# visinf/veto

Measured on AMD Instinct MI355X. Metric: relation-pairs/sec (PredCls, 36 obj/img), higher is better.
Workload: dtype fp16 + e4m3 correction terms (fp16 MFMA main product, e4m3 K=128 MFMA cross terms, fp32 accumulate); 1 GPU; BASELINE.json configs[1]: synthetic PredCls, 12 img x 36 obj = 15120 pairs/GPU, d=576, 8 heads, 4 layers, 51 predicates; images_per_gpu=12, objects_per_image=36, pairs_per_gpu=15120, layers=4, heads=8, precision=mixed, parallelism=single GPU

## Files before the change

### include/veto_amd.h

```cpp
#ifndef VETO_AMD_H_
#define VETO_AMD_H_

#include <stddef.h>
#include <stdint.h>

#ifdef __cplusplus
extern "C" {
#endif

typedef struct veto_handle_s* veto_handle_t;

enum veto_status {
  VETO_OK = 0,
  VETO_ERR_INVALID = -1,
  VETO_ERR_HIP = -2,
  VETO_ERR_WEIGHTS = -3,
  VETO_ERR_WORKSPACE = -4
};

enum veto_precision {
  VETO_PRECISE = 0,
  VETO_FAST = 1,
  VETO_MIXED = 2
};
// ... 425 lines not shown
  float* norms;
  float* total_norm;
  float* coef;
} veto_optim_args_t;

size_t veto_optim_step_workspace_bytes(const veto_optim_args_t* args);
int veto_optim_step(void* stream, const veto_optim_args_t* args, void* workspace, size_t workspace_bytes);

typedef struct veto_roi_pool_args {
  int32_t struct_size;
  int32_t n_levels;
  int32_t n_img, n_roi;
  int32_t channels;
  int32_t depth_channels;
  int32_t pooled;
  int32_t sampling_ratio;
  const float* level_feat[4];
  int32_t level_h[4];
  int32_t level_w[4];
  float level_scale[4];
  const float* depth_feat;
  int32_t depth_h, depth_w;
  const float* rois;
  float* out_rgb;
  float* out_depth;
  int32_t* out_levels;
} veto_roi_pool_args_t;

int veto_roi_pool(void* stream, const veto_roi_pool_args_t* args);

int veto_roi_pool_backward(void* stream, const veto_roi_pool_args_t* args, const float* grad_rgb, const float* grad_depth,
                           float* const* level_grad, float* depth_grad);

typedef struct veto_sgg_eval_args {
  int32_t struct_size;
  int32_t n_img;
  int32_t n_rel_cls;
  int32_t n_zeroshot;
  float iou_thres;
  int32_t reserved0;
  const int32_t* gt_offset;
  const int32_t* obj_offset;
  const int32_t* pair_offset;
  const int64_t* gt_rels;
  const int64_t* gt_classes;
  const float* gt_boxes;
  const int64_t* pred_pairs;
  const float* rel_scores;
  const int64_t* pred_classes;
  const float* pred_boxes;
  const float* obj_scores;
  const int64_t* zeroshot;
  int32_t* gc_rank;
  int32_t* ng_rank;
  int32_t* acc_rank;
  int32_t* zeroshot_flag;
  int32_t* ng_rows;
  int32_t* ng_cols;
  int32_t* ng_count;
  double* metrics;
  const int32_t* pred_obj_offset;
} veto_sgg_eval_args_t;

size_t veto_sgg_eval_workspace_bytes(int32_t n_img, int32_t n_pair_total, int32_t n_gt_total, int32_t n_rel_cls);
int veto_sgg_eval(void* stream, const veto_sgg_eval_args_t* args, int32_t n_pair_total, int32_t n_gt_total,
                  void* workspace, size_t workspace_bytes);

typedef struct veto_sgg_eval_fold_args {
  int32_t struct_size;
  int32_t n_img;
  int32_t n_rel_cls;
  int32_t mode;
  int32_t n_gt_total;
  int32_t reserved0;
  const int32_t* img_gt_offset;
  const int32_t* img_pair_count;
  const int32_t* gt_predicate;
  const int32_t* gc_rank;
  const int32_t* ng_rank;
  const int32_t* acc_rank;
  const int32_t* zeroshot_flag;
  double* metrics;
  double* per_image;
} veto_sgg_eval_fold_args_t;

size_t veto_sgg_eval_fold_workspace_bytes(int32_t n_img, int32_t n_rel_cls);
int veto_sgg_eval_fold(void* stream, const veto_sgg_eval_fold_args_t* args, void* workspace, size_t workspace_bytes);

int veto_sgg_eval_fold_limits(int32_t* images_per_chunk, int32_t* max_rel_cls);

typedef struct veto_det_eval_match_args {
  int32_t struct_size;
  int32_t n_img;
  int32_t n_cls;
  int32_t n_gt;
  int32_t n_det;
  int32_t reserved0;
  int64_t first_gt_id;
  int64_t row_offset;
  double iou_thrs[10];
  double area_rngs[8];
  const int32_t* gt_offset;
  const int32_t* det_offset;
  const int32_t* gt_offset_host;
  const int32_t* det_offset_host;
  const float* gt_boxes;
  const int64_t* gt_labels;
  const float* det_boxes;
  const float* det_scores;
  const int64_t* det_labels;
  uint64_t* rec_key;
  uint64_t* rec_match;
  uint64_t* rec_ignore;
  int64_t* gt_counts;
  int32_t* label_errors;
} veto_det_eval_match_args_t;

size_t veto_det_eval_match_workspace_bytes(int32_t n_img, int32_t n_gt, int32_t n_det);
int veto_det_eval_match(void* stream, const veto_det_eval_match_args_t* args, void* workspace, size_t workspace_bytes);

typedef struct veto_det_eval_accumulate_args {
  int32_t struct_size;
  int32_t n_cls;
  int64_t n_rec;
  double iou_thrs[10];
  double rec_thrs[101];
  const uint64_t* rec_key;
  const uint64_t* rec_match;
  const uint64_t* rec_ignore;
  const int64_t* gt_counts;
  double* precision;
  double* recall;
  double* stats;
  double* recall50_100;
} veto_det_eval_accumulate_args_t;

size_t veto_det_eval_accumulate_workspace_bytes(int64_t n_rec, int32_t n_cls);
int veto_det_eval_accumulate(void* stream, const veto_det_eval_accumulate_args_t* args, void* workspace, size_t workspace_bytes);

int veto_det_eval_limits(int32_t* max_gt_per_image, int32_t* max_det_per_image, int32_t* scan_chunk, int32_t* sort_tile);

int veto_profile_enable(veto_handle_t h, int32_t on);
int veto_profile_collect(veto_handle_t h);
int veto_profile_entry(veto_handle_t h, int index, const char** name, double* total_ms, int64_t* launches,
                       double* flops_per_launch, double* bytes_per_launch);
int veto_profile_reset(veto_handle_t h);

int veto_debug_gemm(void* stream, const float* a, const float* w, const float* bias, float* c, int32_t m,
                    int32_t n, int32_t k, int32_t precision, void* workspace, size_t workspace_bytes);
size_t veto_debug_gemm_workspace_bytes(int32_t m, int32_t n, int32_t k);
int veto_debug_gemm_forms(void* stream, const float* a, const float* w, void* c, int32_t m, int32_t n, int32_t k,
                          int32_t kb_tiles, int32_t kb_steps, int32_t out_form, void* workspace, size_t workspace_bytes);

int veto_debug_ffn(void* stream, const float* a, const float* w1, const float* b1, const float* w2, const float* b2,
                   float* x, int32_t m, int32_t mode, int32_t flags, int32_t reps, float* ms_per_rep, void* workspace,
                   size_t workspace_bytes, const float* ln_w, const float* ln_b, void* ln_rows);
size_t veto_debug_ffn_workspace_bytes(int32_t m);

int veto_debug_outproj(void* stream, const float* a, const float* w, const float* b, float* x, int32_t m, int32_t mode,
                       int32_t flags, int32_t reps, float* ms_per_rep, void* workspace, size_t workspace_bytes,
                       const float* ln_w, const float* ln_b, void* ln_rows);
size_t veto_debug_outproj_workspace_bytes(int32_t m);

int veto_debug_layer_tail(void* stream, const float* a, const float* wo, const float* bo, const float* ln2_w, const float* ln2_b,
                          const float* w1, const float* b1, const float* w2, const float* b2, float* x, int32_t m, int32_t mode,
                          int32_t reps, float* ms_per_rep, void* workspace, size_t workspace_bytes, const float* ln_w,
                          const float* ln_b, void* ln_rows);
size_t veto_debug_layer_tail_workspace_bytes(int32_t m);

int veto_debug_qkv_attn(void* stream, const float* a, const float* wqkv, int32_t n_pair, int32_t heads, int32_t mode, int32_t reps,
                        float* ms_per_rep, void* workspace, size_t workspace_bytes, void* out_rows);
size_t veto_debug_qkv_attn_workspace_bytes(int32_t n_pair);

size_t veto_ce_loss_workspace_bytes(int32_t n);
int veto_ce_loss(void* stream, const float* logits, int64_t ld, const int64_t* labels, const float* weight,
                 const int64_t* rows, int32_t n, int32_t n_cls, float* loss, float* grad, void* workspace,
                 size_t workspace_bytes);

int veto_meet_sample(void* stream, const int64_t* labels, int32_t n, const uint32_t* words, int32_t n_words,
                     const int32_t* incre_idx_list, const int32_t* pos_in_group, const int32_t* group_size,
                     const double* sample_rates, int32_t n_groups, int32_t n_cls, int64_t* chosen,
                     int64_t* group_labels, int32_t* counts, int32_t* words_used);

typedef struct veto_train_opts {
  int32_t struct_size;
  float p_pos, p_emb, p_attn;
  uint64_t seed;
  float* d_roi_rgb;
  float* d_roi_depth;
} veto_train_opts_t;

size_t veto_train_workspace_bytes(veto_handle_t h, int32_t n_obj, int32_t n_pair);
size_t veto_grad_floats(veto_handle_t h);
int veto_weight_offset(veto_handle_t h, int index, size_t* offset_floats);
int veto_forward_train(veto_handle_t h, void* stream, const veto_inputs_t* in, const veto_train_opts_t* opts, void* workspace,
                       size_t workspace_bytes, float* out_logits);
int veto_backward(veto_handle_t h, void* stream, const veto_inputs_t* in, const veto_train_opts_t* opts, void* workspace,
                  size_t workspace_bytes, const float* dlogits, float* grads);

int veto_debug_wgrad(void* stream, const float* dy, const float* x, float* dw, int32_t m, int32_t n, int32_t k,
                     int32_t k_splits, void* workspace, size_t workspace_bytes);
size_t veto_debug_wgrad_workspace_bytes(int32_t m, int32_t n, int32_t k, int32_t k_splits);

int veto_debug_attention_backward(void* stream, const float* qkv, const float* dout, float* dqkv, int32_t n_pair, int32_t heads);
size_t veto_debug_layernorm_backward_workspace_bytes(int32_t rows);
int veto_debug_layernorm_backward(void* stream, const float* x, const float* dy, const float* gamma, const float* dres,
                                  float* dx, float* dgamma_dbeta, int32_t rows, void* workspace, size_t workspace_bytes);
int veto_debug_gelu_backward(void* stream, const float* pre, const float* dh, float* dpre, size_t n);
int veto_debug_column_sums(void* stream, const float* dy, int64_t ld, int32_t rows, int32_t n_cols, float* out,
                           void* workspace, size_t workspace_bytes);

#define VETO_ATTN_BWD_CLS_ONLY 1u
#define VETO_ATTN_BWD_QKV_F24 2u
#define VETO_ATTN_BWD_SPLIT_OUT 4u
int veto_debug_attention_backward_forms(void* stream, const void* qkv, const float* dout, void* dqkv, float* qkv_unpacked,
                                        int32_t n_pair, int32_t heads, uint32_t flags);
int32_t veto_debug_layernorm_backward_col_partial_rows(int32_t rows);
int veto_debug_layernorm_backward_split(void* stream, const float* x, const float* dy, const float* gamma, const float* dres,
                                        float* dx, float* dgamma_dbeta, void* split_rows, float* col_partials, int32_t rows,
                                        uint64_t drop_seed, uint32_t drop_thresh, float drop_scale, void* workspace,
                                        size_t workspace_bytes);

#ifdef __cplusplus
}
#endif
#endif
```

### veto_amd/csrc/abi_core.hip

```cpp
#include <atomic>
#include <cstdlib>
#include <cstring>

#include "abi_internal.h"

thread_local std::string g_abi_err;

namespace veto {
bool env_knob_is(const char* name, const char* value) {
  const char* v = getenv(name);
  return v && !strcmp(v, value);
}
int device_cu_count() {
  static std::atomic<int> cache[64];
  int dev = 0, cus = 0;
  if (hipGetDevice(&dev) != hipSuccess || dev < 0) return -1;
  if (dev < 64 && (cus = cache[dev].load(std::memory_order_relaxed)) > 0) return cus;
  if (hipDeviceGetAttribute(&cus, hipDeviceAttributeMultiprocessorCount, dev) != hipSuccess || cus <= 0) return -1;
  if (dev < 64) cache[dev].store(cus, std::memory_order_relaxed);
  return cus;
}
int env_knob_int(const char* name, int dflt) {
  const char* v = getenv(name);
  return v ? atoi(v) : dflt;
}
}

static int fold_block_width(int heads) {
  static const bool off = env_knob_is("VETO_FOLD_BLOCKS", "0");
  if (off || heads <= 0 || kDim % heads != 0) return 0;
  const int dhp = (kDim / heads + 31) / 32 * 32;
  return 192 % dhp == 0 && (heads * dhp) % 192 == 0 ? dhp : 0;
}

int finalize_weights(veto_handle_t h, hipStream_t s, bool train_only) {
  for (const Param& q : h->params)
    if (!q.loaded) return fail(VETO_ERR_WEIGHTS, "weight '%s' was never loaded", q.name.c_str());
  const int L = h->cfg.layers;
  const bool base = h->dirty;
  for (int l = 0; l < L; ++l) {
    LayerW& w = h->layers[l];
    if (base)
      for (int i = 0; i < 4; ++i) {
        const LayerLinear& q = kLayerLinears[i];
        HIP_TRY(launch_split_rows(h->p(lname(l, q.weight)), w.split(i), q.N, q.K, s));
      }
    if (h->cfg.precision != VETO_PRECISE && !train_only)
      for (int i = 0; i < 4; ++i) {
        const LayerLinear& q = kLayerLinears[i];
        HIP_TRY(launch_mixed_weight_rows(h->p(lname(l, q.weight)), w.mixed_rows(i), q.N, q.K, w.exp_m + i, s));
      }
  }
  if (base) {
  const std::string pe = std::string(kT) + "patch_embed.";
  HIP_TRY(launch_build_patch_weight(h->p(pe + "proj_d.weight"), h->p(pe + "proj_d.bias"), h->p(pe + "proj_v.weight"),
                                    h->p(pe + "proj_v.bias"), h->patch_w, h->patch_bias, s));
  HIP_TRY(launch_transpose_pair_proj(h->p("location_projection.0.weight"), h->loc_wt, kPosDim, s));
  HIP_TRY(launch_transpose_pair_proj(h->p("class_projection.0.weight"), h->cls_wt, h->cfg.embed_dim, s));
  HIP_TRY(launch_transpose_head(h->p("rel_out.weight"), h->head_wt, h->cfg.num_out, s));
  }
  if (train_only) {
    h->dirty = false;
    h->infer_dirty = true;
    ++h->weight_gen;
    return VETO_OK;
  }
  {
    const std::string T0 = kT;
    HIP_TRY(launch_qkv0_consts(h->p(lname(0, "0.fn.to_qkv.weight")), h->layers[0].ln1_w, h->layers[0].ln1_b, h->p(T0 + "pos_embedding"),
                               h->p(T0 + "cls_token"), h->fold_tmp, h->q0_vec, s));
    HIP_TRY(launch_split_rows(h->fold_tmp, h->q0_w, 3 * kDim, kDim, s));
  }
  if (h->cfg.heads <= cls_fold_max_heads()) {
    const int H = h->cfg.heads, dh = kDim / H;
    const float* qkv = h->p(lname(L - 1, "0.fn.to_qkv.weight"));
    const float* wo = h->p(lname(L - 1, "0.fn.to_out.0.weight"));
    if (h->fold_dhp > 0) {
      const int np = H * h->fold_dhp;
      HIP_TRY(launch_fold_blocks(qkv, wo, h->fold_tmp, 0, H, h->fold_dhp, s));
      HIP_TRY(launch_split_rows(h->fold_tmp, h->fold_q, (size_t)np, kDim, s));
      HIP_TRY(launch_fold_blocks(qkv, wo, h->fold_tmp, 1, H, h->fold_dhp, s));
      HIP_TRY(launch_split_rows(h->fold_tmp, h->fold_k, (size_t)H * kDim, np, s));
      HIP_TRY(launch_fold_blocks(qkv, wo, h->fold_tmp, 2, H, h->fold_dhp, s));
      HIP_TRY(launch_split_rows(h->fold_tmp, h->fold_v, (size_t)np, H * kDim, s));
      HIP_TRY(launch_fold_blocks(qkv, wo, h->fold_tmp, 3, H, h->fold_dhp, s));
      HIP_TRY(launch_split_rows(h->fold_tmp, h->fold_o, (size_t)kDim, np, s));
    } else {
    for (int hd = 0; hd < H; ++hd)
      HIP_TRY(launch_sgemm_tn(qkv + ((size_t)kDim + hd * dh) * kDim, kDim, qkv + (size_t)hd * dh * kDim, kDim,
                              h->fold_tmp + (size_t)hd * kDim * kDim, kDim, dh, kDim, kDim, s));
    HIP_TRY(launch_split_rows(h->fold_tmp, h->fold_m, (size_t)H * kDim, kDim, s));
    for (int hd = 0; hd < H; ++hd)
      HIP_TRY(launch_sgemm_nn(wo + hd * dh, kDim, qkv + ((size_t)2 * kDim + hd * dh) * kDim, kDim, h->fold_tmp + (size_t)hd * kDim,
                              (long)H * kDim, kDim, kDim, dh, s));
    HIP_TRY(launch_split_rows(h->fold_tmp, h->fold_n, (size_t)kDim, H * kDim, s));
    }
  }
  if (base) ++h->weight_gen;
  h->dirty = false;
  h->infer_dirty = false;
  return VETO_OK;
}

int run_gemm(veto_handle_t h, hipStream_t s, const char* name, const __bf16* a, SplitW w, const float* bias,
             const float* resid, long ldr, float* c, __bf16* c_split, long ldc, int M, int N, int K, int epi,
             long lda, int w_row0, DropSite drop, const int* w_exp, int kb_tiles, int kb_steps) {
  GemmArgs g{};
  g.kb_tiles = kb_tiles; g.kb_steps = kb_steps;
  if (w_exp) { g.fmt = FMT_MIXED; g.w_exp = w_exp; }
  if (drop.thresh) {
    if (epi != EPI_RESID) return fail(VETO_ERR_INVALID, "dropout is fused into the residual epilogue only");
    epi = EPI_RESID_DROP;
    g.drop_seed = drop.seed; g.drop_thresh = drop.thresh; g.drop_scale = drop.scale; g.drop_row_step = drop.row_step;
  }
  g.a = a; g.lda = lda;
  g.w = w + (size_t)w_row0 * 2 * K;
  g.bias = bias; g.resid = resid; g.c = c; g.c_split = c_split;
  g.M = M; g.N = N; g.K = K; g.ldr = ldr; g.ldc = ldc;
  if (epi == EPI_PRE_GELU) g.ldc_f32 = N;
  const double kk = kb_tiles > 0 ? 32.0 * kb_steps : (double)K;
  const double flops = 2.0 * M * (double)N * kk;
  const double bytes = 4.0 * ((double)M * K + (double)N * kk) + (double)M * N * (epi == EPI_RESID ? 8.0 : epi == EPI_F24 ? 3.0 : 4.0);
  ProfScope ps(h, s, name, flops, bytes);
  HIP_TRY(launch_gemm_split(g, epi, 0, s));
  return VETO_OK;
}

static size_t carve_derived(veto_handle_t h, char* base) {
  Carver c{base};
  const veto_config_t& cfg = h->cfg;
  const int L = cfg.layers, E = cfg.embed_dim;
  const bool mixed = cfg.precision != VETO_PRECISE;
  for (LayerW& w : h->layers) {
    w.qkv = c.take<__bf16>((size_t)3 * kDim * kDim * 4);
    w.out = c.take<__bf16>((size_t)kDim * kDim * 4);
    w.fc1 = c.take<__bf16>((size_t)2 * kDim * kDim * 4);
    w.fc2 = c.take<__bf16>((size_t)2 * kDim * kDim * 4);
    if (!mixed) continue;
    w.qkv_m = c.take<__bf16>((size_t)3 * kDim * kDim * 4);
    w.out_m = c.take<__bf16>((size_t)kDim * kDim * 4);
    w.fc1_m = c.take<__bf16>((size_t)2 * kDim * kDim * 4);
    w.fc2_m = c.take<__bf16>((size_t)2 * kDim * kDim * 4);
  }
  int* exps = c.take<int>((size_t)L * 4 * sizeof(int));
  for (int l = 0; l < L && mixed && exps; ++l) h->layers[l].exp_m = exps + 4 * l;
  h->patch_w = c.take<__bf16>((size_t)2 * kDim * 2048 * 4);
  h->patch_bias = c.take<float>((size_t)2 * kDim * 4);
  h->loc_wt = c.take<float>((size_t)kPosDim * 2 * kDim * 4);
  h->cls_wt = c.take<float>((size_t)E * 2 * kDim * 4);
  h->head_wt = c.take<float>((size_t)kDim * cfg.num_out * 4);
  const int fold_dhp = h->fold_dhp = fold_block_width(cfg.heads);
  const size_t fold_np = (size_t)cfg.heads * (fold_dhp > 0 ? fold_dhp : 0);
  const size_t fold_el = fold_dhp > 0 ? (size_t)cfg.heads * kDim * fold_np : (size_t)cfg.heads * kDim * kDim;
  h->fold_m = c.take<__bf16>(fold_dhp > 0 ? 256 : fold_el * 4);
  h->fold_n = c.take<__bf16>(fold_dhp > 0 ? 256 : fold_el * 4);
  h->fold_tmp = c.take<float>(fold_el * 4);
  h->fold_q = c.take<__bf16>(fold_np * kDim * 4 + 256);
  h->fold_k = c.take<__bf16>((size_t)cfg.heads * kDim * fold_np * 4 + 256);
  h->fold_v = c.take<__bf16>((size_t)cfg.heads * kDim * fold_np * 4 + 256);
  h->fold_o = c.take<__bf16>(fold_np * kDim * 4 + 256);
  h->q0_w = c.take<__bf16>((size_t)3 * kDim * kDim * 4);
  h->q0_vec = c.take<float>((size_t)3 * 3 * kDim * 4);
  return c.off;
}

extern "C" {

const char* veto_last_error(void) { return g_abi_err.c_str(); }
const char* veto_version(void) { return "veto_amd 0.1 (gfx950)"; }

int veto_create(const veto_config_t* cfg, veto_handle_t* out) {
  CHECK_STRUCT_AND(veto_config_t, cfg, out != nullptr);
  if (cfg->dim != kDim) return fail(VETO_ERR_INVALID, "T_INPUT_DIM must be 576 (proj_d 512 + proj_v 64), got %d", cfg->dim);
  if (cfg->patch != 2 || cfg->channels != 256 || cfg->resolution != 8)
    return fail(VETO_ERR_INVALID, "only PATCH_SIZE 2, 256 channels, POOLER_RESOLUTION 8 are supported");
  if (cfg->layers < 1 || cfg->layers > 64) return fail(VETO_ERR_INVALID, "bad ENC_LAYERS %d", cfg->layers);
  if (cfg->heads < 1 || kDim % cfg->heads != 0 || (kDim / cfg->heads) % 4 != 0)
    return fail(VETO_ERR_INVALID, "NHEADS %d must divide 576 with head dim %% 4 == 0", cfg->heads);
  if (cfg->num_obj_cls < 2 || cfg->num_obj_cls > 256 || cfg->embed_dim < 1 || cfg->embed_dim > 256)
    return fail(VETO_ERR_INVALID, "num_obj_cls/embed_dim out of range");
  if (cfg->num_out < 1 || cfg->num_out > 4096) return fail(VETO_ERR_INVALID, "bad num_out %d", cfg->num_out);
  if (cfg->precision != VETO_PRECISE && cfg->precision != VETO_FAST && cfg->precision != VETO_MIXED) return fail(VETO_ERR_INVALID, "bad precision");
  HIP_TRY(hipSetDevice(cfg->device));

  veto_handle_t h = new veto_handle_s();
  h->cfg = *cfg;
  h->dh = kDim / cfg->heads;
  h->chunk = cfg->max_chunk_pairs > 0 ? cfg->max_chunk_pairs : 32768;
  const int E = cfg->embed_dim, L = cfg->layers;
  h->add("obj_embed.weight", (size_t)cfg->num_obj_cls * E);
  h->add("class_projection.0.weight", (size_t)kDim * 2 * E);
  h->add("class_projection.0.bias", kDim);
  h->add("pos_embed.0.weight", 4);
  h->add("pos_embed.0.bias", 4);
  h->add("pos_embed.0.running_mean", 4);
  h->add("pos_embed.0.running_var", 4);
  h->add("pos_embed.1.weight", (size_t)kPosDim * 4);
  h->add("pos_embed.1.bias", kPosDim);
  h->add("location_projection.0.weight", (size_t)kDim * 2 * kPosDim);
  h->add("location_projection.0.bias", kDim);
  h->add(std::string(kT) + "cls_token", kDim);
  h->add(std::string(kT) + "pos_embedding", kDim);
  h->add(std::string(kT) + "patch_embed.proj_d.weight", (size_t)512 * 2048);
  h->add(std::string(kT) + "patch_embed.proj_d.bias", 512);
  h->add(std::string(kT) + "patch_embed.proj_v.weight", (size_t)64 * 2048);
  h->add(std::string(kT) + "patch_embed.proj_v.bias", 64);
  for (int l = 0; l < L; ++l) {
    h->add(lname(l, "0.norm.weight"), kDim);
    h->add(lname(l, "0.norm.bias"), kDim);
    h->add(lname(l, "0.fn.to_qkv.weight"), (size_t)3 * kDim * kDim);
    h->add(lname(l, "0.fn.to_out.0.weight"), (size_t)kDim * kDim);
    h->add(lname(l, "0.fn.to_out.0.bias"), kDim);
    h->add(lname(l, "1.norm.weight"), kDim);
    h->add(lname(l, "1.norm.bias"), kDim);
    h->add(lname(l, "1.fn.net.0.weight"), (size_t)2 * kDim * kDim);
    h->add(lname(l, "1.fn.net.0.bias"), 2 * kDim);
    h->add(lname(l, "1.fn.net.3.weight"), (size_t)2 * kDim * kDim);
    h->add(lname(l, "1.fn.net.3.bias"), kDim);
  }
  h->add("rel_out.weight", (size_t)cfg->num_out * kDim);
  h->add("rel_out.bias", cfg->num_out);
  for (Param& q : h->params) {
    q.offset = h->raw_floats;
    h->raw_floats += align_up(q.numel, 64);
  }
  hipError_t e = hipMalloc((void**)&h->raw, h->raw_floats * sizeof(float));
  if (e != hipSuccess) { delete h; return fail(VETO_ERR_HIP, "hipMalloc(raw weights): %s", hipGetErrorString(e)); }

  h->layers.resize(L);
  e = hipMalloc((void**)&h->derived, carve_derived(h, nullptr));
  if (e != hipSuccess) { (void)hipFree(h->raw); delete h; return fail(VETO_ERR_HIP, "hipMalloc(derived weights): %s", hipGetErrorString(e)); }
  carve_derived(h, h->derived);
  for (int l = 0; l < L; ++l) {
    LayerW& w = h->layers[l];
    w.ln1_w = h->p(lname(l, "0.norm.weight")); w.ln1_b = h->p(lname(l, "0.norm.bias"));
    w.ln2_w = h->p(lname(l, "1.norm.weight")); w.ln2_b = h->p(lname(l, "1.norm.bias"));
    w.out_b = h->p(lname(l, "0.fn.to_out.0.bias"));
    w.fc1_b = h->p(lname(l, "1.fn.net.0.bias"));
    w.fc2_b = h->p(lname(l, "1.fn.net.3.bias"));
  }
  if (cfg->precision == VETO_MIXED) {
    e = hipMalloc((void**)&h->sat_buf, (size_t)L * VETO_SAT_SITES * 4 * sizeof(unsigned long long));
    if (e != hipSuccess) { (void)hipFree(h->raw); (void)hipFree(h->derived); delete h; return fail(VETO_ERR_HIP, "hipMalloc(saturation counters): %s", hipGetErrorString(e)); }
  }
  *out = h;
  return VETO_OK;
}

int veto_destroy(veto_handle_t h) {
  if (!h) return VETO_OK;
  for (ProfRec& r : h->prof_recs) { (void)hipEventDestroy(r.start); (void)hipEventDestroy(r.stop); }
  for (hipEvent_t e : h->event_pool) (void)hipEventDestroy(e);
  (void)hipFree(h->raw);
  (void)hipFree(h->derived);
  if (h->sat_buf) (void)hipFree(h->sat_buf);
  delete h;
  return VETO_OK;
}

int veto_num_weights(veto_handle_t h) { return h ? (int)h->params.size() : fail(VETO_ERR_INVALID, "null handle"); }

int veto_weight_info(veto_handle_t h, int index, const char** name, size_t* numel) {
  if (!h || index < 0 || index >= (int)h->params.size()) return fail(VETO_ERR_INVALID, "bad weight index");
  if (name) *name = h->params[index].name.c_str();
  if (numel) *numel = h->params[index].numel;
  return VETO_OK;
}

int veto_load_weights(veto_handle_t h, const char* name, const float* src, size_t numel, void* stream) {
  if (!h || !name || !src) return fail(VETO_ERR_INVALID, "null argument");
  auto it = h->index.find(name);
  if (it == h->index.end()) return fail(VETO_ERR_INVALID, "unknown weight '%s'", name);
  Param& q = h->params[it->second];
  if (q.numel != numel) return fail(VETO_ERR_INVALID, "weight '%s': expected %zu elements, got %zu", name, q.numel, numel);
  HIP_TRY(hipMemcpyAsync(h->raw + q.offset, src, numel * sizeof(float), hipMemcpyDefault, (hipStream_t)stream));
  q.loaded = true;
  h->dirty = true;
// ... 57 lines not shown
```

### veto_amd/csrc/abi_debug.hip

```cpp
#include "abi_internal.h"

namespace {

struct EventTimer {
  hipEvent_t e0 = nullptr, e1 = nullptr;
  hipStream_t s = nullptr;
  float total_ms = 0.f;
  hipError_t init(hipStream_t stream) {
    s = stream;
    hipError_t e = hipEventCreate(&e0);
    return e != hipSuccess ? e : hipEventCreate(&e1);
  }
  hipError_t start() { return e1 ? hipEventRecord(e0, s) : hipSuccess; }
  hipError_t stop() {
    if (!e1) return hipSuccess;
    float ms = 0.f;
    hipError_t e = hipEventRecord(e1, s);
    if (e == hipSuccess) e = hipEventSynchronize(e1);
    if (e == hipSuccess) e = hipEventElapsedTime(&ms, e0, e1);
    total_ms += ms;
    return e;
  }
  ~EventTimer() {
    if (e0) (void)hipEventDestroy(e0);
    if (e1) (void)hipEventDestroy(e1);
  }
};

const size_t kW = (size_t)kDim * kDim * 4;
size_t act_bytes(size_t rows, size_t k) { return (size_t)gemm_rows_padded((int)rows) * k * 4; }

struct GemmWs { __bf16 *a, *w; int* w_exp; size_t total; };
GemmWs carve_gemm(Carver c, int m, int n, int k) {
  return GemmWs{c.take<__bf16>(act_bytes(m, k)), c.take<__bf16>((size_t)n * k * 4), c.take<int>(256), c.off};
}

struct FfnWs { __bf16 *a, *hid, *w1, *w2; int* exps; size_t total; };
FfnWs carve_ffn(Carver c, int m) {
  return FfnWs{c.take<__bf16>(act_bytes(m, kDim)), c.take<__bf16>(act_bytes(m, 2 * kDim)), c.take<__bf16>(2 * kW), c.take<__bf16>(2 * kW),
               c.take<int>(256), c.off};
}

struct OutprojWs { __bf16 *a, *w; int* exps; size_t total; };
OutprojWs carve_outproj(Carver c, int m) {
  return OutprojWs{c.take<__bf16>(act_bytes(m, kDim)), c.take<__bf16>(kW), c.take<int>(256), c.off};
}

struct LayerTailWs { __bf16 *a, *wo, *w1, *w2; int* exps; size_t total; };
LayerTailWs carve_layer_tail(Carver c, int m) {
  return LayerTailWs{c.take<__bf16>(act_bytes(m, kDim)), c.take<__bf16>(kW), c.take<__bf16>(2 * kW), c.take<__bf16>(2 * kW), c.take<int>(256),
                     c.off};
}

struct QkvAttnWs { __bf16* a; char *o, *qkv; __bf16* w; int* exps; size_t total; };
QkvAttnWs carve_qkv_attn(Carver c, int n_pair) {
  const size_t tile_rows = qkv_attn_rows_padded(n_pair), m = (size_t)n_pair * kTokens, rows = tile_rows > m ? tile_rows : m;
  return QkvAttnWs{c.take<__bf16>(act_bytes(rows, kDim)), c.take(act_bytes(rows, kDim)), c.take((size_t)gemm_rows_padded((int)rows) * 3 * kDim * 3),
                   c.take<__bf16>(3 * kW), c.take<int>(256), c.off};
}

}

extern "C" {

size_t veto_debug_gemm_workspace_bytes(int32_t m, int32_t n, int32_t k) {
  if (m <= 0 || n <= 0 || k <= 0) return 0;
  return carve_gemm(Carver{nullptr}, m, n, k).total;
}

int veto_debug_gemm(void* stream, const float* a, const float* w, const float* bias, float* c, int32_t m, int32_t n,
                    int32_t k, int32_t precision, void* workspace, size_t workspace_bytes) {
  if (!a || !w || !c || !workspace) return fail(VETO_ERR_INVALID, "null argument");
  ABI_TRY(check_workspace(workspace, workspace_bytes, veto_debug_gemm_workspace_bytes(m, n, k), false));
  hipStream_t s = (hipStream_t)stream;
  const auto [a_s, w_s, w_exp, ws_bytes] = carve_gemm(Carver{(char*)workspace}, m, n, k);
  HIP_TRY(hipMemsetAsync(a_s, 0, (char*)w_s - (char*)a_s, s));
  GemmArgs g{};
  if (precision == VETO_MIXED) {
    if (k % 64 != 0) return fail(VETO_ERR_INVALID, "mixed rows need K %% 64 == 0");
    HIP_TRY(launch_mixed_act_rows(a, a_s, (size_t)m, k, s));
    HIP_TRY(launch_mixed_weight_rows(w, w_s, (size_t)n, k, w_exp, s));
    g.fmt = FMT_MIXED; g.w_exp = w_exp;
  } else {
    HIP_TRY(launch_split_rows(a, a_s, (size_t)m, k, s));
    HIP_TRY(launch_split_rows(w, w_s, (size_t)n, k, s));
  }
  g.a = a_s; g.w = w_s; g.bias = bias; g.c = c;
  g.M = m; g.N = n; g.K = k; g.ldc = n;
  hipError_t e = launch_gemm_split(g, EPI_F32, precision == VETO_FAST ? 1 : 0, s);
  if (e != hipSuccess) return fail(e == hipErrorInvalidValue ? VETO_ERR_INVALID : VETO_ERR_HIP,
                                   "gemm launch failed (N must be a multiple of 192, K of 32): %s", hipGetErrorString(e));
  return VETO_OK;
}

int veto_debug_gemm_forms(void* stream, const float* a, const float* w, void* c, int32_t m, int32_t n, int32_t k, int32_t kb_tiles,
                          int32_t kb_steps, int32_t out_form, void* workspace, size_t workspace_bytes) {
  if (!a || !w || !c || !workspace) return fail(VETO_ERR_INVALID, "null argument");
  if (out_form < 0 || out_form > 2) return fail(VETO_ERR_INVALID, "out_form must be 0, 1 or 2");
  ABI_TRY(check_workspace(workspace, workspace_bytes, veto_debug_gemm_workspace_bytes(m, n, k), false));
  hipStream_t s = (hipStream_t)stream;
  const auto [a_s, w_s, w_exp, ws_bytes] = carve_gemm(Carver{(char*)workspace}, m, n, k);
  HIP_TRY(hipMemsetAsync(a_s, 0, (char*)w_s - (char*)a_s, s));
  HIP_TRY(launch_split_rows(a, a_s, (size_t)m, k, s));
  HIP_TRY(launch_split_rows(w, w_s, (size_t)n, k, s));
  GemmArgs g{};
  g.a = a_s; g.w = w_s; g.M = m; g.N = n; g.K = k;
  g.kb_tiles = kb_tiles; g.kb_steps = kb_steps;
  if (out_form == 1) { g.c_split = (__bf16*)c; g.ldc = 2L * n; }
  else { g.c = (float*)c; g.ldc = n; }
  hipError_t e = launch_gemm_split(g, out_form == 1 ? EPI_SPLIT : out_form == 2 ? EPI_F24 : EPI_F32, 0, s);
  if (e != hipSuccess) return fail(e == hipErrorInvalidValue ? VETO_ERR_INVALID : VETO_ERR_HIP,
                                   "gemm launch failed (N a multiple of 192, K of 32, the blocks must tile K): %s", hipGetErrorString(e));
  return VETO_OK;
}

size_t veto_debug_ffn_workspace_bytes(int32_t m) {
  return m > 0 ? carve_ffn(Carver{nullptr}, m).total : 0;
}

int veto_debug_ffn(void* stream, const float* a, const float* w1, const float* b1, const float* w2, const float* b2, float* x,
                   int32_t m, int32_t mode, int32_t flags, int32_t reps, float* ms_per_rep, void* workspace, size_t workspace_bytes,
                   const float* ln_w, const float* ln_b, void* ln_rows) {
  if (!a || !w1 || !b1 || !w2 || !b2 || !x || !workspace) return fail(VETO_ERR_INVALID, "null argument");
  if (m <= 0 || reps <= 0 || (mode != 0 && mode != 1)) return fail(VETO_ERR_INVALID, "bad m / reps / mode");
  if (ln_rows && (!ln_w || !ln_b)) return fail(VETO_ERR_INVALID, "ln_rows needs ln_w and ln_b");
  ABI_TRY(check_workspace(workspace, workspace_bytes, veto_debug_ffn_workspace_bytes(m), false));
  hipStream_t s = (hipStream_t)stream;
  const auto [a_m, hid, w1_m, w2_m, exps, ws_bytes] = carve_ffn(Carver{(char*)workspace}, m);
  if (flags & 1) {
    HIP_TRY(hipMemsetAsync(a_m, 0, (char*)hid - (char*)a_m, s));
    HIP_TRY(launch_mixed_act_rows(a, a_m, (size_t)m, kDim, s));
    HIP_TRY(launch_mixed_weight_rows(w1, w1_m, (size_t)2 * kDim, kDim, exps + 0, s));
    HIP_TRY(launch_mixed_weight_rows(w2, w2_m, (size_t)kDim, 2 * kDim, exps + 1, s));
  }
  EventTimer timer;
  if (ms_per_rep) HIP_TRY(timer.init(s));
  HIP_TRY(timer.start());
  for (int r = 0; r < reps; ++r) {
    if (mode == 1) {
      HIP_TRY(launch_ffn_fused(ffn_panel_args(a_m, MixedLinear{w1_m, b1, exps + 0}, MixedLinear{w2_m, b2, exps + 1}, x, m,
                                              ln_rows ? RowNorm{ln_w, ln_b, ln_rows} : RowNorm()), s));
    } else {
      GemmArgs g1{};
      g1.fmt = FMT_MIXED; g1.w_exp = exps + 0; g1.a = a_m; g1.w = w1_m; g1.bias = b1; g1.c_split = hid;
      g1.M = m; g1.N = 2 * kDim; g1.K = kDim; g1.ldc = 4 * kDim;
      HIP_TRY(launch_gemm_split(g1, EPI_GELU_SPLIT, 0, s));
      GemmArgs g2{};
      g2.fmt = FMT_MIXED; g2.w_exp = exps + 1; g2.a = hid; g2.w = w2_m; g2.bias = b2; g2.resid = x; g2.c = x;
      g2.M = m; g2.N = kDim; g2.K = 2 * kDim; g2.ldr = kDim; g2.ldc = kDim;
      HIP_TRY(launch_gemm_split(g2, EPI_RESID, 0, s));
      if (ln_rows) HIP_TRY(launch_layernorm(x, kDim, ln_w, ln_b, (__bf16*)ln_rows, m, s, FMT_MIXED));
    }
  }
  HIP_TRY(timer.stop());
  if (ms_per_rep) *ms_per_rep = timer.total_ms / reps;
  return VETO_OK;
}

size_t veto_debug_outproj_workspace_bytes(int32_t m) {
  return m > 0 ? carve_outproj(Carver{nullptr}, m).total : 0;
}

int veto_debug_outproj(void* stream, const float* a, const float* w, const float* b, float* x, int32_t m, int32_t mode, int32_t flags,
                       int32_t reps, float* ms_per_rep, void* workspace, size_t workspace_bytes, const float* ln_w, const float* ln_b,
                       void* ln_rows) {
  if (!a || !w || !b || !x || !workspace) return fail(VETO_ERR_INVALID, "null argument");
  if (m <= 0 || reps <= 0 || (mode != 0 && mode != 1)) return fail(VETO_ERR_INVALID, "bad m / reps / mode");
  if (ln_rows && (!ln_w || !ln_b)) return fail(VETO_ERR_INVALID, "ln_rows needs ln_w and ln_b");
  ABI_TRY(check_workspace(workspace, workspace_bytes, veto_debug_outproj_workspace_bytes(m), false));
  hipStream_t s = (hipStream_t)stream;
  const auto [a_m, w_m, exps, ws_bytes] = carve_outproj(Carver{(char*)workspace}, m);
  if (flags & 1) HIP_TRY(launch_mixed_weight_rows(w, w_m, (size_t)kDim, kDim, exps, s));
  EventTimer timer;
  if (ms_per_rep) HIP_TRY(timer.init(s));
  for (int r = 0; r < reps; ++r) {
    HIP_TRY(hipMemsetAsync(a_m, 0, (char*)w_m - (char*)a_m, s));
    HIP_TRY(launch_mixed_act_rows(a, a_m, (size_t)m, kDim, s));
    HIP_TRY(timer.start());
    if (mode == 1) {
      HIP_TRY(launch_out_fused(out_panel_args(a_m, MixedLinear{w_m, b, exps}, x, m, ln_rows ? RowNorm{ln_w, ln_b, ln_rows} : RowNorm()), s));
    } else {
      GemmArgs g{};
      g.fmt = FMT_MIXED; g.w_exp = exps; g.a = a_m; g.w = w_m; g.bias = b; g.resid = x; g.c = x;
      g.M = m; g.N = kDim; g.K = kDim; g.ldr = kDim; g.ldc = kDim;
      HIP_TRY(launch_gemm_split(g, EPI_RESID, 0, s));
      if (ln_rows) HIP_TRY(launch_layernorm(x, kDim, ln_w, ln_b, (__bf16*)ln_rows, m, s, FMT_MIXED));
    }
    HIP_TRY(timer.stop());
  }
  if (ms_per_rep) *ms_per_rep = timer.total_ms / reps;
  return VETO_OK;
}

size_t veto_debug_layer_tail_workspace_bytes(int32_t m) {
  return m > 0 ? carve_layer_tail(Carver{nullptr}, m).total : 0;
}

int veto_debug_layer_tail(void* stream, const float* a, const float* wo, const float* bo, const float* ln2_w, const float* ln2_b,
                          const float* w1, const float* b1, const float* w2, const float* b2, float* x, int32_t m, int32_t mode,
                          int32_t reps, float* ms_per_rep, void* workspace, size_t workspace_bytes, const float* ln_w, const float* ln_b,
                          void* ln_rows) {
  if (!a || !wo || !bo || !ln2_w || !ln2_b || !w1 || !b1 || !w2 || !b2 || !x || !workspace) return fail(VETO_ERR_INVALID, "null argument");
  if (m <= 0 || reps <= 0 || (mode != 0 && mode != 1)) return fail(VETO_ERR_INVALID, "bad m / reps / mode");
  if (ln_rows && (!ln_w || !ln_b)) return fail(VETO_ERR_INVALID, "ln_rows needs ln_w and ln_b");
  ABI_TRY(check_workspace(workspace, workspace_bytes, veto_debug_layer_tail_workspace_bytes(m), false));
  hipStream_t s = (hipStream_t)stream;
  const auto [a_m, wo_m, w1_m, w2_m, exps, ws_bytes] = carve_layer_tail(Carver{(char*)workspace}, m);
  HIP_TRY(launch_mixed_weight_rows(wo, wo_m, (size_t)kDim, kDim, exps + 0, s));
  HIP_TRY(launch_mixed_weight_rows(w1, w1_m, (size_t)2 * kDim, kDim, exps + 1, s));
  HIP_TRY(launch_mixed_weight_rows(w2, w2_m, (size_t)kDim, 2 * kDim, exps + 2, s));
  EventTimer timer;
  if (ms_per_rep) HIP_TRY(timer.init(s));
  for (int r = 0; r < reps; ++r) {
    HIP_TRY(hipMemsetAsync(a_m, 0, (char*)wo_m - (char*)a_m, s));
    HIP_TRY(launch_mixed_act_rows(a, a_m, (size_t)m, kDim, s));
    HIP_TRY(timer.start());
// ... 55 lines not shown
```

### veto_amd/csrc/abi_forward.hip

```cpp
#include "abi_internal.h"

namespace {

struct Workspace {
  int32_t *subj, *obj;
  float* lc;
  __bf16* pa;
  float* patch_tab;
  float* x;
  __bf16* a;
  char* big;
  float* xc;
  __bf16* ptab_split;
  float *sw, *ow;
  float* stats;
  __bf16 *ac, *hc;
  size_t total;
};

Workspace carve(char* base, int n_obj, int n_pair, int chunk) {
  Workspace w;
  Carver c{base};
  const size_t prow = (size_t)gemm_rows_padded(n_obj * 16);
  const size_t tile_rows = qkv_attn_rows_padded(chunk);
  const size_t mpad = (size_t)gemm_rows_padded((int)(tile_rows > (size_t)chunk * kTokens ? tile_rows : (size_t)chunk * kTokens));
  const size_t cpad = (size_t)gemm_rows_padded(chunk);
  w.subj = c.take<int32_t>((size_t)n_pair * 4);
  w.obj = c.take<int32_t>((size_t)n_pair * 4);
  w.lc = c.take<float>((size_t)n_obj * 2 * 2 * kDim * 4);
  w.pa = c.take<__bf16>(prow * 2 * 2048 * 2);
  w.patch_tab = c.take<float>((size_t)n_obj * 16 * 2 * kDim * 4);
  w.x = c.take<float>(mpad * kDim * 4);
  w.a = c.take<__bf16>(mpad * 2 * kDim * 2);
  {
    const size_t qkv_bytes = mpad * 3 * kDim * 4, fold_bytes = 2 * (align_up(cpad * (size_t)cls_fold_max_heads() * kDim * 4, 256));
    w.big = c.take(qkv_bytes > fold_bytes ? qkv_bytes : fold_bytes);
  }
  w.xc = c.take<float>(cpad * kDim * 4);
  w.ptab_split = c.take<__bf16>(prow * 2 * 2 * kDim * 2);
  w.sw = c.take<float>(prow * 3 * kDim * 4);
  w.ow = c.take<float>(prow * 3 * kDim * 4);
  w.stats = c.take<float>(mpad * 2 * 4);
  w.ac = c.take<__bf16>(cpad * 2 * kDim * 2);
  w.hc = c.take<__bf16>(cpad * 4 * kDim * 2);
  w.total = c.off;
  return w;
}

struct ForwardPlan {
  int L, H, dhp;
  bool qkv0_tables, fold_last, mixed, fast, mixed_out, cls_mixed, tail_fused, panel, qkv_f24, qa_fused, x_f24;
  bool ffn_ln_next(int l) const { return mixed && panel && l + 1 < L - 1; }
};

ForwardPlan make_plan(veto_handle_t h, bool sat) {
  ForwardPlan p;
  const int L = p.L = h->cfg.layers, H = p.H = h->cfg.heads;
  p.dhp = h->fold_dhp;
  static const bool tables_off = env_knob_is("VETO_QKV0_TABLES", "0");
  p.qkv0_tables = L >= 2 && !tables_off;
  static const bool fold_off = env_knob_is("VETO_CLS_FOLD", "0");
  p.fold_last = !fold_off && H <= cls_fold_max_heads();
  p.mixed = h->cfg.precision != VETO_PRECISE;
  p.fast = h->cfg.precision == VETO_FAST;
  p.mixed_out = p.mixed && attention_reads_tables(H);
  p.cls_mixed = p.mixed;
  static const bool tail_off = env_knob_is("VETO_TAIL_FUSED", "0");
  p.tail_fused = !tail_off && !sat;
  p.panel = !sat;
  static const bool qkv_f24_off = env_knob_is("VETO_QKV_F24", "0");
  p.qkv_f24 = !qkv_f24_off && attention_reads_tables(H);
  static const bool qa_off = env_knob_is("VETO_QKV_ATTN_FUSED", "0");
  p.qa_fused = p.mixed && p.mixed_out && p.tail_fused && !qa_off && qkv_attn_fused_supports(H);
  static const bool x_f24_on = env_knob_is("VETO_X_F24", "1");
  p.x_f24 = x_f24_on && !p.fast && p.mixed && p.mixed_out && p.tail_fused && p.fold_last && p.qkv0_tables && p.qa_fused && L >= 3;
  return p;
}

int object_side(veto_handle_t h, hipStream_t s, const Workspace& ws, const ForwardPlan& p, const veto_inputs_t* in,
                const veto_debug_outputs_t* dbg) {
  const int n_obj = in->n_obj, n_pair = in->n_pair;
  {
    ProfScope ps(h, s, "pair_indices", 0, (double)n_pair * 24);
    HIP_TRY(launch_pair_indices(in->rel_pairs, in->img_obj_offset, in->img_pair_offset, in->n_img, n_pair, ws.subj,
                                ws.obj, dbg ? dbg->subj_inds : nullptr, dbg ? dbg->obj_inds : nullptr, s));
  }
  {
    if (in->bn_batch_stats) HIP_TRY(launch_bn_batch_stats(in->boxes, in->box_mode, n_obj, in->bn_batch_stats, s));
    const ObjPrepArgs a = obj_prep_args(h, in, ws.lc);
    ProfScope ps(h, s, "obj_prep", 2.0 * n_obj * 2 * kDim * (kPosDim + h->cfg.embed_dim), (double)n_obj * 2 * 2 * kDim * 4);
    HIP_TRY(launch_obj_prep(a, s));
  }
  {
    ProfScope ps(h, s, "patchify", 0, (double)n_obj * 2 * 256 * 64 * (4 + 4));
    HIP_TRY(launch_patchify(in->roi_depth, in->roi_rgb, ws.pa, n_obj, s));
  }
  int rc = run_gemm(h, s, "gemm_patch", ws.pa, h->patch_w, h->patch_bias, nullptr, 0, ws.patch_tab, nullptr, 2 * kDim,
                    n_obj * 16, 2 * kDim, 2048, EPI_F32);
  if (rc || !p.qkv0_tables) return rc;
  const int R = n_obj * 16;
  HIP_TRY(launch_centre_split(ws.patch_tab, ws.ptab_split, R, s));
  ABI_TRY(run_gemm(h, s, "gemm_qkv0_tab", ws.ptab_split, h->q0_w, h->q0_vec + 3 * kDim, nullptr, 0, ws.sw, nullptr, 3 * kDim, R, 3 * kDim, kDim,
                   EPI_F32, (long)2 * 2 * kDim, 0));
  return run_gemm(h, s, "gemm_qkv0_tab", ws.ptab_split + 2 * kDim, h->q0_w, nullptr, nullptr, 0, ws.ow, nullptr, 3 * kDim, R, 3 * kDim, kDim,
                  EPI_F32, (long)2 * 2 * kDim, 0);
}

struct Chunk {
  veto_handle_t h;
  hipStream_t s;
  const Workspace& ws;
  const ForwardPlan& p;
  int c0, np, M;
  unsigned long long* sat;
  const float* xlast;
  float* qkv() const { return (float*)ws.big; }
  __bf16* hid() const { return (__bf16*)ws.big; }
  hipError_t count_sat(int layer, int site, const void* rows, long stride_bytes, int n_rows, int K) const {
    if (!sat) return hipSuccess;
    return launch_count_saturation(rows, stride_bytes, n_rows, K, sat + ((size_t)layer * VETO_SAT_SITES + site) * 4, s);
  }

  int assemble_tokens(float* dbg_tokens) {
    {
      AssembleArgs a = assemble_args(h, ws.patch_tab, ws.lc, ws.subj + c0, ws.obj + c0, ws.x, ws.a, np);
      a.stats = p.qkv0_tables ? ws.stats : nullptr;
      a.x_f24 = p.x_f24 ? 1 : 0;
      a.a_fmt = p.mixed && p.qkv0_tables ? FMT_MIXED : FMT_SPLIT;
      ProfScope ps(h, s, "assemble_tokens", 0, (double)M * kDim * (p.x_f24 ? 3 : 4) + (p.qkv0_tables ? (double)M * 8 + 2.0 * np * kDim * 4 : (double)M * kDim * 4));
      HIP_TRY(launch_assemble(a, s));
    }
    if (dbg_tokens) {
      float* dst = dbg_tokens + (size_t)c0 * kTokens * kDim;
      if (p.x_f24) HIP_TRY(launch_unpack_f24(ws.x, dst, (size_t)M * kDim, s));
      else HIP_TRY(hipMemcpyAsync(dst, ws.x, (size_t)M * kDim * 4, hipMemcpyDeviceToDevice, s));
    }
    return VETO_OK;
  }

  int qkv0_from_tables() {
    const LayerW& w = h->layers[0];
    const bool mixed = p.mixed;
    if (!attention_reads_tables(p.H)) {
      ProfScope ps(h, s, "qkv0_combine", 0, (double)np * 17 * 3 * kDim * 4 * 3);
      HIP_TRY(launch_qkv0_combine(ws.sw, ws.ow, ws.stats, h->q0_vec, ws.subj + c0, ws.obj + c0, qkv(), np, s));
    }
    for (int t = kTokens - 2; t < kTokens; ++t) {
      if (mixed) HIP_TRY(count_sat(0, VETO_SAT_QKV_IN, ws.a + (size_t)t * 2 * kDim, (long)kTokens * kDim * 4, np, kDim));
      ABI_TRY(run_gemm(h, s, "gemm_qkv0_lc", ws.a + (size_t)t * 2 * kDim, mixed ? w.qkv_m : w.qkv, nullptr, nullptr, 0,
                       qkv() + (size_t)t * 3 * kDim, nullptr, (long)kTokens * 3 * kDim, np, 3 * kDim, kDim, EPI_F32, (long)kTokens * 2 * kDim, 0,
                       DropSite(), mixed ? w.exp_m + LIN_QKV : nullptr));
    }
    return VETO_OK;
  }

  int attention(int l, bool qkv_f24) {
    const bool last = l == p.L - 1;
    AttnArgs a{};
    a.qkv = qkv(); a.n_pair = np; a.heads = p.H; a.cls_only = last ? 1 : 0;
    a.qkv_f24 = qkv_f24 ? 1 : 0;
    a.o = last ? ws.ac : ws.a;
    a.o_fmt = (!last && p.mixed_out) ? FMT_MIXED : FMT_SPLIT;
    if (l == 0 && p.qkv0_tables && attention_reads_tables(p.H)) {
      a.sw = ws.sw; a.ow = ws.ow; a.stats = ws.stats; a.vec = h->q0_vec; a.subj = ws.subj + c0; a.obj = ws.obj + c0;
    }
    const double nq = last ? 1 : kTokens;
    ProfScope ps(h, s, last ? "attention_cls" : "attention", 4.0 * np * nq * kTokens * kDim,
                 (double)M * 3 * kDim * (qkv_f24 ? 3 : 4) + (double)np * nq * kDim * 4);
    HIP_TRY(launch_attention(a, s));
    if (a.o_fmt == FMT_MIXED) HIP_TRY(count_sat(l, VETO_SAT_ATTN_OUT, ws.a, (long)kDim * 4, M, kDim));
    return VETO_OK;
  }

  int qkv_attention(int l, bool* attn_in_big) {
    const LayerW& w = h->layers[l];
    if (p.qa_fused && l > 0) {
      QkvAttnArgs q{};
      q.a = (const char*)ws.a; q.w = (const char*)w.qkv_m; q.w_exp = w.exp_m + LIN_QKV; q.o = ws.big; q.n_pair = np; q.heads = p.H; q.fast = p.fast ? 1 : 0;
      ProfScope ps(h, s, "qkv_attn_fused", 2.0 * M * 3.0 * kDim * kDim + 4.0 * np * kTokens * kTokens * kDim,
                   (double)M * kDim * 8 + 3.0 * kDim * kDim * 4);
      HIP_TRY(launch_qkv_attn_fused(q, s));
      *attn_in_big = true;
      return VETO_OK;
    }
    const bool mq = p.mixed && l > 0;
    const bool qkv_f24 = mq && p.qkv_f24;
    if (mq) HIP_TRY(count_sat(l, VETO_SAT_QKV_IN, ws.a, (long)kDim * 4, M, kDim));
    int rc = run_gemm(h, s, "gemm_qkv", ws.a, mq ? w.qkv_m : w.qkv, nullptr, nullptr, 0, qkv(), nullptr, 3 * kDim, M, 3 * kDim, kDim,
                      qkv_f24 ? EPI_F24 : EPI_F32, 0, 0, DropSite(), mq ? w.exp_m + LIN_QKV : nullptr);
    return rc ? rc : attention(l, qkv_f24);
  }

  int layer_tail_one_launch(int l, bool attn_in_big) {
    const LayerW& w = h->layers[l];
    const LayerW& nx = h->layers[l + 1];
    const bool ln_next = p.ffn_ln_next(l);
    char* rows = attn_in_big ? ws.big : (char*)ws.a;
    const RowNorm next{ln_next ? nx.ln1_w : nullptr, ln_next ? nx.ln1_b : nullptr, attn_in_big ? ws.a : nullptr};
    FfnArgs f = layer_tail_args(rows, w.mixed(LIN_OUT), RowNorm{w.ln2_w, w.ln2_b, rows}, w.mixed(LIN_FC1), w.mixed(LIN_FC2), ws.x, M, next);
    f.fast = p.fast ? 1 : 0;
    if (p.x_f24) {
      f.resid_f24 = 1;
      if (l + 1 < p.L - 1) f.out_f24 = 1;
      else {
        if (!attn_in_big) return fail(VETO_ERR_INVALID, "internal: 3-byte residual rows without a free buffer for the last tail's fp32 rows");
        f.out = (float*)ws.a;
        xlast = (const float*)ws.a;
      }
    }
    ProfScope ps(h, s, "layer_tail_fused", 2.0 * M * (double)kDim * kDim + 2.0 * 2.0 * M * (double)kDim * 2 * kDim,
                 (double)M * kDim * (p.x_f24 ? (f.out_f24 ? 14 : 15) : 16) + 5.0 * kDim * kDim * 4);
    HIP_TRY(launch_layer_tail(f, s));
    return VETO_OK;
  }

  int out_projection(int l) {
    const LayerW& w = h->layers[l];
    if (p.mixed_out && p.panel) {
      const FfnArgs f = out_panel_args(ws.a, w.mixed(LIN_OUT), ws.x, M, RowNorm{w.ln2_w, w.ln2_b, ws.a});
      ProfScope ps(h, s, "out_ln_fused", 2.0 * M * (double)kDim * kDim, (double)M * kDim * 16 + (double)kDim * kDim * 4);
      HIP_TRY(launch_out_fused(f, s));
      return VETO_OK;
    }
    ABI_TRY(run_gemm(h, s, "gemm_out", ws.a, p.mixed_out ? w.out_m : w.out, w.out_b, ws.x, kDim, ws.x, nullptr, kDim, M, kDim, kDim, EPI_RESID,
                     0, 0, DropSite(), p.mixed_out ? w.exp_m + LIN_OUT : nullptr));
    {
      ProfScope ps(h, s, "layernorm", 0, (double)M * kDim * 8);
      HIP_TRY(launch_layernorm(ws.x, kDim, w.ln2_w, w.ln2_b, ws.a, M, s, p.mixed ? FMT_MIXED : FMT_SPLIT));
    }
    if (p.mixed) HIP_TRY(count_sat(l, VETO_SAT_FFN_IN, ws.a, (long)kDim * 4, M, kDim));
    return VETO_OK;
  }

  int feed_forward(int l) {
    const LayerW& w = h->layers[l];
    const bool mixed = p.mixed;
    if (mixed && p.panel) {
      const LayerW& nx = h->layers[l + 1];
      const FfnArgs f = ffn_panel_args(ws.a, w.mixed(LIN_FC1), w.mixed(LIN_FC2), ws.x, M,
                                       p.ffn_ln_next(l) ? RowNorm{nx.ln1_w, nx.ln1_b, ws.a} : RowNorm());
      ProfScope ps(h, s, "ffn_fused", 2.0 * 2.0 * M * (double)kDim * 2 * kDim, (double)M * kDim * 12 + 2.0 * 2 * kDim * kDim * 4);
      HIP_TRY(launch_ffn_fused(f, s));
      return VETO_OK;
    }
    ABI_TRY(run_gemm(h, s, "gemm_fc1", ws.a, mixed ? w.fc1_m : w.fc1, w.fc1_b, nullptr, 0, nullptr, hid(), 4 * kDim, M, 2 * kDim, kDim,
                     EPI_GELU_SPLIT, 0, 0, DropSite(), mixed ? w.exp_m + LIN_FC1 : nullptr));
    if (mixed) HIP_TRY(count_sat(l, VETO_SAT_HIDDEN, hid(), (long)2 * kDim * 4, M, 2 * kDim));
    return run_gemm(h, s, "gemm_fc2", hid(), mixed ? w.fc2_m : w.fc2, w.fc2_b, ws.x, kDim, ws.x, nullptr, kDim, M, kDim, 2 * kDim, EPI_RESID,
                    0, 0, DropSite(), mixed ? w.exp_m + LIN_FC2 : nullptr);
  }

  int layer_tail(int l, bool attn_in_big) {
    if (p.mixed_out && p.tail_fused) return layer_tail_one_launch(l, attn_in_big);
    const int rc = out_projection(l);
    return rc ? rc : feed_forward(l);
  }

  int layernorm_next(int l) {
    const LayerW& nx = h->layers[l + 1];
    if (l + 1 == p.L - 1 && p.fold_last) return VETO_OK;
    if (p.ffn_ln_next(l)) return VETO_OK;
    ProfScope ps(h, s, "layernorm", 0, (double)M * kDim * 8);
    HIP_TRY(launch_layernorm(ws.x, kDim, nx.ln1_w, nx.ln1_b, ws.a, M, s, (p.mixed && l + 1 < p.L - 1) ? FMT_MIXED : FMT_SPLIT));
    return VETO_OK;
  }

  int last_layer_folded() {
    const LayerW& w = h->layers[p.L - 1];
    const int H = p.H;
    int rc;
    Carver fold{ws.big};
    float* u = fold.take<float>((size_t)gemm_rows_padded(np) * H * kDim * 4);
    __bf16* abar = fold.take<__bf16>((size_t)gemm_rows_padded(np) * 2 * H * kDim * 2);
    {
      ProfScope ps(h, s, "layernorm_cls", 0, (double)np * kDim * 8);
      HIP_TRY(launch_layernorm(xlast, (long)kTokens * kDim, w.ln1_w, w.ln1_b, ws.ac, np, s));
    }
    const int dhp = p.dhp, npad = H * dhp;
    bool u24 = false;
    if (dhp > 0) {
      ABI_TRY(run_gemm(h, s, "gemm_q_cls", ws.ac, h->fold_q, nullptr, nullptr, 0, nullptr, ws.hc, 2L * npad, np, npad, kDim, EPI_SPLIT));
      u24 = cls_fold_reads_f24();
      rc = run_gemm(h, s, "gemm_u_cls", ws.hc, h->fold_k, nullptr, nullptr, 0, u, nullptr, (long)H * kDim, np, H * kDim, npad,
                    u24 ? EPI_F24 : EPI_F32, 0, 0, DropSite(), nullptr, 3, dhp / 32);
    } else {
      rc = run_gemm(h, s, "gemm_u_cls", ws.ac, h->fold_m, nullptr, nullptr, 0, u, nullptr, (long)H * kDim, np, H * kDim, kDim, EPI_F32);
    }
    if (rc) return rc;
    {
      ProfScope ps(h, s, "attention_cls", 4.0 * np * H * kTokens * kDim, (double)M * kDim * 4 + (double)np * H * kDim * 8);
      HIP_TRY(launch_cls_fold_attention(xlast, w.ln1_w, w.ln1_b, u, abar, np, H, s, u24));
    }
    if (dhp > 0) {
      const int hpt = 192 / dhp;
      ABI_TRY(run_gemm(h, s, "gemm_v_cls", abar, h->fold_v, nullptr, nullptr, 0, nullptr, ws.hc, 2L * npad, np, npad, H * kDim, EPI_SPLIT,
                       0, 0, DropSite(), nullptr, 1, hpt * kDim / 32));
      return run_gemm(h, s, "gemm_out_cls", ws.hc, h->fold_o, w.out_b, xlast, (long)kTokens * kDim, ws.xc, nullptr, kDim, np, kDim, npad,
                      EPI_RESID);
// ... 125 lines not shown
```

### veto_amd/csrc/abi_internal.h

```cpp
#pragma once
#include <hip/hip_runtime.h>

#include <cmath>
#include <cstdarg>
#include <cstddef>
#include <cstdint>
#include <cstdio>
#include <map>
#include <string>
#include <vector>

#include "../../include/veto_amd.h"
#include "kernels.h"

using namespace veto;

#pragma GCC visibility push(hidden)

extern thread_local std::string g_abi_err;

inline int fail(int code, const char* fmt, ...) {
  char buf[512];
  va_list ap;
  va_start(ap, fmt);
// ... 96 lines not shown
  p.obj_logits = a->obj_logits; p.rel_pairs = a->rel_pairs;
  p.n_obj = a->n_obj; p.n_pair = a->n_pair; p.n_rel_cls = a->n_rel_cls; p.n_obj_cls = a->n_obj_cls;
  p.obj_scores = a->obj_scores; p.obj_pred = a->obj_pred; p.out_prob = a->rel_prob_sorted;
  p.out_pairs = a->rel_pairs_sorted; p.out_labels = a->rel_labels_sorted; p.out_triple = a->triple_sorted;
  return p;
}

struct Param {
  std::string name;
  size_t numel = 0;
  size_t offset = 0;
  bool loaded = false;
};

typedef __bf16* SplitW;

enum { LIN_QKV = 0, LIN_OUT = 1, LIN_FC1 = 2, LIN_FC2 = 3 };
struct LayerLinear { const char* weight; const char* bias; int N, K; };
const LayerLinear kLayerLinears[4] = {{"0.fn.to_qkv.weight", nullptr, 3 * kDim, kDim},
                                      {"0.fn.to_out.0.weight", "0.fn.to_out.0.bias", kDim, kDim},
                                      {"1.fn.net.0.weight", "1.fn.net.0.bias", 2 * kDim, kDim},
                                      {"1.fn.net.3.weight", "1.fn.net.3.bias", kDim, 2 * kDim}};

struct MixedLinear {
  const void* w;
  const float* b;
  const int* exp;
};

struct LayerW {
  const float *ln1_w, *ln1_b, *ln2_w, *ln2_b, *out_b, *fc1_b, *fc2_b;
  SplitW qkv = nullptr, out = nullptr, fc1 = nullptr, fc2 = nullptr;
  SplitW qkv_m = nullptr, out_m = nullptr, fc1_m = nullptr, fc2_m = nullptr;
  int* exp_m = nullptr;
  SplitW split(int lin) const { return lin == LIN_QKV ? qkv : lin == LIN_OUT ? out : lin == LIN_FC1 ? fc1 : fc2; }
  SplitW mixed_rows(int lin) const { return lin == LIN_QKV ? qkv_m : lin == LIN_OUT ? out_m : lin == LIN_FC1 ? fc1_m : fc2_m; }
  MixedLinear mixed(int lin) const {
    const float* const bias[4] = {nullptr, out_b, fc1_b, fc2_b};
    return MixedLinear{mixed_rows(lin), bias[lin], exp_m + lin};
  }
};

struct ProfRec {
  int name_id;
  hipEvent_t start, stop;
  double flops, bytes;
};

struct veto_handle_s {
  veto_config_t cfg;
  int dh = 0;
  int chunk = 0;
  std::vector<Param> params;
  std::map<std::string, int> index;
  float* raw = nullptr;
  size_t raw_floats = 0;
  char* derived = nullptr;
  bool dirty = true;
  bool infer_dirty = false;
  uint64_t weight_gen = 0;
  static constexpr size_t kMaxTrainWorkspaces = 8;
  std::map<const void*, uint64_t> train_gen;
  void stamp_train_workspace(const void* ws) {
    if (train_gen.size() >= kMaxTrainWorkspaces && !train_gen.count(ws)) {
      auto old = train_gen.begin();
      for (auto it = train_gen.begin(); it != train_gen.end(); ++it)
        if (it->second < old->second) old = it;
      train_gen.erase(old);
    }
    train_gen[ws] = weight_gen;
  }
  std::vector<LayerW> layers;
  SplitW patch_w = nullptr;
  SplitW fold_m = nullptr, fold_n = nullptr;
  float* fold_tmp = nullptr;
  SplitW fold_q = nullptr, fold_k = nullptr, fold_v = nullptr, fold_o = nullptr;
  int fold_dhp = 0;
  SplitW q0_w = nullptr;
  float* q0_vec = nullptr;
  float* patch_bias = nullptr;
  float* loc_wt = nullptr;
  float* cls_wt = nullptr;
  float* head_wt = nullptr;
  unsigned long long* sat_buf = nullptr;
  bool prof_on = false;
  std::vector<std::string> prof_names;
  std::vector<ProfRec> prof_recs;
  std::vector<hipEvent_t> event_pool;
  struct Agg { double ms = 0; int64_t n = 0; double flops = 0, bytes = 0; };
  std::vector<Agg> prof_agg;

  const float* p(const std::string& name) const { return raw + params[index.at(name)].offset; }
  void add(const std::string& name, size_t numel) {
    Param q;
    q.name = name;
    q.numel = numel;
    index[name] = (int)params.size();
    params.push_back(q);
  }
};

constexpr const char* kT = "fusion_transformer.transformer.";

inline std::string lname(int l, const char* rest) {
  char buf[160];
  snprintf(buf, sizeof(buf), "%slayers.%d.%s", kT, l, rest);
  return buf;
}

inline int prof_id(veto_handle_t h, const char* name) {
  for (size_t i = 0; i < h->prof_names.size(); ++i)
    if (h->prof_names[i] == name) return (int)i;
  h->prof_names.push_back(name);
  h->prof_agg.emplace_back();
  return (int)h->prof_names.size() - 1;
}

struct ProfScope {
  veto_handle_t h;
  hipStream_t s;
  int rec = -1;
  ProfScope(veto_handle_t h_, hipStream_t s_, const char* name, double flops, double bytes) : h(h_), s(s_) {
    if (!h || !h->prof_on) return;
    ProfRec r;
    r.name_id = prof_id(h, name);
    r.flops = flops;
    r.bytes = bytes;
    for (hipEvent_t* e : {&r.start, &r.stop}) {
      if (!h->event_pool.empty()) { *e = h->event_pool.back(); h->event_pool.pop_back(); }
      else if (hipEventCreate(e) != hipSuccess) return;
    }
    (void)hipEventRecord(r.start, s);
    h->prof_recs.push_back(r);
    rec = (int)h->prof_recs.size() - 1;
  }
  ~ProfScope() {
    if (rec >= 0) (void)hipEventRecord(h->prof_recs[rec].stop, s);
  }
};

int finalize_weights(veto_handle_t h, hipStream_t s, bool train_only = false);

struct DropSite {
  unsigned long long seed = 0;
  unsigned thresh = 0;
  float scale = 1.f;
  int row_step = 1;
};

int run_gemm(veto_handle_t h, hipStream_t s, const char* name, const __bf16* a, SplitW w, const float* bias, const float* resid, long ldr,
             float* c, __bf16* c_split, long ldc, int M, int N, int K, int epi, long lda = 0, int w_row0 = 0, DropSite drop = DropSite(),
             const int* w_exp = nullptr, int kb_tiles = 0, int kb_steps = 0);

inline ObjPrepArgs obj_prep_args(veto_handle_t h, const veto_inputs_t* in, float* lc) {
  ObjPrepArgs a{};
  a.boxes = in->boxes; a.box_mode = in->box_mode; a.labels = in->obj_labels; a.obj_logits = in->obj_logits;
  a.embed = h->p("obj_embed.weight"); a.num_obj_cls = h->cfg.num_obj_cls; a.embed_dim = h->cfg.embed_dim;
  a.bn_w = h->p("pos_embed.0.weight"); a.bn_b = h->p("pos_embed.0.bias");
  a.bn_mean = in->bn_batch_stats ? in->bn_batch_stats : h->p("pos_embed.0.running_mean");
  a.bn_var = in->bn_batch_stats ? in->bn_batch_stats + 4 : h->p("pos_embed.0.running_var");
  a.pos_w = h->p("pos_embed.1.weight"); a.pos_b = h->p("pos_embed.1.bias");
  a.loc_wt = h->loc_wt; a.loc_b = h->p("location_projection.0.bias");
  a.cls_wt = h->cls_wt; a.cls_b = h->p("class_projection.0.bias");
  a.lc = lc; a.pos_out = nullptr; a.n_obj = in->n_obj;
  return a;
}

inline AssembleArgs assemble_args(veto_handle_t h, const float* patch_tab, const float* lc, const int32_t* subj, const int32_t* obj, float* x,
                                  __bf16* a_rows, int n_pair) {
  AssembleArgs a{};
  a.patch_tab = patch_tab; a.lc = lc; a.cls_token = h->p(std::string(kT) + "cls_token");
  a.pos_embedding = h->p(std::string(kT) + "pos_embedding");
  a.ln_w = h->layers[0].ln1_w; a.ln_b = h->layers[0].ln1_b;
  a.subj = subj; a.obj = obj; a.x = x; a.a = a_rows; a.n_pair = n_pair;
  return a;
}

struct RowNorm {
  const float* w = nullptr;
  const float* b = nullptr;
  void* rows = nullptr;
};

inline FfnArgs ffn_panel_args(const void* a, MixedLinear fc1, MixedLinear fc2, float* x, int M, RowNorm next = RowNorm()) {
  FfnArgs f{};
  f.a = (const char*)a; f.w1 = (const char*)fc1.w; f.w2 = (const char*)fc2.w; f.b1 = fc1.b; f.b2 = fc2.b;
  f.resid = x; f.out = x; f.ldr = kDim; f.ldo = kDim; f.M = M; f.exp1 = fc1.exp; f.exp2 = fc2.exp;
  f.ln_w = next.w; f.ln_b = next.b; f.ln_out = (char*)next.rows;
  return f;
}

inline FfnArgs out_panel_args(const void* a, MixedLinear out, float* x, int M, RowNorm ln2 = RowNorm()) {
  FfnArgs f{};
  f.a = (const char*)a; f.w2 = (const char*)out.w; f.b2 = out.b; f.resid = x; f.out = x; f.ldr = kDim; f.ldo = kDim;
  f.M = M; f.exp2 = out.exp; f.ln_w = ln2.w; f.ln_b = ln2.b; f.ln_out = (char*)ln2.rows;
  return f;
}

inline FfnArgs layer_tail_args(const void* a, MixedLinear out, RowNorm ln2, MixedLinear fc1, MixedLinear fc2, float* x, int M,
                               RowNorm next = RowNorm()) {
  FfnArgs f = ffn_panel_args(a, fc1, fc2, x, M);
  f.wo = (const char*)out.w; f.bo = out.b; f.expo = out.exp; f.lnm_w = ln2.w; f.lnm_b = ln2.b; f.ln_out = (char*)ln2.rows;
  f.ln_w = next.w; f.ln_b = next.b; f.ln1_out = (char*)next.rows;
  return f;
}

#pragma GCC visibility pop
```

### veto_amd/csrc/gemm_split_ps.hip

```cpp
#include "common.h"
#include "kernels.h"

#include <cstdio>
#include <cstdlib>

namespace veto {

namespace {

constexpr int BM = 256, BN = 192, BK = 32;
constexpr int NCONS = 8, NLOAD = 4;
constexpr int kABytes = BM * 128;
constexpr int kWBytes = BN * 128;
constexpr int kDumpOff = 3 * kABytes + 2 * kWBytes;
constexpr int kBiasOff = kDumpOff + 1024;
constexpr int kBiasSlices = 3;
constexpr int kLdsBytes = kBiasOff + kBiasSlices * BN * 4;
constexpr int kPrefSteps = BN * 4 / 128;
constexpr int CPA = BM / 8 / NLOAD;
constexpr int CPWL = BN / 8 / NLOAD;
#ifndef VETO_GEMM_EPI_T
#define VETO_GEMM_EPI_T 1
#endif
constexpr bool kEpiT = VETO_GEMM_EPI_T;

__device__ __forceinline__ void glds16(const char* src, char* lds_dst) {
  __builtin_amdgcn_global_load_lds((const __attribute__((address_space(1))) void*)src,
                                   (__attribute__((address_space(3))) void*)lds_dst, 16, 0, 0);
}

#ifdef VETO_GEMM_STAMPS
__device__ unsigned long long g_stamps[256 * 8];
__device__ __forceinline__ unsigned long long stamp() {
  __builtin_amdgcn_sched_barrier(0);
  unsigned long long t;
  asm volatile("s_memtime %0\n\ts_waitcnt lgkmcnt(0)" : "=s"(t)::"memory");
  __builtin_amdgcn_sched_barrier(0);
  return t;
}
#define STAMP(x) x = stamp()
#define ACC(a, t1, t0) a += (t1) - (t0)
#else
#define STAMP(x)
#define ACC(a, t1, t0)
#endif

__device__ __forceinline__ void wg_barrier() {
  asm volatile("" ::: "memory");
  __builtin_amdgcn_s_barrier();
  asm volatile("" ::: "memory");
}

typedef int i32x4 __attribute__((ext_vector_type(4)));
typedef int i32x8 __attribute__((ext_vector_type(8)));
typedef _Float16 f16x8 __attribute__((ext_vector_type(8)));
template <int V> struct IntTag { static constexpr int value = V; };

typedef short s16x4 __attribute__((ext_vector_type(4)));
typedef short s16x8 __attribute__((ext_vector_type(8)));
__device__ __forceinline__ s16x4 lds_tr16(const char* p) {
  return __builtin_amdgcn_ds_read_tr16_b64_v4i16((__attribute__((address_space(3))) s16x4*)p);
}
__device__ __forceinline__ bf16x8 lds_tr_frag(const char* p, int pitch4) {
  const s16x4 a = lds_tr16(p), b = lds_tr16(p + pitch4);
  const s16x8 v = __builtin_shufflevector(a, b, 0, 1, 2, 3, 4, 5, 6, 7);
  return __builtin_bit_cast(bf16x8, v);
}

template <int NTERMS, int EPI_T, bool TN = false>
__global__ __launch_bounds__(64 * (NCONS + NLOAD), 3) void gemm_split_ps_kernel(GemmArgs g) {
  constexpr bool kDrop = EPI_T == EPI_RESID_DROP;
  constexpr bool kMixed = NTERMS == 2;
  if constexpr (kMixed) saturating_conversions_on();
  static_assert(!(kMixed && TN), "the mixed-row format has no transposed (weight-gradient) form");
  constexpr bool kGeluBwd = EPI_T == EPI_GELU_BWD;
  constexpr int EPI = kDrop || kGeluBwd ? (int)EPI_RESID : EPI_T;
  __shared__ __attribute__((aligned(16))) char smem[kLdsBytes];

  const int tid = threadIdx.x;
  const int lane = tid & 63;
  const int w = __builtin_amdgcn_readfirstlane(tid >> 6);
  const int b = blockIdx.x;
  const int ksp = EPI == EPI_ATOMIC && g.k_splits > 1 ? g.k_splits : 1;
  const int out_tiles = g.tiles_m * g.tiles_n;
  const int ntiles = out_tiles * ksp;
  const int K = g.K;
  const int nk = g.kb_tiles > 0 ? g.kb_steps : K / BK / ksp;
  const int per_xcd = gridDim.x >> 3;
  auto tile_of = [&](int it) { return (it * 8 + (b & 7)) * per_xcd + (b >> 3); };
  int my_tiles = 0;
  while (tile_of(my_tiles) < ntiles) ++my_tiles;
  if (my_tiles == 0) return;
  const int nstages = my_tiles * nk;

  if (w >= NCONS) {
    const int lw = (w - NCONS) & (NLOAD - 1);
    const int rr = lane >> 3;
    const char* srcA[CPA];
    const char* srcW[CPWL];
    auto src_of = [&](const __bf16* base, long ld, int row, int c) {
      const int r16 = ((c & 1) << 3) + rr;
      const int slot = (lane & 7) ^ ((r16 >> 1) & 7);
      return (const char*)(base + (size_t)row * ld) + slot * 16;
    };
    auto tn_swz = [](int r) { return 2 * ((r & 3) | (((r >> 3) & 1) << 2)); };
    const char* tnA = nullptr;
    const char* tnW = nullptr;
    int tn_rowA = 0, tn_rowW = 0;
    int tn_xa[2] = {0, 0}, tn_wr[CPWL], tn_wx[CPWL];
    if constexpr (TN) {
      tn_xa[0] = (lane ^ tn_swz(lw)) << 4;
      tn_xa[1] = (lane ^ tn_swz(lw + 8)) << 4;
#pragma unroll
      for (int i = 0; i < CPWL; ++i) {
        const int slot = (lw + NLOAD * i) * 64 + lane, r = slot / 48, cc = slot % 48;
        tn_wr[i] = r;
        tn_wx[i] = (cc ^ tn_swz(r)) << 4;
      }
    }
    auto setupA = [&](int tile) {
      int k0 = (tile / out_tiles) * nk;
      tile %= out_tiles;
      const int tile_m = tile / g.tiles_n;
      if (g.kb_tiles > 0) k0 = ((tile % g.tiles_n) / g.kb_tiles) * nk;
      if constexpr (TN) {
        tnA = (const char*)g.a + (size_t)tile_m * (BM * 4);
        tn_rowA = k0 * BK;
        return;
      }
#pragma unroll
      for (int i = 0; i < CPA; ++i) {
        const int c = lw + NLOAD * i;
        int row = tile_m * BM + c * 8 + rr;
        if (g.lda != 2 * K && row >= g.M) row = g.M - 1;
        srcA[i] = src_of(g.a, g.lda, row, c) + (size_t)k0 * 128;
      }
    };
    auto setupW = [&](int tile) {
      int k0 = (tile / out_tiles) * nk;
      tile %= out_tiles;
      const int tile_n = tile % g.tiles_n;
      if (g.kb_tiles > 0) k0 = (tile_n / g.kb_tiles) * nk;
      if constexpr (TN) {
        tnW = (const char*)g.w + (size_t)tile_n * (BN * 4);
        tn_rowW = k0 * BK;
        return;
      }
#pragma unroll
      for (int i = 0; i < CPWL; ++i) {
        const int c = lw + NLOAD * i;
        srcW[i] = src_of(g.w, 2 * K, tile_n * BN + c * 8 + rr, c) + (size_t)k0 * 128;
      }
    };
    int itA = 0, ktA = 0, bufA = 0, itW = 0, ktW = 0, bufW = 0;
    auto issueA = [&]() {
      if (ktA == 0 && lw == 0 && g.bias && lane < BN / 4) {
        const int tn = (tile_of(itA) % out_tiles) % g.tiles_n;
        glds16((const char*)(g.bias + tn * BN) + lane * 16, smem + kBiasOff + (itA % kBiasSlices) * (BN * 4));
      }
      char* dst = smem + bufA * kABytes + lw * 1024;
      if constexpr (TN) {
#pragma unroll
        for (int i = 0; i < CPA; ++i) {
          const int row = tn_rowA + ktA * BK + lw + NLOAD * i;
          const char* p = row < g.k_valid ? tnA + (size_t)row * (size_t)(g.lda * 2) : (const char*)g.zero;
          glds16(p + tn_xa[(i >> 1) & 1], dst + NLOAD * i * 1024);
        }
      } else {
#pragma unroll
      for (int i = 0; i < CPA; ++i) glds16(srcA[i] + (size_t)ktA * 128, dst + NLOAD * i * 1024);
      }
      bufA = bufA == 2 ? 0 : bufA + 1;
      if (++ktA == nk) {
        ktA = 0;
        if (++itA < my_tiles) setupA(tile_of(itA));
      }
    };
    auto issueW = [&]() {
      char* dst = smem + 3 * kABytes + bufW * kWBytes + lw * 1024;
      if constexpr (TN) {
#pragma unroll
        for (int i = 0; i < CPWL; ++i) {
          const int row = tn_rowW + ktW * BK + tn_wr[i];
          const char* p = row < g.k_valid ? tnW + (size_t)row * (size_t)(g.ldw * 2) : (const char*)g.zero;
          glds16(p + tn_wx[i], dst + NLOAD * i * 1024);
        }
      } else {
#pragma unroll
      for (int i = 0; i < CPWL; ++i) glds16(srcW[i] + (size_t)ktW * 128, dst + NLOAD * i * 1024);
      }
      bufW ^= 1;
      if (++ktW == nk) {
        ktW = 0;
        if (++itW < my_tiles) setupW(tile_of(itW));
      }
    };
    auto prefetch_resid = [&](int tile, int j) {
      const int tile_n = tile % g.tiles_n, tile_m = tile / g.tiles_n;
      int row = tile_m * BM + lw * 64 + lane;
      if (row >= g.M) row = g.M - 1;
      const float* p = g.resid + (size_t)row * g.ldr + tile_n * BN + j * 32;
      __builtin_amdgcn_global_load_lds((const __attribute__((address_space(1))) void*)p,
                                       (__attribute__((address_space(3))) void*)(smem + kDumpOff + lw * 256), 4, 0, 0);
    };
    unsigned long long tA = 0, tB = 0, tC = 0, tD = 0, t_begin = 0, a_vm = 0, a_bar = 0, a_iss = 0;
    (void)tA; (void)tB; (void)tC; (void)tD; (void)t_begin; (void)a_vm; (void)a_bar; (void)a_iss;
    STAMP(t_begin);
    setupA(tile_of(0));
    setupW(tile_of(0));
    issueA();
    issueW();
    if (nstages > 1) issueA();
    bool pref_in_flight = false;
    int itC = 0, ktC = 0;
    for (int s = 0; s < nstages; ++s) {
      STAMP(tA);
      if (s + 1 >= nstages) asm volatile("s_waitcnt vmcnt(0)" ::: "memory");
      else if (pref_in_flight) asm volatile("s_waitcnt vmcnt(%0)" ::"n"(CPA + 1) : "memory");
      else asm volatile("s_waitcnt vmcnt(%0)" ::"n"(CPA) : "memory");
      STAMP(tB);
      wg_barrier();
      STAMP(tC);
      if (s + 1 < nstages) issueW();
      if (s + 2 < nstages) issueA();
      pref_in_flight = false;
      if (EPI == EPI_RESID && s + 2 < nstages && ktC >= nk - kPrefSteps) {
        prefetch_resid(tile_of(itC), ktC - (nk - kPrefSteps));
        pref_in_flight = true;
      }
      if (++ktC == nk) { ktC = 0; ++itC; }
      STAMP(tD);
      ACC(a_vm, tB, tA); ACC(a_bar, tC, tB); ACC(a_iss, tD, tC);
    }
#ifdef VETO_GEMM_STAMPS
    if (lw == 0 && lane == 0) {
      g_stamps[b * 8 + 4] = a_vm; g_stamps[b * 8 + 5] = a_bar; g_stamps[b * 8 + 6] = a_iss; g_stamps[b * 8 + 7] = tD - t_begin;
    }
#endif
    return;
  }

  const int wm = w >> 1, wn = w & 1;
  const int fr = lane & 15, fq = lane >> 4;
  const int frag_off = fr * 128 + ((fq ^ ((fr >> 1) & 7)) << 4);
  const int a_off = (wm * 64) * 128 + frag_off;
  const int w_off = 3 * kABytes + (wn * 96) * 128 + frag_off;
  const int tn_g = lane >> 4, tn_q = (lane >> 2) & 3, tn_p = lane & 3;
  const int tn_y = ((2 * (tn_q | ((tn_g & 1) << 2))) ^ (tn_p >> 1)) << 4;
  const int tn_a = (8 * tn_g + tn_q) * (BM * 4) + tn_y + (tn_p & 1) * 8 + wm * 256;
  const int tn_w = 3 * kABytes + (8 * tn_g + tn_q) * (BN * 4) + (tn_p & 1) * 8;

  const int mix_scale = kMixed ? (127 - kMixActExp - __builtin_amdgcn_readfirstlane(*g.w_exp)) * 0x01010101 : 0;
  (void)mix_scale;
  unsigned long long t0 = 0, t1 = 0, t2 = 0, t3 = 0, t_begin = 0, a_bar = 0, a_cmp = 0, a_epi = 0;
  (void)t0; (void)t1; (void)t2; (void)t3; (void)t_begin; (void)a_bar; (void)a_cmp; (void)a_epi;
  STAMP(t_begin);
  int s = 0, s3 = 0;
  for (int it = 0; it < my_tiles; ++it) {
    const int tile = tile_of(it) % out_tiles;
    const int tile_n = tile % g.tiles_n, tile_m = tile / g.tiles_n;
    f32x4 acc[6][4];
#pragma unroll
    for (int n = 0; n < 6; ++n)
#pragma unroll
      for (int m = 0; m < 4; ++m) acc[n][m] = f32x4{0.f, 0.f, 0.f, 0.f};

    bf16x8 ah[4], al[4], wh[6], wl[6];
    i32x4 fa0[4], fa1[4], fw0[6], fw1[6];
    auto stage = [&](auto kind_tag) {
      constexpr int KIND = decltype(kind_tag)::value;
      STAMP(t0);
      wg_barrier();
      STAMP(t1);
      const char* sa = smem + s3 * kABytes;
      const char* sw = smem + (s & 1) * kWBytes;
      auto rdA = [&](int m) {
        if constexpr (kMixed) {
          fa0[m] = *(const i32x4*)(sa + a_off + m * 2048);
          fa1[m] = *(const i32x4*)(sa + ((a_off + m * 2048) ^ 64));
        } else if constexpr (TN) {
          const int o = tn_a ^ (((m >> 1) * 8 + (m & 1) * 2) << 4);
          ah[m] = lds_tr_frag(sa + o, 4 * BM * 4);
          if (NTERMS == 3) al[m] = lds_tr_frag(sa + (o ^ 64), 4 * BM * 4);
        } else {
          ah[m] = *(const bf16x8*)(sa + a_off + m * 2048);
          if (NTERMS == 3) al[m] = *(const bf16x8*)(sa + ((a_off + m * 2048) ^ 64));
        }
      };
      auto rdW = [&](int n) {
        if constexpr (kMixed) {
          fw0[n] = *(const i32x4*)(sw + w_off + n * 2048);
          fw1[n] = *(const i32x4*)(sw + ((w_off + n * 2048) ^ 64));
        } else if constexpr (TN) {
          const int o = tn_w + ((((wn * 3 + (n >> 1)) * 8 + (n & 1) * 2) << 4) ^ tn_y);
          wh[n] = lds_tr_frag(sw + o, 4 * BN * 4);
          if (NTERMS == 3) wl[n] = lds_tr_frag(sw + (o ^ 64), 4 * BN * 4);
        } else {
          wh[n] = *(const bf16x8*)(sw + w_off + n * 2048);
          if (NTERMS == 3) wl[n] = *(const bf16x8*)(sw + ((w_off + n * 2048) ^ 64));
        }
      };
      auto mma = [&](int n, int m) {
        if constexpr (kMixed) {
          if constexpr (KIND == 0) {
            acc[n][m] = __builtin_amdgcn_mfma_f32_16x16x32_f16(__builtin_bit_cast(f16x8, fw0[n]), __builtin_bit_cast(f16x8, fa0[m]), acc[n][m], 0, 0, 0);
            acc[n][m] = __builtin_amdgcn_mfma_f32_16x16x32_f16(__builtin_bit_cast(f16x8, fw1[n]), __builtin_bit_cast(f16x8, fa1[m]), acc[n][m], 0, 0, 0);
          } else {
            const i32x8 w8 = __builtin_shufflevector(fw0[n], fw1[n], 0, 1, 2, 3, 4, 5, 6, 7), a8 = __builtin_shufflevector(fa0[m], fa1[m], 0, 1, 2, 3, 4, 5, 6, 7);
            acc[n][m] = __builtin_amdgcn_mfma_scale_f32_16x16x128_f8f6f4(w8, a8, acc[n][m], 0, 0, 0, mix_scale, 0, 0x7f7f7f7f);
          }
        } else {
          if (NTERMS == 3) {
            acc[n][m] = __builtin_amdgcn_mfma_f32_16x16x32_bf16(wl[n], ah[m], acc[n][m], 0, 0, 0);
            acc[n][m] = __builtin_amdgcn_mfma_f32_16x16x32_bf16(wh[n], al[m], acc[n][m], 0, 0, 0);
          }
          acc[n][m] = __builtin_amdgcn_mfma_f32_16x16x32_bf16(wh[n], ah[m], acc[n][m], 0, 0, 0);
        }
      };
      rdW(0);
      rdA(0);
#pragma unroll
      for (int m = 0; m < 4; ++m) {
        if (m < 3) rdA(m + 1); else rdW(1);
        mma(0, m);
      }
#pragma unroll
      for (int n = 1; n < 6; ++n) {
        if (n < 5) rdW(n + 1);
#pragma unroll
        for (int m = 0; m < 4; ++m) mma(n, m);
      }
      if (NTERMS >= 2) {
        constexpr int R = TN ? 2 : 1;
        constexpr int MPB = kMixed ? (KIND == 0 ? 2 : 1) : 3;
        __builtin_amdgcn_sched_group_barrier(0x100, 4 * R, 0);
#pragma unroll
        for (int m = 0; m < 4; ++m) {
          __builtin_amdgcn_sched_group_barrier(0x100, 2 * R, 0);
          __builtin_amdgcn_sched_group_barrier(0x8, MPB, 0);
        }
#pragma unroll
        for (int n = 1; n < 6; ++n) {
          if (n < 5) __builtin_amdgcn_sched_group_barrier(0x100, 2 * R, 0);
          __builtin_amdgcn_sched_group_barrier(0x8, 4 * MPB, 0);
        }
      }
      STAMP(t2);
      ACC(a_bar, t1, t0); ACC(a_cmp, t2, t1);
      ++s;
      s3 = s3 == 2 ? 0 : s3 + 1;
    };
    if constexpr (kMixed) {
      for (int kt = 0; kt < nk; kt += 2) {
        stage(IntTag<0>());
        stage(IntTag<1>());
      }
    } else {
      for (int kt = 0; kt < nk; ++kt) stage(IntTag<0>());
    }

    int lane_e = lane;
    asm volatile("" : "+v"(lane_e));
    const int er = kEpiT ? lane_e >> 2 : lane_e & 15;
    const int eq = kEpiT ? lane_e & 3 : lane_e >> 4;
    const int perm_addr = ((eq << 4) + er) << 2;
    const int row0 = tile_m * BM + wm * 64 + er;
    const int col0 = tile_n * BN + wn * 96 + eq * 4;
    const char* bias_lds = smem + kBiasOff + (it % kBiasSlices) * (BN * 4) + (wn * 96 + eq * 4) * 4;
    f32x4 res[2][3];
    auto load_res = [&](int u, f32x4 (&r)[3]) {
      int row = row0 + (u >> 1) * 16;
      if (row >= g.M) row = g.M - 1;
#pragma unroll
      for (int j = 0; j < 3; ++j) r[j] = *(const f32x4*)(g.resid + (size_t)row * g.ldr + col0 + ((u & 1) * 3 + j) * 16);
    };
    if (EPI == EPI_RESID) load_res(0, res[0]);
#pragma unroll
    for (int u = 0; u < 8; ++u) {
      const int m = u >> 1, h = u & 1;
      if (EPI == EPI_RESID && u < 7) load_res(u + 1, res[(u + 1) & 1]);
      const int row = row0 + m * 16;
#pragma unroll
      for (int j = 0; j < 3; ++j) {
        const int n = h * 3 + j;
        f32x4 t = acc[n][m];
        if (kEpiT) {
#pragma unroll
          for (int e = 0; e < 4; ++e)
            t[e] = __int_as_float(__builtin_amdgcn_ds_bpermute(perm_addr, __float_as_int(acc[n][m][e])));
        }
        if (kGeluBwd) {
          f32x4 v;
#pragma unroll
          for (int e = 0; e < 4; ++e) v[e] = row < g.M ? t[e] * gelu_erf_grad(res[u & 1][j][e]) : 0.f;
          acc[n][m] = v;
        } else if (EPI == EPI_RESID && !kDrop) {
          f32x4 v = t + res[u & 1][j];
          if (g.bias) v += *(const f32x4*)(bias_lds + n * 64);
          acc[n][m] = v;
        } else if (row < g.M) {
          const int col = col0 + n * 16;
          f32x4 v = t;
          if (g.bias) v += *(const f32x4*)(bias_lds + n * 64);
          if (kDrop) {
#pragma unroll
            for (int e = 0; e < 4; ++e)
              v[e] = dropout_keep(g.drop_seed, (unsigned long long)row * g.drop_row_step * g.N + col + e, g.drop_thresh) ? v[e] * g.drop_scale : 0.f;
          }
          if (EPI == EPI_RESID) v += res[u & 1][j];
          if (EPI == EPI_GELU_SPLIT || EPI == EPI_SPLIT) {
            if (EPI == EPI_GELU_SPLIT) {
#pragma unroll
              for (int e = 0; e < 4; ++e) v[e] = gelu_sigmoid(v[e]);
            }
            store_act4<kMixed ? FMT_MIXED : FMT_SPLIT>(g.c_split + (size_t)row * g.ldc, col, v);
          } else if (EPI == EPI_PRE_GELU) {
            *(f32x4*)(g.c + (size_t)row * g.ldc_f32 + col) = v;
#pragma unroll
            for (int e = 0; e < 4; ++e) v[e] = gelu_erf(v[e]);
            store_act4<FMT_SPLIT>(g.c_split + (size_t)row * g.ldc, col, v);
          } else if (EPI == EPI_ATOMIC) {
            float* dstc = g.c + (size_t)row * g.ldc + col;
#pragma unroll
            for (int e = 0; e < 4; ++e) unsafeAtomicAdd(dstc + e, v[e]);
          } else if (EPI == EPI_RESID) {
            acc[n][m] = v;
          } else if (EPI == EPI_F24) {
            *(u32x3*)((char*)g.c + ((size_t)row * g.ldc + col) * 3) = pack_f24x4(v);
          } else {
            *(f32x4*)(g.c + (size_t)row * g.ldc + col) = v;
          }
        }
      }
    }
    if (kGeluBwd) {
      float* cp = g.col_partial + (size_t)(tile_m * 4 + wm) * g.N + col0;
#pragma unroll
      for (int n = 0; n < 6; ++n) {
        f32x4 sum = (acc[n][0] + acc[n][1]) + (acc[n][2] + acc[n][3]);
#pragma unroll
        for (int e = 0; e < 4; ++e) {
          float x = sum[e];
          if (kEpiT) { x += __shfl_xor(x, 4, 64); x += __shfl_xor(x, 8, 64); x += __shfl_xor(x, 16, 64); x += __shfl_xor(x, 32, 64); }
          else { x += __shfl_xor(x, 1, 64); x += __shfl_xor(x, 2, 64); x += __shfl_xor(x, 4, 64); x += __shfl_xor(x, 8, 64); }
          sum[e] = x;
        }
        if (er == 0) *(f32x4*)(cp + n * 16) = sum;
      }
#pragma unroll
      for (int u = 0; u < 8; ++u) {
        const int m = u >> 1, h = u & 1;
        const int row = row0 + m * 16;
        if (row < g.M) {
#pragma unroll
          for (int j = 0; j < 3; ++j) {
            const int n = h * 3 + j;
            store_act4<FMT_SPLIT>(g.c_split + (size_t)row * g.ldc, col0 + n * 16, acc[n][m]);
          }
        }
      }
    } else if (EPI == EPI_RESID) {
#pragma unroll
      for (int u = 0; u < 8; ++u) {
        const int m = u >> 1, h = u & 1;
        const int row = row0 + m * 16;
        if (row < g.M) {
#pragma unroll
          for (int j = 0; j < 3; ++j) {
            const int n = h * 3 + j;
            *(f32x4*)(g.c + (size_t)row * g.ldc + col0 + n * 16) = acc[n][m];
          }
        }
      }
    }
    STAMP(t3);
    ACC(a_epi, t3, t2);
  }
#ifdef VETO_GEMM_STAMPS
  if (w == 0 && lane == 0) {
    g_stamps[b * 8 + 0] = a_bar; g_stamps[b * 8 + 1] = a_cmp; g_stamps[b * 8 + 2] = a_epi; g_stamps[b * 8 + 3] = t3 - t_begin;
  }
#endif
}

template <int NTERMS>
hipError_t launch_ps_terms(GemmArgs g, int epi, int nblocks, hipStream_t s) {
  dim3 grid(nblocks), block(64 * (NCONS + NLOAD));
  if constexpr (NTERMS == 2) {
    switch (epi) {
      case EPI_F32: VETO_LAUNCH((gemm_split_ps_kernel<2, EPI_F32>), grid, block, 0, s, g); break;
      case EPI_F24: VETO_LAUNCH((gemm_split_ps_kernel<2, EPI_F24>), grid, block, 0, s, g); break;
      case EPI_RESID: VETO_LAUNCH((gemm_split_ps_kernel<2, EPI_RESID>), grid, block, 0, s, g); break;
      case EPI_GELU_SPLIT: VETO_LAUNCH((gemm_split_ps_kernel<2, EPI_GELU_SPLIT>), grid, block, 0, s, g); break;
      default: return hipErrorInvalidValue;
    }
    return hipGetLastError();
  } else
  switch (epi) {
    case EPI_F32: VETO_LAUNCH((gemm_split_ps_kernel<NTERMS, EPI_F32>), grid, block, 0, s, g); break;
    case EPI_F24: VETO_LAUNCH((gemm_split_ps_kernel<NTERMS, EPI_F24>), grid, block, 0, s, g); break;
    case EPI_RESID: VETO_LAUNCH((gemm_split_ps_kernel<NTERMS, EPI_RESID>), grid, block, 0, s, g); break;
    case EPI_GELU_SPLIT: VETO_LAUNCH((gemm_split_ps_kernel<NTERMS, EPI_GELU_SPLIT>), grid, block, 0, s, g); break;
    case EPI_SPLIT: VETO_LAUNCH((gemm_split_ps_kernel<NTERMS, EPI_SPLIT>), grid, block, 0, s, g); break;
    case EPI_PRE_GELU:
      if constexpr (NTERMS == 3) { VETO_LAUNCH((gemm_split_ps_kernel<NTERMS, EPI_PRE_GELU>), grid, block, 0, s, g); break; }
      else return hipErrorInvalidValue;
    case EPI_GELU_BWD:
      if constexpr (NTERMS == 3) {
        if (!g.resid || !g.c_split || !g.col_partial || g.bias) return hipErrorInvalidValue;
        VETO_LAUNCH((gemm_split_ps_kernel<NTERMS, EPI_GELU_BWD>), grid, block, 0, s, g);
        break;
      } else return hipErrorInvalidValue;
    case EPI_ATOMIC:
      if (g.tn) VETO_LAUNCH((gemm_split_ps_kernel<NTERMS, EPI_ATOMIC, true>), grid, block, 0, s, g);
      else VETO_LAUNCH((gemm_split_ps_kernel<NTERMS, EPI_ATOMIC>), grid, block, 0, s, g);
      break;
    case EPI_RESID_DROP: VETO_LAUNCH((gemm_split_ps_kernel<NTERMS, EPI_RESID_DROP>), grid, block, 0, s, g); break;
    default: return hipErrorInvalidValue;
  }
  return hipGetLastError();
}

}

int gemm_rows_padded(int m) { return (m + BM - 1) / BM * BM; }

hipError_t launch_gemm_split(GemmArgs g, int epi, int precision, hipStream_t s) {
  if (g.N % BN != 0 || g.K % BK != 0 || g.M <= 0) return hipErrorInvalidValue;
  if (g.lda == 0) g.lda = 2 * (long)g.K;
  g.tiles_m = (g.M + BM - 1) / BM;
  g.tiles_n = g.N / BN;
  return launch_gemm_split_ps(g, epi, precision, s);
}

hipError_t launch_gemm_split_ps(GemmArgs g, int epi, int precision, hipStream_t s) {
  int num_cu = device_cu_count();
  if (num_cu < 1) return hipErrorInvalidDevice;
  num_cu = num_cu / 8 * 8;
  if (num_cu < 8) num_cu = 8;
  const int ksp = epi == EPI_ATOMIC && g.k_splits > 1 ? g.k_splits : 1;
  if ((g.K / BK) % ksp != 0) return hipErrorInvalidValue;
  if (g.kb_tiles > 0 && (ksp != 1 || g.tn || g.fmt == FMT_MIXED || g.kb_steps <= 0 || g.tiles_n % g.kb_tiles != 0 ||
                         (g.tiles_n / g.kb_tiles) * g.kb_steps != g.K / BK))
    return hipErrorInvalidValue;
  if (g.tn && (epi != EPI_ATOMIC || !g.zero || g.lda <= 0 || g.ldw <= 0 || g.k_valid <= 0 || g.k_valid > g.K)) return hipErrorInvalidValue;
  const int ntiles = g.tiles_m * g.tiles_n * ksp;
  int nblocks = num_cu;
  if (ntiles < nblocks) nblocks = (ntiles + 7) / 8 * 8;
  if (g.fmt == FMT_MIXED && (g.tn || !g.w_exp || (g.K / BK) % 2 != 0 || ksp != 1)) return hipErrorInvalidValue;
  hipError_t rc = g.fmt == FMT_MIXED ? launch_ps_terms<2>(g, epi, nblocks, s)
                  : precision == 0 ? launch_ps_terms<3>(g, epi, nblocks, s) : launch_ps_terms<1>(g, epi, nblocks, s);
#ifdef VETO_GEMM_STAMPS
  {
    static unsigned long long host[256 * 8];
    hipDeviceSynchronize();
    hipMemcpyFromSymbol(host, HIP_SYMBOL(g_stamps), sizeof(host));
    double sum[8] = {0};
    for (int bb = 0; bb < nblocks && bb < 256; ++bb)
      for (int k = 0; k < 8; ++k) sum[k] += (double)host[bb * 8 + k];
    fprintf(stderr, "[stamps M%d N%d K%d epi%d] consumer: barrier %.0f compute %.0f epilogue %.0f total %.0f | loader: vmwait %.0f "
            "barrier %.0f issue %.0f total %.0f (mean cycles per workgroup; %d tiles x %d k-steps each)\n", g.M, g.N, g.K, epi,
            sum[0] / nblocks, sum[1] / nblocks, sum[2] / nblocks, sum[3] / nblocks, sum[4] / nblocks, sum[5] / nblocks,
            sum[6] / nblocks, sum[7] / nblocks, (ntiles + nblocks - 1) / nblocks, g.K / BK);
  }
#endif
  return rc;
}

}
```

### veto_amd/csrc/kernels.h

```cpp
#pragma once
#include "common.h"

namespace veto {

enum Epi { EPI_F32 = 0, EPI_RESID = 1, EPI_GELU_SPLIT = 2, EPI_ATOMIC = 3, EPI_RESID_DROP = 4, EPI_F24 = 5, EPI_SPLIT = 6, EPI_PRE_GELU = 7, EPI_GELU_BWD = 8 };

struct GemmArgs {
  const __bf16* a;
  const __bf16* w;
  const float* bias;
  const float* resid;
  float* c;
  __bf16* c_split;
  int M, N, K;
  long lda;
  long ldr;
  long ldc;
  long ldc_f32;
  float* col_partial;
  int k_splits;
  unsigned long long drop_seed;
  unsigned drop_thresh;
  float drop_scale;
  int drop_row_step;
  int tiles_m, tiles_n;
  int fmt;
  int kb_tiles, kb_steps;
  const int* w_exp;
  int tn;
  long ldw;
  int k_valid;
  const __bf16* zero;
};

bool env_knob_is(const char* name, const char* value);
int env_knob_int(const char* name, int dflt);
int gemm_rows_padded(int m);
int device_cu_count();
hipError_t launch_gemm_split(GemmArgs g, int epi, int precision, hipStream_t s);
hipError_t launch_gemm_split_ps(GemmArgs g, int epi, int precision, hipStream_t s);

struct FfnArgs {
  const char* a;
  const char* w1;
  const char* w2;
  const float* b1;
  const float* b2;
  const float* resid;
  float* out;
  long ldr, ldo;
  int M;
  const int* exp1;
  const int* exp2;
  const float* ln_w;
  const float* ln_b;
  char* ln_out;
  char* ln1_out;
  const char* wo;
  const float* bo;
  const int* expo;
  const float* lnm_w;
  const float* lnm_b;
  int resid_f24, out_f24;
  int fast;
  int n_panels;
  int late;
};
int ffn_panel_rows();
hipError_t launch_ffn_fused(FfnArgs g, hipStream_t s);
hipError_t launch_out_fused(FfnArgs g, hipStream_t s);
hipError_t launch_layer_tail(FfnArgs g, hipStream_t s);

hipError_t launch_split_rows(const float* src, __bf16* dst, size_t rows, int K, hipStream_t s);
hipError_t launch_fold_blocks(const float* qkv, const float* wo, float* out, int which, int heads, int dhp, hipStream_t s);
hipError_t launch_mixed_act_rows(const float* src, __bf16* dst, size_t rows, int K, hipStream_t s);
hipError_t launch_mixed_weight_rows(const float* src, __bf16* dst, size_t rows, int K, int* exp_out, hipStream_t s);
hipError_t launch_transpose_split(const float* src, long ld, int M, int N, __bf16* dst, int Mp, hipStream_t s);
hipError_t launch_build_patch_weight(const float* wd, const float* bd, const float* wv, const float* bv,
                                     __bf16* dst, float* bias_cat, hipStream_t s);
hipError_t launch_transpose_pair_proj(const float* src, float* dst, int kin, hipStream_t s);
hipError_t launch_transpose_head(const float* src, float* dst, int n_out, hipStream_t s);

struct ObjPrepArgs {
  const float* boxes;
  int box_mode;
  const int64_t* labels;
  const float* obj_logits;
  const float* embed;
  int num_obj_cls, embed_dim;
  const float* bn_w; const float* bn_b; const float* bn_mean; const float* bn_var;
  const float* pos_w; const float* pos_b;
  const float* loc_wt; const float* loc_b;
  const float* cls_wt; const float* cls_b;
  float* lc;
  float* pos_out;
  int n_obj;
  unsigned long long drop_seed;
  unsigned drop_thresh;
  float drop_scale;
};
hipError_t launch_obj_prep(const ObjPrepArgs& a, hipStream_t s);
hipError_t launch_bn_batch_stats(const float* boxes, int box_mode, int n_obj, float* out, hipStream_t s);
hipError_t launch_patchify(const float* depth, const float* rgb, __bf16* dst, int n_obj, hipStream_t s);

hipError_t launch_pair_indices(const int64_t* rel_pairs, const int32_t* img_obj_off,
                               const int32_t* img_pair_off, int n_img, int n_pair, int32_t* subj,
                               int32_t* obj, int64_t* subj64, int64_t* obj64, hipStream_t s);
hipError_t launch_enumerate_pairs(int n, int64_t* out, hipStream_t s);

struct AssembleArgs {
  const float* patch_tab;
  const float* lc;
  const float* cls_token;
  const float* pos_embedding;
  const float* ln_w; const float* ln_b;
  const int32_t* subj; const int32_t* obj;
  float* x;
  __bf16* a;
  float* stats;
  int a_fmt;
  int x_f24;
  int n_pair;
  unsigned long long drop_seed;
  unsigned drop_thresh;
  float drop_scale;
};
hipError_t launch_assemble(const AssembleArgs& a, hipStream_t s);
hipError_t launch_centre_split(const float* patch_tab, __bf16* dst, int rows, hipStream_t s);
hipError_t launch_qkv0_combine(const float* sw, const float* ow, const float* stats, const float* vec, const int32_t* subj,
                               const int32_t* obj, float* qkv, int n_pair, hipStream_t s);
hipError_t launch_qkv0_consts(const float* wq, const float* gamma, const float* beta, const float* pos, const float* cls, float* wp,
                              float* vec, hipStream_t s);
hipError_t launch_dropout_apply(const float* x, float* y, size_t rows, int n_cols, unsigned long long seed, unsigned thresh,
                                float scale, hipStream_t s);

hipError_t launch_count_saturation(const void* base, long stride_bytes, int rows, int K, unsigned long long* counters, hipStream_t s);
hipError_t launch_layernorm(const float* x, long ldx, const float* w, const float* b, __bf16* dst, int rows,
                            hipStream_t s, int fmt = FMT_SPLIT, long ldd = 0, bool x_f24 = false);
hipError_t launch_unpack_f24(const void* src, float* dst, size_t n, hipStream_t s);

struct AttnArgs {
  const float* qkv;
  __bf16* o;
  int n_pair, heads, cls_only;
  int qkv_f24 = 0;
  int o_fmt = FMT_SPLIT;
  const float* sw = nullptr;
  const float* ow = nullptr;
  const float* stats = nullptr;
  const float* vec = nullptr;
  const int32_t* subj = nullptr;
  const int32_t* obj = nullptr;
};
hipError_t launch_attention(const AttnArgs& a, hipStream_t s);
bool attention_reads_tables(int heads);

struct QkvAttnArgs {
  const char* a;
  const char* w;
  const int* w_exp;
  char* o;
  int n_pair, heads;
  int fast;
};
bool qkv_attn_fused_supports(int heads);
size_t qkv_attn_rows_padded(int n_pair);
hipError_t launch_qkv_attn_fused(const QkvAttnArgs& g, hipStream_t s);
int cls_fold_max_heads();
hipError_t launch_cls_fold_attention(const float* x, const float* ln_w, const float* ln_b, const float* u, __bf16* abar, int n_pair, int heads,
                                     hipStream_t s, bool u_f24 = false);
bool cls_fold_reads_f24();

hipError_t launch_head(const float* cls, const float* wt, const float* bias, float* out, int n_pair,
                       int n_out, hipStream_t s, long ld = kDim);

struct PostArgs {
  const float* rel_logits;
  const float* obj_logits;
  const int64_t* rel_pairs;
  const int32_t* img_obj_off;
  const int32_t* img_pair_off;
  int n_img, n_obj, n_pair, n_rel_cls, n_obj_cls;
  float* obj_scores;
  int64_t* obj_pred;
  float* out_prob;
  int64_t* out_pairs;
  int64_t* out_labels;
  float* out_triple;
  float* prob_tmp;
  float* triple;
  int32_t* label_tmp;
  int32_t* perm;
  int single_cnt;
  int pair_mod;
  int32_t* kept_count;
};
struct MeetGroup {
  const float* logits;
  int width;
  int row0;
  int cols[104];
};
hipError_t launch_postprocess_meet(PostArgs a, const MeetGroup* groups, int n_groups, hipStream_t s);
struct VoteGroup {
  const float* logits[3];
  int width;
  int row0;
  int cols[104];
};
hipError_t launch_postprocess_vote(PostArgs a, const VoteGroup* groups, int n_groups, int voting, hipStream_t s);
int postprocess_max_pairs_per_image();
hipError_t launch_postprocess(const PostArgs& a, hipStream_t s);

struct ObjDecodeArgs {
  const float* logits;
  const int64_t* labels;
  const float* boxes_per_cls;
  const int32_t* img_off;
  int n_img, n_cls;
  int mode;
  float thr;
  float* prob_ws;
  int64_t* obj_pred;
  float* obj_scores;
  float* out_boxes;
};
int obj_decode_max_objects();
hipError_t launch_obj_decode(const ObjDecodeArgs& a, hipStream_t s);
struct PairArgs {
  const float* boxes;
  const float* scores;
  const int32_t* img_off;
  const int32_t* out_off;
  int n_img, max_pairs, require_overlap;
  int64_t* pairs;
  int32_t* counts;
};
int prepare_pairs_max_pairs();
hipError_t launch_prepare_pairs(const PairArgs& a, hipStream_t s);

struct NmsArgs {
  const float* boxes;
  const float* scores;
  const int32_t* seg_off;
  int n_seg, max_keep;
  float thr;
  int64_t* keep;
  int32_t* counts;
};
int nms_max_segment();
hipError_t launch_nms(const NmsArgs& a, int max_seg, hipStream_t s);
struct BoxPostArgs {
  const float* logits;
  const float* regression;
  const float* proposals;
  const float* image_sizes;
  const int32_t* img_off;
  const int32_t* out_off;
  int n_img, n_box, n_cls, reg_cols, cls_agnostic, topn, filter_dup, det_per_img;
  float score_thresh, nms_thresh, wx, wy, ww, wh, xform_clip;
  float* prob;
// ... 406 lines not shown
```

### veto_amd/csrc/rowops.hip

```cpp
#include "common.h"
#include "kernels.h"

namespace veto {

namespace {

__global__ void split_rows_kernel(const float* __restrict__ src, __bf16* __restrict__ dst, size_t n, int K) {
  size_t i = (size_t)blockIdx.x * blockDim.x + threadIdx.x;
  const size_t stride = (size_t)gridDim.x * blockDim.x;
  for (; i < n; i += stride) {
    const size_t row = i / K;
    const int k = (int)(i % K);
    __bf16 h, l;
    split_bf16(src[i], h, l);
    __bf16* d = dst + row * (2 * (size_t)K) + split_index(k);
    d[0] = h;
    d[32] = l;
  }
}

__global__ void mixed_act_rows_kernel(const float* __restrict__ src, __bf16* __restrict__ dst, size_t n, int K) {
  saturating_conversions_on();
  for (size_t i = ((size_t)blockIdx.x * blockDim.x + threadIdx.x) * 4; i < n; i += (size_t)gridDim.x * blockDim.x * 4) {
    const size_t row = i / K;
// ... 4 lines not shown
__global__ void absmax_bits_kernel(const float* __restrict__ src, size_t n, unsigned* __restrict__ out) {
  unsigned m = 0;
  for (size_t i = (size_t)blockIdx.x * blockDim.x + threadIdx.x; i < n; i += (size_t)gridDim.x * blockDim.x) {
    const unsigned b = __float_as_uint(src[i]) & 0x7fffffffu;
    m = b > m ? b : m;
  }
#pragma unroll
  for (int o = 32; o > 0; o >>= 1) { const unsigned t = __shfl_xor(m, o, 64); m = t > m ? t : m; }
  if ((threadIdx.x & 63) == 0) atomicMax(out, m);
}
__device__ __forceinline__ int weight_exp_of(unsigned maxbits) {
  const float mx = __uint_as_float(maxbits);
  int e = 24;
  while (e > 0 && !(ldexpf(mx, e) <= 448.f)) --e;
  return e;
}
__global__ void mixed_weight_rows_kernel(const float* __restrict__ src, __bf16* __restrict__ dst, size_t n, int K,
                                         const int* __restrict__ maxbits) {
  saturating_conversions_on();
  const int e = weight_exp_of((unsigned)*maxbits);
  const float sx = ldexpf(1.f, e), sy = ldexpf(1.f, e + kMixWLoShift);
  for (size_t i = ((size_t)blockIdx.x * blockDim.x + threadIdx.x) * 4; i < n; i += (size_t)gridDim.x * blockDim.x * 4) {
    const size_t row = i / K;
    const int k = (int)(i % K);
    const f32x4 w = *(const f32x4*)(src + i);
    char* base = (char*)dst + row * (4 * (size_t)K);
    f16x4 h;
    float x[4], y[4];
#pragma unroll
    for (int j = 0; j < 4; ++j) {
      h[j] = (_Float16)w[j];
      x[j] = (float)h[j] * sx;
      y[j] = (w[j] - (float)h[j]) * sy;
    }
    *(f16x4*)(base + mixed_h_offset(k)) = h;
    *(u32x2*)(base + mixed_x_offset(k)) = u32x2{pack_e4m3x4(x[0], x[1], x[2], x[3]), pack_e4m3x4(y[0], y[1], y[2], y[3])};
  }
}
__global__ void finish_weight_exp_kernel(int* e) { *e = weight_exp_of((unsigned)*e); }

__global__ __launch_bounds__(256) void transpose_split_kernel(const float* __restrict__ src, long ld, int M, int N,
                                                              __bf16* __restrict__ dst, int Mp) {
  __shared__ float t[32][65];
  const int m0 = blockIdx.x * 32, n0 = blockIdx.y * 64, tid = threadIdx.x;
  const int tx = tid & 63, ty = tid >> 6;
#pragma unroll
  for (int i = 0; i < 8; ++i) {
    const int m = m0 + ty * 8 + i, n = n0 + tx;
    t[ty * 8 + i][tx] = (m < M && n < N) ? src[(size_t)m * ld + n] : 0.f;
  }
  __syncthreads();
#pragma unroll
  for (int r = 0; r < 2; ++r) {
    const int id = tid + 256 * r, nl = id >> 3, piece = id & 7;
    if (n0 + nl >= N) continue;
    bf16x8 out;
#pragma unroll
    for (int e = 0; e < 8; ++e) {
      __bf16 h, l;
      split_bf16(t[8 * (piece & 3) + e][nl], h, l);
      out[e] = piece < 4 ? h : l;
    }
    __bf16* d = dst + (size_t)(n0 + nl) * (2 * (size_t)Mp) + (size_t)(m0 >> 5) * 64 + (piece < 4 ? 8 * piece : 32 + 8 * (piece - 4));
    *(bf16x8*)d = out;
  }
}

__global__ void build_patch_weight_kernel(const float* __restrict__ wd, const float* __restrict__ bd,
                                          const float* __restrict__ wv, const float* __restrict__ bv,
                                          __bf16* __restrict__ dst, float* __restrict__ bias_cat) {
  const int j = blockIdx.x;
  const int half = j / kDim, jj = j % kDim;
  for (int kk = threadIdx.x; kk < 2048; kk += blockDim.x) {
    const int mod = kk >> 10, f = kk & 1023, pp = f >> 8, c = f & 255;
    float v = 0.f;
    if (jj < 512 && mod == 0) v = wd[(size_t)jj * 2048 + pp * 512 + half * 256 + c];
    if (jj >= 512 && mod == 1) v = wv[(size_t)(jj - 512) * 2048 + pp * 512 + half * 256 + c];
    __bf16 h, l;
    split_bf16(v, h, l);
    __bf16* d = dst + (size_t)j * 4096 + split_index(kk);
    d[0] = h;
    d[32] = l;
  }
  if (threadIdx.x == 0) bias_cat[j] = half == 0 ? (jj < 512 ? bd[jj] : bv[jj - 512]) : 0.f;
}

__global__ void build_patch_weight_t_kernel(const float* __restrict__ wd, const float* __restrict__ wv, __bf16* __restrict__ dst) {
  const int kk = blockIdx.x;
  const int mod = kk >> 10, f = kk & 1023, pp = f >> 8, c = f & 255;
  for (int j = threadIdx.x; j < 2 * kDim; j += blockDim.x) {
    const int half = j / kDim, jj = j % kDim;
    float v = 0.f;
    if (kk < 2048) {
      if (jj < 512 && mod == 0) v = wd[(size_t)jj * 2048 + pp * 512 + half * 256 + c];
      if (jj >= 512 && mod == 1) v = wv[(size_t)(jj - 512) * 2048 + pp * 512 + half * 256 + c];
    }
    __bf16 h, l;
    split_bf16(v, h, l);
    __bf16* d = dst + (size_t)kk * (2 * 2 * kDim) + split_index(j);
    d[0] = h;
    d[32] = l;
  }
}

__global__ void transpose_pair_proj_kernel(const float* __restrict__ src, float* __restrict__ dst,
                                           int kin) {
  const int k = blockIdx.x;
  for (int jj = threadIdx.x; jj < 2 * kDim; jj += blockDim.x) {
    const int half = jj / kDim, j = jj % kDim;
    dst[(size_t)k * (2 * kDim) + jj] = src[(size_t)j * (2 * kin) + half * kin + k];
  }
}

__global__ void transpose_head_kernel(const float* __restrict__ src, float* __restrict__ dst, int n_out) {
  const int k = blockIdx.x;
  for (int c = threadIdx.x; c < n_out; c += blockDim.x) dst[(size_t)k * n_out + c] = src[(size_t)c * kDim + k];
}

__global__ __launch_bounds__(256) void bn_batch_stats_kernel(const float* __restrict__ boxes, int box_mode, int n_obj,
                                                             float* __restrict__ out) {
  __shared__ double s_acc[256][4];
  __shared__ double s_mean[4];
  const int tid = threadIdx.x;
  auto feat = [&](int n, double (&v)[4]) {
    const float* b = boxes + (size_t)n * 4;
    float w, h;
    if (box_mode == 0) { w = b[2] - b[0] + 1.f; h = b[3] - b[1] + 1.f; } else { w = b[2]; h = b[3]; }
    v[0] = b[0] + 0.5f * w; v[1] = b[1] + 0.5f * h; v[2] = w; v[3] = h;
  };
  for (int pass = 0; pass < 2; ++pass) {
    double acc[4] = {0, 0, 0, 0};
    for (int n = tid; n < n_obj; n += 256) {
      double v[4];
      feat(n, v);
      for (int k = 0; k < 4; ++k) { const double d = pass == 0 ? v[k] : v[k] - s_mean[k]; acc[k] += pass == 0 ? d : d * d; }
    }
    for (int k = 0; k < 4; ++k) s_acc[tid][k] = acc[k];
    __syncthreads();
    if (tid < 4) {
      double t = 0;
      for (int i = 0; i < 256; ++i) t += s_acc[i][tid];
      if (pass == 0) {
        s_mean[tid] = t / n_obj;
        out[tid] = (float)s_mean[tid];
      } else {
        out[4 + tid] = (float)(t / n_obj);
        out[8 + tid] = (float)(n_obj > 1 ? t / (n_obj - 1) : t);
      }
    }
    __syncthreads();
  }
}

__global__ __launch_bounds__(256) void obj_prep_kernel(ObjPrepArgs a) {
  __shared__ float s_box[4];
  __shared__ float s_pos[kPosDim];
  __shared__ float s_emb[256];
  __shared__ float s_prob[256];
  __shared__ float s_red[2];
  const int n = blockIdx.x, tid = threadIdx.x;

  if (tid < 4) {
    const float* b = a.boxes + (size_t)n * 4;
    float w, h;
    if (a.box_mode == 0) { w = b[2] - b[0] + 1.f; h = b[3] - b[1] + 1.f; }
    else { w = b[2]; h = b[3]; }
    float v = tid == 0 ? b[0] + 0.5f * w : tid == 1 ? b[1] + 0.5f * h : tid == 2 ? w : h;
    s_box[tid] = (v - a.bn_mean[tid]) / sqrtf(a.bn_var[tid] + 1e-5f) * a.bn_w[tid] + a.bn_b[tid];
  }
  if (a.obj_logits) {
    for (int c = tid; c < a.num_obj_cls; c += 256) s_prob[c] = a.obj_logits[(size_t)n * a.num_obj_cls + c];
  }
  __syncthreads();
  if (tid < kPosDim) {
    float acc = a.pos_b[tid];
#pragma unroll
    for (int k = 0; k < 4; ++k) acc += a.pos_w[tid * 4 + k] * s_box[k];
    s_pos[tid] = fmaxf(acc, 0.f);
    if (a.drop_thresh)
      s_pos[tid] = dropout_keep(a.drop_seed, (unsigned long long)n * kPosDim + tid, a.drop_thresh) ? s_pos[tid] * a.drop_scale : 0.f;
    if (a.pos_out && blockIdx.y == 0) a.pos_out[(size_t)n * kPosDim + tid] = s_pos[tid];
  }
  if (a.obj_logits) {
    if (tid == 0) {
      float mx = -INFINITY;
      for (int c = 0; c < a.num_obj_cls; ++c) mx = fmaxf(mx, s_prob[c]);
      float sum = 0.f;
      for (int c = 0; c < a.num_obj_cls; ++c) sum += expf(s_prob[c] - mx);
      s_red[0] = mx;
      s_red[1] = sum;
    }
    __syncthreads();
    const float mx = s_red[0], inv = 1.f / s_red[1];
    __syncthreads();
    for (int c = tid; c < a.num_obj_cls; c += 256) s_prob[c] = expf(s_prob[c] - mx) * inv;
    __syncthreads();
    for (int e = tid; e < a.embed_dim; e += 256) {
      float acc = 0.f;
      for (int c = 0; c < a.num_obj_cls; ++c) acc += s_prob[c] * a.embed[(size_t)c * a.embed_dim + e];
      s_emb[e] = acc;
    }
  } else {
    const int64_t lab = a.labels[n];
    for (int e = tid; e < a.embed_dim; e += 256) s_emb[e] = a.embed[(size_t)lab * a.embed_dim + e];
  }
  __syncthreads();
  float* out = a.lc + (size_t)n * 2 * (2 * kDim);
  const int jj = blockIdx.y * 256 + tid;
  if (jj < 2 * kDim) {
    float acc = jj < kDim ? a.loc_b[jj] : 0.f;
#pragma unroll 16
    for (int k = 0; k < kPosDim; ++k) acc += a.loc_wt[(size_t)k * (2 * kDim) + jj] * s_pos[k];
    out[jj] = acc;
    float acc2 = jj < kDim ? a.cls_b[jj] : 0.f;
#pragma unroll 8
    for (int k = 0; k < a.embed_dim; ++k) acc2 += a.cls_wt[(size_t)k * (2 * kDim) + jj] * s_emb[k];
    out[2 * kDim + jj] = acc2;
  }
}

__global__ __launch_bounds__(256) void patchify_kernel(const float* __restrict__ depth,
                                                       const float* __restrict__ rgb,
                                                       __bf16* __restrict__ dst) {
  const int n = blockIdx.x, mod = blockIdx.y, c = threadIdx.x;
  const float* in = (mod == 0 ? depth : rgb) + ((size_t)n * 256 + c) * 64;
  float v[64];
#pragma unroll
  for (int i = 0; i < 16; ++i) {
    const f32x4 t = *(const f32x4*)(in + 4 * i);
    v[4 * i] = t[0]; v[4 * i + 1] = t[1]; v[4 * i + 2] = t[2]; v[4 * i + 3] = t[3];
  }
#pragma unroll
  for (int y = 0; y < 8; ++y)
#pragma unroll
    for (int x = 0; x < 8; ++x) {
      const int row = n * 16 + (y >> 1) * 4 + (x >> 1);
      const int col = mod * 1024 + ((y & 1) * 2 + (x & 1)) * 256 + c;
      __bf16 h, l;
      split_bf16(v[y * 8 + x], h, l);
      __bf16* d = dst + (size_t)row * 4096 + split_index(col);
      d[0] = h;
      d[32] = l;
    }
}

__global__ __launch_bounds__(256) void unpatchify_kernel(const float* __restrict__ dpa, long ld, float* __restrict__ d_depth,
                                                         float* __restrict__ d_rgb) {
  const int n = blockIdx.x, mod = blockIdx.y, c = threadIdx.x;
  float* out = (mod == 0 ? d_depth : d_rgb);
  if (!out) return;
  out += ((size_t)n * 256 + c) * 64;
#pragma unroll
  for (int y = 0; y < 8; ++y) {
    f32x4 lo, hi;
#pragma unroll
    for (int x = 0; x < 8; ++x) {
      const int row = n * 16 + (y >> 1) * 4 + (x >> 1);
      const int col = mod * 1024 + ((y & 1) * 2 + (x & 1)) * 256 + c;
      const float v = dpa[(size_t)row * ld + col];
      if (x < 4) lo[x] = v; else hi[x - 4] = v;
    }
    *(f32x4*)(out + y * 8) = lo;
    *(f32x4*)(out + y * 8 + 4) = hi;
  }
}

__global__ void pair_indices_kernel(const int64_t* __restrict__ rel_pairs,
                                    const int32_t* __restrict__ img_obj_off,
                                    const int32_t* __restrict__ img_pair_off, int n_img, int n_pair,
                                    int32_t* __restrict__ subj, int32_t* __restrict__ obj,
                                    int64_t* __restrict__ subj64, int64_t* __restrict__ obj64) {
  const int p = blockIdx.x * blockDim.x + threadIdx.x;
  if (p >= n_pair) return;
  int lo = 0, hi = n_img - 1;
  while (lo < hi) {
    const int mid = (lo + hi + 1) >> 1;
    if (img_pair_off[mid] <= p) lo = mid; else hi = mid - 1;
  }
  const int64_t off = img_obj_off[lo];
  const int64_t s = rel_pairs[2 * (size_t)p] + off, o = rel_pairs[2 * (size_t)p + 1] + off;
  subj[p] = (int32_t)s;
  obj[p] = (int32_t)o;
  if (subj64) subj64[p] = s;
  if (obj64) obj64[p] = o;
}

__global__ void enumerate_pairs_kernel(int n, int64_t* __restrict__ out) {
  const long total = n > 1 ? (long)n * (n - 1) : 1;
  const long p = (long)blockIdx.x * blockDim.x + threadIdx.x;
  if (p >= total) return;
  if (n <= 1) { out[0] = 0; out[1] = 0; return; }
  const long i = p / (n - 1), r = p % (n - 1);
  out[2 * p] = i;
  out[2 * p + 1] = r + (r >= i ? 1 : 0);
}

struct RowQ { f32x4 v[9]; };

__device__ __forceinline__ float group16_sum(float v) {
#pragma unroll
  for (int o = 8; o > 0; o >>= 1) v += __shfl_xor(v, o, 64);
  return v;
}

__device__ __forceinline__ void rowq_stats(const RowQ& r, float& mean, float& rstd) {
  float s = 0.f;
#pragma unroll
  for (int j = 0; j < 9; ++j) s += (r.v[j][0] + r.v[j][1]) + (r.v[j][2] + r.v[j][3]);
  mean = group16_sum(s) * (1.f / kDim);
  float sq = 0.f;
#pragma unroll
  for (int j = 0; j < 9; ++j)
#pragma unroll
    for (int e = 0; e < 4; ++e) { const float d = r.v[j][e] - mean; sq += d * d; }
  rstd = 1.f / sqrtf(group16_sum(sq) * (1.f / kDim) + 1e-5f);
}

template <int FMT = FMT_SPLIT>
__device__ __forceinline__ void rowq_normalized_store(const RowQ& r, int q, float mean, float rstd, const float* __restrict__ w,
                                                      const float* __restrict__ b, __bf16* __restrict__ dst) {
#pragma unroll
  for (int j = 0; j < 9; ++j) {
    const int c = 4 * (q + 16 * j);
    const f32x4 wv = *(const f32x4*)(w + c), bv = *(const f32x4*)(b + c);
    f32x4 y;
#pragma unroll
    for (int e = 0; e < 4; ++e) y[e] = (r.v[j][e] - mean) * rstd * wv[e] + bv[e];
    store_act4<FMT>(dst, c, y);
  }
}

template <int FMT = FMT_SPLIT>
__device__ __forceinline__ void rowq_layernorm_store(const RowQ& r, int q, const float* __restrict__ w,
                                                     const float* __restrict__ b, __bf16* __restrict__ dst) {
  float mean, rstd;
  rowq_stats(r, mean, rstd);
  rowq_normalized_store<FMT>(r, q, mean, rstd, w, b, dst);
}

template <bool STATS_ONLY>
__global__ __launch_bounds__(256) void assemble_kernel(AssembleArgs a) {
  const long per_xcd = gridDim.x >> 3;
  const long row = ((long)(blockIdx.x & 7) * per_xcd + (blockIdx.x >> 3)) * 16 + (threadIdx.x >> 4);
  if (row >= (long)a.n_pair * kTokens) return;
  const int q = threadIdx.x & 15;
  const int p = (int)(row / kTokens), t = (int)(row % kTokens);
  const int s = a.subj[p], o = a.obj[p];
  const float *ps = nullptr, *po = nullptr;
  if (t >= 1 && t <= kPatchTokens) {
    ps = a.patch_tab + ((size_t)s * 16 + (t - 1)) * (2 * kDim);
    po = a.patch_tab + ((size_t)o * 16 + (t - 1)) * (2 * kDim) + kDim;
  } else if (t > kPatchTokens) {
    const int which = t - kPatchTokens - 1;
    ps = a.lc + ((size_t)s * 2 + which) * (2 * kDim);
    po = a.lc + ((size_t)o * 2 + which) * (2 * kDim) + kDim;
  }
  RowQ r;
  float* xr = a.x + (size_t)row * kDim;
  char* xr24 = (char*)a.x + (size_t)row * (kDim * 3);
#pragma unroll
  for (int g3 = 0; g3 < 3; ++g3) {
    f32x4 vs[3], vo[3], vp[3];
#pragma unroll
    for (int jj = 0; jj < 3; ++jj) {
      const int c = 4 * (q + 16 * (g3 * 3 + jj));
      vp[jj] = *(const f32x4*)(a.pos_embedding + c);
      if (t == 0) {
        vs[jj] = *(const f32x4*)(a.cls_token + c);
        vo[jj] = f32x4{0.f, 0.f, 0.f, 0.f};
      } else {
        vs[jj] = *(const f32x4*)(ps + c);
        vo[jj] = *(const f32x4*)(po + c);
      }
    }
#pragma unroll
    for (int jj = 0; jj < 3; ++jj) {
      const int j = g3 * 3 + jj, c = 4 * (q + 16 * j);
      f32x4 v = t == 0 ? vs[jj] : vs[jj] + vo[jj];
      if (t > kPatchTokens) {
#pragma unroll
        for (int e = 0; e < 4; ++e) v[e] = fmaxf(v[e], 0.f);
      }
      v += vp[jj];
      if (a.drop_thresh) {
#pragma unroll
        for (int e = 0; e < 4; ++e)
          v[e] = dropout_keep(a.drop_seed, (unsigned long long)row * kDim + c + e, a.drop_thresh) ? v[e] * a.drop_scale : 0.f;
      }
      r.v[j] = v;
      if (a.x_f24) {
        __builtin_nontemporal_store(pack_f24x4(v), (u32x3*)(xr24 + 3 * c));
        continue;
      }
      __builtin_nontemporal_store(v, (f32x4*)(xr + c));
    }
    asm volatile("" ::: "memory");
  }
  if constexpr (STATS_ONLY) {
    float mean, rstd;
    rowq_stats(r, mean, rstd);
    if (q == 0) *(float2*)(a.stats + (size_t)row * 2) = float2{mean, rstd};
  } else {
    rowq_layernorm_store(r, q, a.ln_w, a.ln_b, a.a + (size_t)row * (2 * kDim));
  }
}

__global__ __launch_bounds__(256) void qkv0_combine_kernel(const float* __restrict__ sw, const float* __restrict__ ow,
                                                           const float* __restrict__ stats, const float* __restrict__ vec,
                                                           const int32_t* __restrict__ subj, const int32_t* __restrict__ obj,
                                                           float* __restrict__ qkv, int n_pair) {
  constexpr int N = 3 * kDim, N4 = N / 4;
  __shared__ __attribute__((aligned(16))) float s_vec[N];
  for (int i = threadIdx.x; i < N4; i += 256) ((f32x4*)s_vec)[i] = ((const f32x4*)vec)[i];
  __syncthreads();
  const f32x4* c2 = (const f32x4*)s_vec;
  const int lane = threadIdx.x & 63;
  const long rows = (long)n_pair * (kPatchTokens + 1), per_xcd = (rows + 7) / 8;
  const long r_begin = (blockIdx.x & 7) * per_xcd, r_end = r_begin + per_xcd < rows ? r_begin + per_xcd : rows;
  const long stride = (long)(gridDim.x >> 3) * 4;
  for (long r = r_begin + (long)(blockIdx.x >> 3) * 4 + (threadIdx.x >> 6); r < r_end; r += stride) {
    const int p = (int)(r / (kPatchTokens + 1)), t = (int)(r % (kPatchTokens + 1));
    f32x4* dst = (f32x4*)(qkv + ((size_t)p * kTokens + t) * N);
    if (t == 0) {
      const f32x4* src = (const f32x4*)(vec + 2 * N);
      for (int i = lane; i < N4; i += 64) dst[i] = src[i];
      continue;
    }
    const float rstd = stats[((size_t)p * kTokens + t) * 2 + 1];
    const f32x4* a = (const f32x4*)(sw + ((size_t)subj[p] * kPatchTokens + t - 1) * N);
    const f32x4* b = (const f32x4*)(ow + ((size_t)obj[p] * kPatchTokens + t - 1) * N);
#pragma unroll
    for (int k = 0; k < (N4 + 63) / 64; ++k) {
      const int i = lane + 64 * k;
      if (i < N4) dst[i] = rstd * (a[i] + b[i]) + c2[i];
    }
  }
}
// ... 64 lines not shown
__global__ __launch_bounds__(256) void layernorm_kernel(const float* __restrict__ x, long ldx,
                                                        const float* __restrict__ w,
                                                        const float* __restrict__ b,
                                                        __bf16* __restrict__ dst, int rows, long ldd) {
  saturating_conversions_on();
  const int row = blockIdx.x * 16 + (threadIdx.x >> 4);
  if (row >= rows) return;
  const int q = threadIdx.x & 15;
  RowQ r;
  if constexpr (XF24) {
    const char* xr = (const char*)x + (size_t)row * ldx * 3;
#pragma unroll
    for (int j = 0; j < 9; ++j) {
      const u32x3 d = *(const u32x3*)(xr + 12 * (q + 16 * j));
      r.v[j] = unpack_f24x4(d[0], d[1], d[2]);
    }
  } else {
    const float* xr = x + (size_t)row * ldx;
#pragma unroll
    for (int j = 0; j < 9; ++j) r.v[j] = *(const f32x4*)(xr + 4 * (q + 16 * j));
  }
  rowq_layernorm_store<FMT>(r, q, w, b, dst + (size_t)row * ldd);
}

__global__ __launch_bounds__(256) void unpack_f24_kernel(const char* __restrict__ src, float* __restrict__ dst, size_t n4) {
  for (size_t i = (size_t)blockIdx.x * 256 + threadIdx.x; i < n4; i += (size_t)gridDim.x * 256) {
    const u32x3 d = *(const u32x3*)(src + i * 12);
    *(f32x4*)(dst + i * 4) = unpack_f24x4(d[0], d[1], d[2]);
  }
}

__global__ __launch_bounds__(256) void dropout_apply_kernel(const float* __restrict__ x, float* __restrict__ y, size_t n,
                                                            unsigned long long seed, unsigned thresh, float scale) {
  size_t i = (size_t)blockIdx.x * 256 + threadIdx.x;
  const size_t stride = (size_t)gridDim.x * 256;
  for (; i < n; i += stride) y[i] = dropout_keep(seed, i, thresh) ? x[i] * scale : 0.f;
}

__global__ __launch_bounds__(128) void head_kernel(const float* __restrict__ cls,
                                                   const float* __restrict__ wt,
                                                   const float* __restrict__ bias, float* __restrict__ out,
                                                   int n_pair, int n_out, long ld) {
  __shared__ float s_cls[4][kDim];
  const int p0 = blockIdx.x * 4;
  for (int i = threadIdx.x; i < 4 * kDim; i += 128) {
    const int pp = i / kDim, k = i % kDim;
    s_cls[pp][k] = p0 + pp < n_pair ? cls[(size_t)(p0 + pp) * ld + k] : 0.f;
  }
  __syncthreads();
  for (int c = threadIdx.x; c < n_out; c += 128) {
    float acc[4] = {0.f, 0.f, 0.f, 0.f};
    for (int k = 0; k < kDim; ++k) {
      const float wv = wt[(size_t)k * n_out + c];
#pragma unroll
      for (int pp = 0; pp < 4; ++pp) acc[pp] += wv * s_cls[pp][k];
    }
    const float bv = bias[c];
#pragma unroll
    for (int pp = 0; pp < 4; ++pp)
      if (p0 + pp < n_pair) out[(size_t)(p0 + pp) * n_out + c] = acc[pp] + bv;
  }
}

}

hipError_t launch_split_rows(const float* src, __bf16* dst, size_t rows, int K, hipStream_t s) {
  if (K % 32 != 0) return hipErrorInvalidValue;
  const size_t n = rows * (size_t)K;
  const int blocks = (int)((n + 255) / 256 < 4096 ? (n + 255) / 256 : 4096);
  VETO_LAUNCH(split_rows_kernel, dim3(blocks), dim3(256), 0, s, src, dst, n, K);
  return hipGetLastError();
}

namespace {
__global__ __launch_bounds__(256) void fold_blocks_kernel(const float* __restrict__ qkv, const float* __restrict__ wo, float* __restrict__ out,
                                                          int which, int H, int dh, int dhp, size_t n) {
  const int np = H * dhp, hk = H * kDim;
  for (size_t e = (size_t)blockIdx.x * 256 + threadIdx.x; e < n; e += (size_t)gridDim.x * 256) {
    float v = 0.f;
    if (which == 0) {
      const int r = (int)(e / kDim), c = (int)(e % kDim), h = r / dhp, d = r % dhp;
      if (d < dh) v = qkv[(size_t)(h * dh + d) * kDim + c];
    } else if (which == 1) {
      const int r = (int)(e / np), k = (int)(e % np), h = r / kDim, c = r % kDim, hk2 = k / dhp, d = k % dhp;
      if (hk2 == h && d < dh) v = qkv[(size_t)(kDim + h * dh + d) * kDim + c];
    } else if (which == 2) {
      const int r = (int)(e / hk), k = (int)(e % hk), h = r / dhp, d = r % dhp, hk2 = k / kDim, c = k % kDim;
      if (hk2 == h && d < dh) v = qkv[(size_t)(2 * kDim + h * dh + d) * kDim + c];
    } else {
      const int r = (int)(e / np), k = (int)(e % np), h = k / dhp, d = k % dhp;
      if (d < dh) v = wo[(size_t)r * kDim + h * dh + d];
    }
    out[e] = v;
  }
}
}

hipError_t launch_fold_blocks(const float* qkv, const float* wo, float* out, int which, int heads, int dhp, hipStream_t s) {
  if (heads <= 0 || kDim % heads != 0 || dhp < kDim / heads || which < 0 || which > 3) return hipErrorInvalidValue;
  const int dh = kDim / heads, np = heads * dhp;
  const size_t n = which == 0 ? (size_t)np * kDim : which == 1 ? (size_t)heads * kDim * np : which == 2 ? (size_t)np * heads * kDim : (size_t)kDim * np;
  const int blocks = (int)((n + 255) / 256 < 4096 ? (n + 255) / 256 : 4096);
  VETO_LAUNCH(fold_blocks_kernel, dim3(blocks), dim3(256), 0, s, qkv, wo, out, which, heads, dh, dhp, n);
  return hipGetLastError();
}

hipError_t launch_build_patch_weight_t(const float* wd, const float* wv, __bf16* dst, hipStream_t s) {
  VETO_LAUNCH(build_patch_weight_t_kernel, dim3(kPatchTRows), dim3(256), 0, s, wd, wv, dst);
  return hipGetLastError();
}

hipError_t launch_unpatchify(const float* dpa, long ld, float* d_depth, float* d_rgb, int n_obj, hipStream_t s) {
  VETO_LAUNCH(unpatchify_kernel, dim3(n_obj, 2), dim3(256), 0, s, dpa, ld, d_depth, d_rgb);
  return hipGetLastError();
}

hipError_t launch_transpose_split(const float* src, long ld, int M, int N, __bf16* dst, int Mp, hipStream_t s) {
  if (Mp % 32 != 0 || Mp < M) return hipErrorInvalidValue;
  VETO_LAUNCH(transpose_split_kernel, dim3(Mp / 32, (N + 63) / 64), dim3(256), 0, s, src, ld, M, N, dst, Mp);
  return hipGetLastError();
}

hipError_t launch_build_patch_weight(const float* wd, const float* bd, const float* wv, const float* bv,
                                     __bf16* dst, float* bias_cat, hipStream_t s) {
  VETO_LAUNCH(build_patch_weight_kernel, dim3(2 * kDim), dim3(256), 0, s, wd, bd, wv, bv, dst, bias_cat);
  return hipGetLastError();
}

hipError_t launch_transpose_pair_proj(const float* src, float* dst, int kin, hipStream_t s) {
  VETO_LAUNCH(transpose_pair_proj_kernel, dim3(kin), dim3(256), 0, s, src, dst, kin);
  return hipGetLastError();
}

hipError_t launch_transpose_head(const float* src, float* dst, int n_out, hipStream_t s) {
  VETO_LAUNCH(transpose_head_kernel, dim3(kDim), dim3(128), 0, s, src, dst, n_out);
  return hipGetLastError();
}

hipError_t launch_dropout_apply(const float* x, float* y, size_t rows, int n_cols, unsigned long long seed, unsigned thresh,
                                float scale, hipStream_t s) {
  const size_t n = rows * (size_t)n_cols;
  const int blocks = (int)((n + 255) / 256 < 16384 ? (n + 255) / 256 : 16384);
  VETO_LAUNCH(dropout_apply_kernel, dim3(blocks), dim3(256), 0, s, x, y, n, seed, thresh, scale);
  return hipGetLastError();
}

hipError_t launch_bn_batch_stats(const float* boxes, int box_mode, int n_obj, float* out, hipStream_t s) {
  VETO_LAUNCH(bn_batch_stats_kernel, dim3(1), dim3(256), 0, s, boxes, box_mode, n_obj, out);
  return hipGetLastError();
}

hipError_t launch_obj_prep(const ObjPrepArgs& a, hipStream_t s) {
  if (a.num_obj_cls > 256 || a.embed_dim > 256) return hipErrorInvalidValue;
  VETO_LAUNCH(obj_prep_kernel, dim3(a.n_obj, (2 * kDim + 255) / 256), dim3(256), 0, s, a);
  return hipGetLastError();
}

hipError_t launch_patchify(const float* depth, const float* rgb, __bf16* dst, int n_obj, hipStream_t s) {
  VETO_LAUNCH(patchify_kernel, dim3(n_obj, 2), dim3(256), 0, s, depth, rgb, dst);
  return hipGetLastError();
}

hipError_t launch_pair_indices(const int64_t* rel_pairs, const int32_t* img_obj_off,
                               const int32_t* img_pair_off, int n_img, int n_pair, int32_t* subj,
                               int32_t* obj, int64_t* subj64, int64_t* obj64, hipStream_t s) {
  VETO_LAUNCH(pair_indices_kernel, dim3((n_pair + 255) / 256), dim3(256), 0, s, rel_pairs,
                     img_obj_off, img_pair_off, n_img, n_pair, subj, obj, subj64, obj64);
  return hipGetLastError();
}

hipError_t launch_enumerate_pairs(int n, int64_t* out, hipStream_t s) {
  const long total = n > 1 ? (long)n * (n - 1) : 1;
  VETO_LAUNCH(enumerate_pairs_kernel, dim3((unsigned)((total + 255) / 256)), dim3(256), 0, s, n, out);
  return hipGetLastError();
}

hipError_t launch_assemble(const AssembleArgs& a, hipStream_t s) {
  const long blocks = ((long)a.n_pair * kTokens + 15) / 16;
  if (a.stats) {
    VETO_LAUNCH(assemble_kernel<true>, dim3((unsigned)((blocks + 7) / 8 * 8)), dim3(256), 0, s, a);
    for (int t = kPatchTokens + 1; t < kTokens; ++t) {
      const float* xt = a.x_f24 ? (const float*)((const char*)a.x + (size_t)t * kDim * 3) : a.x + (size_t)t * kDim;
      hipError_t e = launch_layernorm(xt, (long)kTokens * kDim, a.ln_w, a.ln_b, a.a + (size_t)t * 2 * kDim, a.n_pair, s,
                                      a.a_fmt == FMT_MIXED ? FMT_MIXED : FMT_SPLIT, (long)kTokens * 2 * kDim, a.x_f24 != 0);
      if (e != hipSuccess) return e;
    }
  } else {
    if (a.x_f24) return hipErrorInvalidValue;
    VETO_LAUNCH(assemble_kernel<false>, dim3((unsigned)((blocks + 7) / 8 * 8)), dim3(256), 0, s, a);
  }
  return hipGetLastError();
}

hipError_t launch_unpack_f24(const void* src, float* dst, size_t n, hipStream_t s) {
  if (n % 4 != 0) return hipErrorInvalidValue;
  const size_t n4 = n / 4;
  const int blocks = (int)((n4 + 255) / 256 < 4096 ? (n4 + 255) / 256 : 4096);
  VETO_LAUNCH(unpack_f24_kernel, dim3(blocks), dim3(256), 0, s, (const char*)src, dst, n4);
  return hipGetLastError();
}

hipError_t launch_qkv0_combine(const float* sw, const float* ow, const float* stats, const float* vec, const int32_t* subj,
                               const int32_t* obj, float* qkv, int n_pair, hipStream_t s) {
  const long rows = (long)n_pair * (kPatchTokens + 1);
  const unsigned blocks = (unsigned)(rows / 4 + 8 < 4096 ? (rows / 4 + 8) / 8 * 8 : 4096);
  VETO_LAUNCH(qkv0_combine_kernel, dim3(blocks), dim3(256), 0, s, sw, ow, stats, vec, subj, obj, qkv, n_pair);
  return hipGetLastError();
}

__global__ __launch_bounds__(256) void count_saturation_kernel(const char* base, long stride, int rows, int K, unsigned long long* counters) {
  const int per_row = K / 4;
  const long total = (long)rows * per_row;
  unsigned nf = 0, nv = 0, nr = 0;
  for (long i = (long)blockIdx.x * 256 + threadIdx.x; i < total; i += (long)gridDim.x * 256) {
    const int r = (int)(i / per_row), c = (int)(i % per_row);
    const u32x4 v = *(const u32x4*)(base + (size_t)r * stride + (size_t)c * 16);
    if ((c & 15) < 8) {
#pragma unroll
      for (int e = 0; e < 4; ++e) {
        nf += (v[e] & 0x7fffu) >= 0x7bffu;
        nf += ((v[e] >> 16) & 0x7fffu) >= 0x7bffu;
      }
    } else {
#pragma unroll
      for (int e = 0; e < 4; ++e)
#pragma unroll
        for (int b = 0; b < 4; ++b) {
          const unsigned hit = ((v[e] >> (8 * b)) & 0x7fu) >= 0x7eu;
          if (e & 1) nv += hit; else nr += hit;
        }
    }
  }
  unsigned long long f = nf, vv = nv, rr = nr;
#pragma unroll
  for (int o = 32; o > 0; o >>= 1) {
    f += __shfl_xor(f, o, 64);
    vv += __shfl_xor(vv, o, 64);
    rr += __shfl_xor(rr, o, 64);
  }
  if ((threadIdx.x & 63) == 0) {
    if (f) atomicAdd(counters + 1, f);
    if (vv) atomicAdd(counters + 2, vv);
    if (rr) atomicAdd(counters + 3, rr);
    if (blockIdx.x == 0 && threadIdx.x == 0) atomicAdd(counters, (unsigned long long)rows * K);
  }
}

hipError_t launch_centre_split(const float* patch_tab, __bf16* dst, int rows, hipStream_t s) {
  VETO_LAUNCH(centre_split_kernel, dim3((unsigned)((2L * rows + 15) / 16)), dim3(256), 0, s, patch_tab, dst, rows);
  return hipGetLastError();
}

hipError_t launch_qkv0_consts(const float* wq, const float* gamma, const float* beta, const float* pos, const float* cls, float* wp,
                              float* vec, hipStream_t s) {
  VETO_LAUNCH(qkv0_consts_kernel, dim3(3 * kDim), dim3(64), 0, s, wq, gamma, beta, pos, cls, wp, vec);
  return hipGetLastError();
}

hipError_t launch_layernorm(const float* x, long ldx, const float* w, const float* b, __bf16* dst, int rows,
                            hipStream_t s, int fmt, long ldd, bool x_f24) {
  if (ldd == 0) ldd = 2 * kDim;
  if (x_f24) {
    if (fmt == FMT_MIXED) VETO_LAUNCH((layernorm_kernel<FMT_MIXED, true>), dim3((rows + 15) / 16), dim3(256), 0, s, x, ldx, w, b, dst, rows, ldd);
    else VETO_LAUNCH((layernorm_kernel<FMT_SPLIT, true>), dim3((rows + 15) / 16), dim3(256), 0, s, x, ldx, w, b, dst, rows, ldd);
    return hipGetLastError();
  }
  if (fmt == FMT_MIXED) VETO_LAUNCH(layernorm_kernel<FMT_MIXED>, dim3((rows + 15) / 16), dim3(256), 0, s, x, ldx, w, b, dst, rows, ldd);
  else VETO_LAUNCH(layernorm_kernel<FMT_SPLIT>, dim3((rows + 15) / 16), dim3(256), 0, s, x, ldx, w, b, dst, rows, ldd);
  return hipGetLastError();
}

hipError_t launch_mixed_act_rows(const float* src, __bf16* dst, size_t rows, int K, hipStream_t s) {
  if (K % 64 != 0) return hipErrorInvalidValue;
  const size_t n = rows * (size_t)K;
  const int blocks = (int)((n / 4 + 255) / 256 < 2048 ? (n / 4 + 255) / 256 : 2048);
  VETO_LAUNCH(mixed_act_rows_kernel, dim3(blocks), dim3(256), 0, s, src, dst, n, K);
  return hipGetLastError();
}

hipError_t launch_mixed_weight_rows(const float* src, __bf16* dst, size_t rows, int K, int* exp_out, hipStream_t s) {
  if (K % 64 != 0) return hipErrorInvalidValue;
  const size_t n = rows * (size_t)K;
  const int blocks = (int)((n / 4 + 255) / 256 < 2048 ? (n / 4 + 255) / 256 : 2048);
  hipError_t e = hipMemsetAsync(exp_out, 0, sizeof(int), s);
  if (e != hipSuccess) return e;
  VETO_LAUNCH(absmax_bits_kernel, dim3(blocks), dim3(256), 0, s, src, n, (unsigned*)exp_out);
  VETO_LAUNCH(mixed_weight_rows_kernel, dim3(blocks), dim3(256), 0, s, src, dst, n, K, exp_out);
  VETO_LAUNCH(finish_weight_exp_kernel, dim3(1), dim3(1), 0, s, exp_out);
  return hipGetLastError();
}

hipError_t launch_count_saturation(const void* base, long stride_bytes, int rows, int K, unsigned long long* counters, hipStream_t s) {
  if (rows <= 0 || K % 64 != 0 || !counters) return hipErrorInvalidValue;
  const long pieces = (long)rows * (K / 4);
  const int blocks = (int)((pieces + 255) / 256 < 4096 ? (pieces + 255) / 256 : 4096);
  VETO_LAUNCH(count_saturation_kernel, dim3(blocks), dim3(256), 0, s, (const char*)base, stride_bytes, rows, K, counters);
  return hipGetLastError();
}

hipError_t launch_head(const float* cls, const float* wt, const float* bias, float* out, int n_pair,
                       int n_out, hipStream_t s, long ld) {
  VETO_LAUNCH(head_kernel, dim3((n_pair + 3) / 4), dim3(128), 0, s, cls, wt, bias, out, n_pair, n_out, ld);
  return hipGetLastError();
}

}
```

### veto_amd/native.py

```python
import ctypes
import itertools
import os

import torch
from ctypes import (POINTER, Structure, byref, c_char_p, c_double, c_float, c_int, c_int32, c_int64,
                    c_size_t, c_uint32, c_uint64, c_void_p)

_LIB = None

VETO_PRECISE, VETO_FAST, VETO_MIXED = 0, 1, 2
VETO_ATTN_BWD_CLS_ONLY, VETO_ATTN_BWD_QKV_F24, VETO_ATTN_BWD_SPLIT_OUT = 1, 2, 4


class VetoConfig(Structure):
    _fields_ = [(n, c_int32) for n in (
        "struct_size", "dim", "layers", "heads", "patch", "channels", "resolution", "num_obj_cls",
        "embed_dim", "num_out", "precision", "device", "max_chunk_pairs")]


class VetoInputs(Structure):
    _fields_ = [
        ("struct_size", c_int32), ("n_obj", c_int32), ("n_pair", c_int32), ("n_img", c_int32),
        ("roi_rgb", c_void_p), ("roi_depth", c_void_p), ("boxes", c_void_p),
        ("box_mode", c_int32), ("reserved0", c_int32),
# ... 82 lines not shown
                                       "num_pos_per_img")] + \
               [("seed", ctypes.c_uint64)] + \
               [(n, c_void_p) for n in ("relation", "img_obj_offset", "img_rel_offset", "pairs", "labels", "binary_rel",
                                        "counts")]


class VetoBoxMatchArgs(Structure):
    _fields_ = [(n, c_int32) for n in ("struct_size", "n_img", "n_prp", "n_tgt", "mode")] + \
               [("high_threshold", ctypes.c_float), ("low_threshold", ctypes.c_float), ("reg_weights", ctypes.c_float * 4),
                ("reserved0", c_int32)] + \
               [(n, c_void_p) for n in ("prp_boxes", "tgt_boxes", "tgt_labels", "img_prp_offset", "img_tgt_offset",
                                        "img_prp_offset_host", "img_tgt_offset_host", "matched_idxs", "labels", "matched_rows",
                                        "regression_targets")]


class VetoBoxSubsampleArgs(Structure):
    _fields_ = [(n, c_int32) for n in ("struct_size", "n_img", "n_prp", "batch_size_per_image", "num_pos_per_img", "reserved0")] + \
               [("seed", ctypes.c_uint64)] + \
               [(n, c_void_p) for n in ("labels", "img_prp_offset", "img_prp_offset_host", "sampled_inds", "counts")]


class VetoRpnLossArgs(Structure):
    _fields_ = [(n, c_int32) for n in ("struct_size", "n_img", "n_lvl", "n_tgt", "batch_size_per_image", "num_pos_per_img",
                                       "allow_low_quality_matches", "reserved0")] + \
               [(n, ctypes.c_float) for n in ("high_threshold", "low_threshold", "straddle_thresh", "reserved1")] + \
               [("reg_weights", ctypes.c_float * 4), ("beta", c_double), ("seed", ctypes.c_uint64)] + \
               [(n, c_int32 * RPN_MAX_LEVELS) for n in ("level_a", "level_h", "level_w")] + \
               [(n, c_void_p * RPN_MAX_LEVELS) for n in ("objectness", "box_regression", "anchors", "d_objectness",
                                                         "d_box_regression")] + \
               [(n, c_void_p) for n in ("image_sizes", "tgt_boxes", "img_tgt_offset", "img_tgt_offset_host", "losses", "labels",
                                        "matched_idxs", "regression_targets", "sampled_inds", "counts")]


class VetoBoxLossArgs(Structure):
    _fields_ = [(n, c_int32) for n in ("struct_size", "n_rows", "n_cls", "n_reg_cols", "cls_agnostic", "reserved0")] + \
               [("ld_logits", c_int64), ("ld_reg", c_int64)] + \
               [(n, c_void_p) for n in ("class_logits", "box_regression", "labels", "regression_targets", "losses",
                                        "d_class_logits", "d_box_regression")]


class VetoOptimTensor(Structure):
    _fields_ = [(n, c_void_p) for n in ("param", "grad", "exp_avg", "exp_avg_sq")] + [("numel", c_int64), ("step", c_int64)] + \
               [(n, c_double) for n in ("lr", "weight_decay", "beta1", "beta2", "eps")]


class VetoOptimArgs(Structure):
    _fields_ = [(n, c_int32) for n in ("struct_size", "tensor_size", "n_tensors", "mode")] + [("max_norm", c_double)] + \
               [("tensors", POINTER(VetoOptimTensor))] + [(n, c_void_p) for n in ("norms", "total_norm", "coef")]


VETO_OPTIM_NORMS, VETO_OPTIM_CLIP, VETO_OPTIM_STEP, VETO_OPTIM_CLIP_STEP = 0, 1, 2, 3
VETO_OPTIM_CHUNK = 8192


class VetoPostMeetArgs(Structure):
    _fields_ = [(n, c_int32) for n in ("struct_size", "n_obj", "n_pair", "n_groups", "n_rel_cls", "n_obj_cls")] + \
               [(n, c_void_p) for n in ("group_logits", "group_widths", "incre_idx_list", "obj_logits", "rel_pairs",
                                        "obj_scores", "obj_pred", "rel_prob_sorted", "rel_pairs_sorted",
                                        "rel_labels_sorted", "triple_sorted")]


class VetoPostVoteArgs(Structure):
    _fields_ = [(n, c_int32) for n in ("struct_size", "n_obj", "n_pair", "n_groups", "n_rel_cls", "n_obj_cls",
                                       "voting", "reserved0")] + \
               [(n, c_void_p) for n in ("expert_logits", "group_widths", "incre_idx_list", "obj_logits", "rel_pairs",
                                        "obj_scores", "obj_pred", "rel_prob_sorted", "rel_pairs_sorted",
                                        "rel_labels_sorted", "triple_sorted", "kept_count")]


class VetoRoiPoolArgs(Structure):
    _fields_ = [(n, c_int32) for n in ("struct_size", "n_levels", "n_img", "n_roi", "channels", "depth_channels",
                                       "pooled", "sampling_ratio")] + \
               [("level_feat", c_void_p * 4), ("level_h", c_int32 * 4), ("level_w", c_int32 * 4),
                ("level_scale", ctypes.c_float * 4), ("depth_feat", c_void_p), ("depth_h", c_int32),
                ("depth_w", c_int32), ("rois", c_void_p), ("out_rgb", c_void_p), ("out_depth", c_void_p),
                ("out_levels", c_void_p)]


class VetoSggEvalArgs(Structure):
    _fields_ = [("struct_size", c_int32), ("n_img", c_int32), ("n_rel_cls", c_int32), ("n_zeroshot", c_int32),
                ("iou_thres", ctypes.c_float), ("reserved0", c_int32)] + \
               [(n, c_void_p) for n in ("gt_offset", "obj_offset", "pair_offset", "gt_rels", "gt_classes", "gt_boxes",
                                        "pred_pairs", "rel_scores", "pred_classes", "pred_boxes", "obj_scores", "zeroshot",
                                        "gc_rank", "ng_rank", "acc_rank", "zeroshot_flag", "ng_rows", "ng_cols", "ng_count",
                                        "metrics", "pred_obj_offset")]


class VetoSggEvalFoldArgs(Structure):
    _fields_ = [(n, c_int32) for n in ("struct_size", "n_img", "n_rel_cls", "mode", "n_gt_total", "reserved0")] + \
               [(n, c_void_p) for n in ("img_gt_offset", "img_pair_count", "gt_predicate", "gc_rank", "ng_rank", "acc_rank",
                                        "zeroshot_flag", "metrics", "per_image")]


class VetoDetEvalMatchArgs(Structure):
    _fields_ = [(n, c_int32) for n in ("struct_size", "n_img", "n_cls", "n_gt", "n_det", "reserved0")] + \
               [("first_gt_id", c_int64), ("row_offset", c_int64), ("iou_thrs", c_double * 10), ("area_rngs", c_double * 8)] + \
               [(n, c_void_p) for n in ("gt_offset", "det_offset", "gt_offset_host", "det_offset_host", "gt_boxes", "gt_labels",
                                        "det_boxes", "det_scores", "det_labels", "rec_key", "rec_match", "rec_ignore",
                                        "gt_counts", "label_errors")]


class VetoDetEvalAccumulateArgs(Structure):
    _fields_ = [("struct_size", c_int32), ("n_cls", c_int32), ("n_rec", c_int64), ("iou_thrs", c_double * 10),
                ("rec_thrs", c_double * 101)] + \
               [(n, c_void_p) for n in ("rec_key", "rec_match", "rec_ignore", "gt_counts", "precision", "recall", "stats",
                                        "recall50_100")]


class VetoTrainOpts(Structure):
    _fields_ = [("struct_size", c_int32), ("p_pos", ctypes.c_float), ("p_emb", ctypes.c_float), ("p_attn", ctypes.c_float),
                ("seed", ctypes.c_uint64), ("d_roi_rgb", c_void_p), ("d_roi_depth", c_void_p)]


STRUCTS = {
    "veto_config_t": VetoConfig, "veto_inputs_t": VetoInputs, "veto_debug_outputs_t": VetoDebugOutputs,
    "veto_saturation_t": VetoSaturation, "veto_post_args_t": VetoPostArgs, "veto_post_meet_args_t": VetoPostMeetArgs,
    "veto_post_vote_args_t": VetoPostVoteArgs, "veto_obj_decode_args_t": VetoObjDecodeArgs, "veto_pair_args_t": VetoPairArgs,
    "veto_nms_args_t": VetoNmsArgs, "veto_box_post_args_t": VetoBoxPostArgs, "veto_rpn_args_t": VetoRpnArgs,
    "veto_detect_relsample_args_t": VetoDetectRelsampleArgs, "veto_gtbox_relsample_args_t": VetoGtboxRelsampleArgs,
    "veto_box_match_args_t": VetoBoxMatchArgs, "veto_box_subsample_args_t": VetoBoxSubsampleArgs,
    "veto_rpn_loss_args_t": VetoRpnLossArgs, "veto_box_loss_args_t": VetoBoxLossArgs,
    "veto_optim_tensor_t": VetoOptimTensor, "veto_optim_args_t": VetoOptimArgs,
    "veto_roi_pool_args_t": VetoRoiPoolArgs, "veto_sgg_eval_args_t": VetoSggEvalArgs, "veto_train_opts_t": VetoTrainOpts,
    "veto_det_eval_match_args_t": VetoDetEvalMatchArgs, "veto_det_eval_accumulate_args_t": VetoDetEvalAccumulateArgs,
    "veto_sgg_eval_fold_args_t": VetoSggEvalFoldArgs,
}

_P, _I, _Z = c_void_p, c_int32, c_size_t


def _sig(*argtypes, ret=c_int):
    return ret, list(argtypes)


SIGNATURES = {
    "veto_last_error": _sig(ret=c_char_p),
    "veto_version": _sig(ret=c_char_p),
    "veto_create": _sig(POINTER(VetoConfig), POINTER(_P)),
    "veto_destroy": _sig(_P),
    "veto_num_weights": _sig(_P),
    "veto_weight_info": _sig(_P, _I, POINTER(c_char_p), POINTER(_Z)),
    "veto_load_weights": _sig(_P, c_char_p, _P, _Z, _P),
    "veto_workspace_bytes": _sig(_P, _I, _I, ret=_Z),
    "veto_forward": _sig(_P, _P, POINTER(VetoInputs), _P, _Z, _P, POINTER(VetoDebugOutputs)),
    "veto_forward_saturation": _sig(_P, _P, POINTER(VetoInputs), _P, _Z, _P, POINTER(VetoSaturation), _I),
    "veto_enumerate_pairs": _sig(_P, _I, _P),
    "veto_profile_enable": _sig(_P, _I),
    "veto_profile_collect": _sig(_P),
    "veto_profile_entry": _sig(_P, _I, POINTER(c_char_p), POINTER(c_double), POINTER(c_int64), POINTER(c_double), POINTER(c_double)),
    "veto_profile_reset": _sig(_P),
    "veto_debug_gemm": _sig(_P, _P, _P, _P, _P, _I, _I, _I, _I, _P, _Z),
    "veto_debug_gemm_workspace_bytes": _sig(_I, _I, _I, ret=_Z),
    "veto_debug_gemm_forms": _sig(_P, _P, _P, _P, _I, _I, _I, _I, _I, _I, _P, _Z),
    "veto_debug_ffn": _sig(_P, _P, _P, _P, _P, _P, _P, _I, _I, _I, _I, POINTER(c_float), _P, _Z, _P, _P, _P),
    "veto_debug_ffn_workspace_bytes": _sig(_I, ret=_Z),
    "veto_debug_outproj": _sig(_P, _P, _P, _P, _P, _I, _I, _I, _I, POINTER(c_float), _P, _Z, _P, _P, _P),
    "veto_debug_outproj_workspace_bytes": _sig(_I, ret=_Z),
    "veto_debug_layer_tail": _sig(_P, _P, _P, _P, _P, _P, _P, _P, _P, _P, _P, _I, _I, _I, POINTER(c_float), _P, _Z, _P, _P, _P),
    "veto_debug_layer_tail_workspace_bytes": _sig(_I, ret=_Z),
    "veto_debug_qkv_attn": _sig(_P, _P, _P, _I, _I, _I, _I, POINTER(c_float), _P, _Z, _P),
    "veto_debug_qkv_attn_workspace_bytes": _sig(_I, ret=_Z),
    "veto_postprocess": _sig(_P, POINTER(VetoPostArgs), _P, _Z),
    "veto_postprocess_workspace_bytes": _sig(_I, _I, ret=_Z),
    "veto_postprocess_meet": _sig(_P, POINTER(VetoPostMeetArgs), _P, _Z),
    "veto_postprocess_vote": _sig(_P, POINTER(VetoPostVoteArgs), _P, _Z),
    "veto_obj_decode": _sig(_P, POINTER(VetoObjDecodeArgs), _P, _Z),
    "veto_obj_decode_workspace_bytes": _sig(_I, _I, ret=_Z),
    "veto_prepare_test_pairs": _sig(_P, POINTER(VetoPairArgs)),
    "veto_detect_relsample": _sig(_P, POINTER(VetoDetectRelsampleArgs), _P, _Z),
    "veto_detect_relsample_workspace_bytes": _sig(_I, _I, ret=_Z),
    "veto_gtbox_relsample": _sig(_P, POINTER(VetoGtboxRelsampleArgs)),
    "veto_box_match": _sig(_P, POINTER(VetoBoxMatchArgs)),
    "veto_box_subsample": _sig(_P, POINTER(VetoBoxSubsampleArgs)),
    "veto_nms": _sig(_P, POINTER(VetoNmsArgs)),
    "veto_nms_max_segment": _sig(),
    "veto_box_postprocess": _sig(_P, POINTER(VetoBoxPostArgs), _P, _Z),
    "veto_box_postprocess_workspace_bytes": _sig(_I, _I, _I, ret=_Z),
    "veto_rpn_proposals": _sig(_P, POINTER(VetoRpnArgs), _P, _Z),
    "veto_rpn_proposals_workspace_bytes": _sig(POINTER(VetoRpnArgs), ret=_Z),
    "veto_rpn_loss": _sig(_P, POINTER(VetoRpnLossArgs), _P, _Z),
    "veto_rpn_loss_workspace_bytes": _sig(POINTER(VetoRpnLossArgs), ret=_Z),
    "veto_box_loss": _sig(_P, POINTER(VetoBoxLossArgs), _P, _Z),
    "veto_box_loss_workspace_bytes": _sig(POINTER(VetoBoxLossArgs), ret=_Z),
    "veto_optim_step": _sig(_P, POINTER(VetoOptimArgs), _P, _Z),
    "veto_optim_step_workspace_bytes": _sig(POINTER(VetoOptimArgs), ret=_Z),
    "veto_train_workspace_bytes": _sig(_P, _I, _I, ret=_Z),
    "veto_grad_floats": _sig(_P, ret=_Z),
    "veto_weight_offset": _sig(_P, _I, POINTER(_Z)),
    "veto_forward_train": _sig(_P, _P, POINTER(VetoInputs), POINTER(VetoTrainOpts), _P, _Z, _P),
    "veto_backward": _sig(_P, _P, POINTER(VetoInputs), POINTER(VetoTrainOpts), _P, _Z, _P, _P),
    "veto_debug_attention_backward": _sig(_P, _P, _P, _P, _I, _I),
    "veto_debug_layernorm_backward": _sig(_P, _P, _P, _P, _P, _P, _P, _I, _P, _Z),
    "veto_debug_layernorm_backward_workspace_bytes": _sig(_I, ret=_Z),
    "veto_debug_gelu_backward": _sig(_P, _P, _P, _P, _Z),
    "veto_debug_column_sums": _sig(_P, _P, c_int64, _I, _I, _P, _P, _Z),
    "veto_debug_attention_backward_forms": _sig(_P, _P, _P, _P, _P, _I, _I, c_uint32),
    "veto_debug_layernorm_backward_split": _sig(_P, _P, _P, _P, _P, _P, _P, _P, _P, _I, c_uint64, c_uint32, c_float, _P, _Z),
    "veto_debug_layernorm_backward_col_partial_rows": _sig(_I, ret=_I),
    "veto_debug_wgrad": _sig(_P, _P, _P, _P, _I, _I, _I, _I, _P, _Z),
    "veto_debug_wgrad_workspace_bytes": _sig(_I, _I, _I, _I, ret=_Z),
    "veto_ce_loss": _sig(_P, _P, c_int64, _P, _P, _P, _I, _I, _P, _P, _P, _Z),
    "veto_ce_loss_workspace_bytes": _sig(_I, ret=_Z),
    "veto_meet_sample": _sig(_P, _P, _I, _P, _I, _P, _P, _P, _P, _I, _I, _P, _P, _P, _P),
    "veto_roi_pool": _sig(_P, POINTER(VetoRoiPoolArgs)),
    "veto_roi_pool_backward": _sig(_P, POINTER(VetoRoiPoolArgs), _P, _P, POINTER(_P), _P),
    "veto_sgg_eval": _sig(_P, POINTER(VetoSggEvalArgs), _I, _I, _P, _Z),
    "veto_sgg_eval_workspace_bytes": _sig(_I, _I, _I, _I, ret=_Z),
    "veto_sgg_eval_fold": _sig(_P, POINTER(VetoSggEvalFoldArgs), _P, _Z),
    "veto_sgg_eval_fold_workspace_bytes": _sig(_I, _I, ret=_Z),
    "veto_sgg_eval_fold_limits": _sig(POINTER(_I), POINTER(_I)),
    "veto_det_eval_match": _sig(_P, POINTER(VetoDetEvalMatchArgs), _P, _Z),
    "veto_det_eval_match_workspace_bytes": _sig(_I, _I, _I, ret=_Z),
    "veto_det_eval_accumulate": _sig(_P, POINTER(VetoDetEvalAccumulateArgs), _P, _Z),
    "veto_det_eval_accumulate_workspace_bytes": _sig(c_int64, _I, ret=_Z),
    "veto_det_eval_limits": _sig(POINTER(_I), POINTER(_I), POINTER(_I), POINTER(_I)),
}
EXPORTS = list(SIGNATURES)


class VetoError(RuntimeError):
    pass


def library_path():
    return os.environ.get("VETO_AMD_LIB") or os.path.join(os.path.dirname(os.path.abspath(__file__)), "csrc",
                                                          "libveto_amd.so")


def load_library():
    global _LIB
    if _LIB is not None:
        return _LIB
    path = library_path()
    if not os.path.exists(path):
        from .build import build_native
        build_native()
    lib = ctypes.CDLL(path)
    for name, (restype, argtypes) in SIGNATURES.items():
        fn = getattr(lib, name)
        fn.restype, fn.argtypes = restype, argtypes
    _LIB = lib
    return lib


def check(rc):
    if rc < 0:
        raise VetoError("veto_amd native call failed (%d): %s" % (rc, load_library().veto_last_error().decode()))
    return rc


_OFFSETS = {}
_PLAIN = (int, float, type(None))
_WORKSPACES = {}


def device_offsets(*size_lists, device):
    key = (str(device),) + tuple(tuple(sizes) for sizes in size_lists)
    hit = _OFFSETS.get(key)
    if hit is None:
        if len(_OFFSETS) >= 256:
            _OFFSETS.clear()
        rows = [[0] + list(itertools.accumulate(sizes)) for sizes in key[1:]]
        hit = _OFFSETS[key] = torch.tensor(rows, dtype=torch.int32, device=device).unbind(0)
    return hit


class Launch:

    def __init__(self, device, what):
        self.device = torch.device(device)
        if self.device.type != "cuda":
            raise RuntimeError("%s (got %s)" % (what, device))
        self.lib = load_library()
        self.stream = torch.cuda.current_stream(self.device)
        self._tensors = []

    def ptr(self, t):
        if t is None or t.numel() == 0:
            return None
        self._tensors.append(t)
        return t.data_ptr()

    def args(self, struct_cls, **fields):
        a = struct_cls(struct_size=ctypes.sizeof(struct_cls))
        keep = self._tensors.append
        for name, v in fields.items():
            if type(v) not in _PLAIN and isinstance(v, torch.Tensor):
                if v.numel():
                    keep(v)
                    v = v.data_ptr()
                else:
                    v = None
            setattr(a, name, v)
        return a

    def workspace(self, need):
        key = (self.stream.device_index, self.stream.cuda_stream)
        ws = _WORKSPACES.get(key)
        if ws is None or ws.numel() < need:
            ws = _WORKSPACES[key] = torch.empty(max(need, 256), dtype=torch.uint8, device=self.device)
        return ws

    def run(self, name, *tail, handle=None):
        head = (c_void_p(self.stream.cuda_stream),) if handle is None else (handle, c_void_p(self.stream.cuda_stream))
        rc = check(getattr(self.lib, name)(*head, *tail))
        self.record()
# ... 87 lines not shown
```

Baseline: 1.385 million pairs/s.

## Group small GEMMs and fuse object-side prep kernels into single launches

```diff
diff --git a/include/veto_amd.h b/include/veto_amd.h
--- a/include/veto_amd.h
+++ b/include/veto_amd.h
@@ -601,6 +601,8 @@
 int veto_debug_gemm_forms(void* stream, const float* a, const float* w, void* c, int32_t m, int32_t n, int32_t k,
                           int32_t kb_tiles, int32_t kb_steps, int32_t out_form, void* workspace, size_t workspace_bytes);
 
+int veto_debug_gemm_group_tile(const int32_t* rows, int32_t n_prob, int32_t tiles_n, int32_t tile, int32_t* out);
+
 int veto_debug_ffn(void* stream, const float* a, const float* w1, const float* b1, const float* w2, const float* b2,
                    float* x, int32_t m, int32_t mode, int32_t flags, int32_t reps, float* ms_per_rep, void* workspace,
                    size_t workspace_bytes, const float* ln_w, const float* ln_b, void* ln_rows);
diff --git a/veto_amd/csrc/abi_core.hip b/veto_amd/csrc/abi_core.hip
--- a/veto_amd/csrc/abi_core.hip
+++ b/veto_amd/csrc/abi_core.hip
@@ -123,6 +123,21 @@
   const double bytes = 4.0 * ((double)M * K + (double)N * kk) + (double)M * N * (epi == EPI_RESID ? 8.0 : epi == EPI_F24 ? 3.0 : 4.0);
   ProfScope ps(h, s, name, flops, bytes);
   HIP_TRY(launch_gemm_split(g, epi, 0, s));
+  return VETO_OK;
+}
+
+int run_gemm_grouped(veto_handle_t h, hipStream_t s, const char* name, const GemmProblem* probs, int n_prob, SplitW w, long ldc, int N, int K,
+                     long lda, const int* w_exp) {
+  GemmArgs g{};
+  if (w_exp) { g.fmt = FMT_MIXED; g.w_exp = w_exp; }
+  g.w = w; g.lda = lda; g.ldc = ldc; g.N = N; g.K = K;
+  double flops = 0, bytes = 0;
+  for (int i = 0; i < n_prob; ++i) {
+    flops += 2.0 * probs[i].M * (double)N * K;
+    bytes += 4.0 * ((double)probs[i].M * K + (double)N * K) + (double)probs[i].M * N * 4.0;
+  }
+  ProfScope ps(h, s, name, flops, bytes);
+  HIP_TRY(launch_gemm_split_grouped(g, probs, n_prob, EPI_F32, 0, s));
   return VETO_OK;
 }
 
diff --git a/veto_amd/csrc/abi_debug.hip b/veto_amd/csrc/abi_debug.hip
--- a/veto_amd/csrc/abi_debug.hip
+++ b/veto_amd/csrc/abi_debug.hip
@@ -62,6 +62,18 @@
 }
 
 extern "C" {
+
+int veto_debug_gemm_group_tile(const int32_t* rows, int32_t n_prob, int32_t tiles_n, int32_t tile, int32_t* out) {
+  if (!rows || !out || tiles_n <= 0) return fail(VETO_ERR_INVALID, "null argument or tiles_n <= 0");
+  int rt_end[kGemmMaxProblems - 1];
+  const int total = gemm_group_row_tiles(rows, n_prob, rt_end);
+  if (total <= 0) return fail(VETO_ERR_INVALID, "1 to %d problems of at least one row each", kGemmMaxProblems);
+  out[0] = total * tiles_n;
+  if (tile < 0 || tile >= total * tiles_n) return fail(VETO_ERR_INVALID, "tile %d outside the walk's %d tiles", tile, total * tiles_n);
+  const GemmTileRef t = gemm_group_tile(tile, tiles_n, rt_end[0], rt_end[1], rt_end[2]);
+  out[1] = t.prob; out[2] = t.tile_m; out[3] = t.tile_n;
+  return VETO_OK;
+}
 
 size_t veto_debug_gemm_workspace_bytes(int32_t m, int32_t n, int32_t k) {
   if (m <= 0 || n <= 0 || k <= 0) return 0;
diff --git a/veto_amd/csrc/abi_forward.hip b/veto_amd/csrc/abi_forward.hip
--- a/veto_amd/csrc/abi_forward.hip
+++ b/veto_amd/csrc/abi_forward.hip
@@ -49,7 +49,7 @@
 
 struct ForwardPlan {
   int L, H, dhp;
-  bool qkv0_tables, fold_last, mixed, fast, mixed_out, cls_mixed, tail_fused, panel, qkv_f24, qa_fused, x_f24;
+  bool qkv0_tables, fold_last, mixed, fast, mixed_out, cls_mixed, tail_fused, panel, qkv_f24, qa_fused, x_f24, grouped;
   bool ffn_ln_next(int l) const { return mixed && panel && l + 1 < L - 1; }
 };
 
@@ -74,32 +74,49 @@
   p.qa_fused = p.mixed && p.mixed_out && p.tail_fused && !qa_off && qkv_attn_fused_supports(H);
   static const bool x_f24_on = env_knob_is("VETO_X_F24", "1");
   p.x_f24 = x_f24_on && !p.fast && p.mixed && p.mixed_out && p.tail_fused && p.fold_last && p.qkv0_tables && p.qa_fused && L >= 3;
+  static const bool grouped_off = env_knob_is("VETO_GROUPED_LAUNCHES", "0");
+  p.grouped = !grouped_off;
   return p;
 }
 
 int object_side(veto_handle_t h, hipStream_t s, const Workspace& ws, const ForwardPlan& p, const veto_inputs_t* in,
                 const veto_debug_outputs_t* dbg) {
   const int n_obj = in->n_obj, n_pair = in->n_pair;
-  {
-    ProfScope ps(h, s, "pair_indices", 0, (double)n_pair * 24);
-    HIP_TRY(launch_pair_indices(in->rel_pairs, in->img_obj_offset, in->img_pair_offset, in->n_img, n_pair, ws.subj,
-                                ws.obj, dbg ? dbg->subj_inds : nullptr, dbg ? dbg->obj_inds : nullptr, s));
-  }
-  {
-    if (in->bn_batch_stats) HIP_TRY(launch_bn_batch_stats(in->boxes, in->box_mode, n_obj, in->bn_batch_stats, s));
-    const ObjPrepArgs a = obj_prep_args(h, in, ws.lc);
-    ProfScope ps(h, s, "obj_prep", 2.0 * n_obj * 2 * kDim * (kPosDim + h->cfg.embed_dim), (double)n_obj * 2 * 2 * kDim * 4);
-    HIP_TRY(launch_obj_prep(a, s));
-  }
-  {
-    ProfScope ps(h, s, "patchify", 0, (double)n_obj * 2 * 256 * 64 * (4 + 4));
-    HIP_TRY(launch_patchify(in->roi_depth, in->roi_rgb, ws.pa, n_obj, s));
+  if (in->bn_batch_stats) HIP_TRY(launch_bn_batch_stats(in->boxes, in->box_mode, n_obj, in->bn_batch_stats, s));
+  if (p.grouped) {
+    SidePrepArgs a{};
+    a.obj = obj_prep_args(h, in, ws.lc);
+    a.depth = in->roi_depth; a.rgb = in->roi_rgb; a.pa = ws.pa;
+    a.rel_pairs = in->rel_pairs; a.img_obj_off = in->img_obj_offset; a.img_pair_off = in->img_pair_offset; a.n_img = in->n_img; a.n_pair = n_pair;
+    a.subj = ws.subj; a.obj_idx = ws.obj; a.subj64 = dbg ? dbg->subj_inds : nullptr; a.obj64 = dbg ? dbg->obj_inds : nullptr;
+    ProfScope ps(h, s, "side_prep", 2.0 * n_obj * 2 * kDim * (kPosDim + h->cfg.embed_dim),
+                 (double)n_pair * 24 + (double)n_obj * 2 * 2 * kDim * 4 + (double)n_obj * 2 * 256 * 64 * (4 + 4));
+    HIP_TRY(launch_side_prep(a, s));
+  } else {
+    {
+      ProfScope ps(h, s, "pair_indices", 0, (double)n_pair * 24);
+      HIP_TRY(launch_pair_indices(in->rel_pairs, in->img_obj_offset, in->img_pair_offset, in->n_img, n_pair, ws.subj,
+                                  ws.obj, dbg ? dbg->subj_inds : nullptr, dbg ? dbg->obj_inds : nullptr, s));
+    }
+    {
+      const ObjPrepArgs a = obj_prep_args(h, in, ws.lc);
+      ProfScope ps(h, s, "obj_prep", 2.0 * n_obj * 2 * kDim * (kPosDim + h->cfg.embed_dim), (double)n_obj * 2 * 2 * kDim * 4);
+      HIP_TRY(launch_obj_prep(a, s));
+    }
+    {
+      ProfScope ps(h, s, "patchify", 0, (double)n_obj * 2 * 256 * 64 * (4 + 4));
+      HIP_TRY(launch_patchify(in->roi_depth, in->roi_rgb, ws.pa, n_obj, s));
+    }
   }
   int rc = run_gemm(h, s, "gemm_patch", ws.pa, h->patch_w, h->patch_bias, nullptr, 0, ws.patch_tab, nullptr, 2 * kDim,
                     n_obj * 16, 2 * kDim, 2048, EPI_F32);
   if (rc || !p.qkv0_tables) return rc;
   const int R = n_obj * 16;
   HIP_TRY(launch_centre_split(ws.patch_tab, ws.ptab_split, R, s));
+  if (p.grouped) {
+    const GemmProblem tabs[2] = {{ws.ptab_split, ws.sw, h->q0_vec + 3 * kDim, R}, {ws.ptab_split + 2 * kDim, ws.ow, nullptr, R}};
+    return run_gemm_grouped(h, s, "gemm_qkv0_tab", tabs, 2, h->q0_w, 3 * kDim, 3 * kDim, kDim, (long)2 * 2 * kDim);
+  }
   ABI_TRY(run_gemm(h, s, "gemm_qkv0_tab", ws.ptab_split, h->q0_w, h->q0_vec + 3 * kDim, nullptr, 0, ws.sw, nullptr, 3 * kDim, R, 3 * kDim, kDim,
                    EPI_F32, (long)2 * 2 * kDim, 0));
   return run_gemm(h, s, "gemm_qkv0_tab", ws.ptab_split + 2 * kDim, h->q0_w, nullptr, nullptr, 0, ws.ow, nullptr, 3 * kDim, R, 3 * kDim, kDim,
@@ -144,6 +161,16 @@
     if (!attention_reads_tables(p.H)) {
       ProfScope ps(h, s, "qkv0_combine", 0, (double)np * 17 * 3 * kDim * 4 * 3);
       HIP_TRY(launch_qkv0_combine(ws.sw, ws.ow, ws.stats, h->q0_vec, ws.subj + c0, ws.obj + c0, qkv(), np, s));
+    }
+    if (p.grouped) {
+      GemmProblem lc[2];
+      for (int i = 0; i < 2; ++i) {
+        const int t = kTokens - 2 + i;
+        if (mixed) HIP_TRY(count_sat(0, VETO_SAT_QKV_IN, ws.a + (size_t)t * 2 * kDim, (long)kTokens * kDim * 4, np, kDim));
+        lc[i] = GemmProblem{ws.a + (size_t)t * 2 * kDim, qkv() + (size_t)t * 3 * kDim, nullptr, np};
+      }
+      return run_gemm_grouped(h, s, "gemm_qkv0_lc", lc, 2, mixed ? w.qkv_m : w.qkv, (long)kTokens * 3 * kDim, 3 * kDim, kDim,
+                              (long)kTokens * 2 * kDim, mixed ? w.exp_m + LIN_QKV : nullptr);
     }
     for (int t = kTokens - 2; t < kTokens; ++t) {
       if (mixed) HIP_TRY(count_sat(0, VETO_SAT_QKV_IN, ws.a + (size_t)t * 2 * kDim, (long)kTokens * kDim * 4, np, kDim));
diff --git a/veto_amd/csrc/abi_internal.h b/veto_amd/csrc/abi_internal.h
--- a/veto_amd/csrc/abi_internal.h
+++ b/veto_amd/csrc/abi_internal.h
@@ -272,6 +272,9 @@
              float* c, __bf16* c_split, long ldc, int M, int N, int K, int epi, long lda = 0, int w_row0 = 0, DropSite drop = DropSite(),
              const int* w_exp = nullptr, int kb_tiles = 0, int kb_steps = 0);
 
+int run_gemm_grouped(veto_handle_t h, hipStream_t s, const char* name, const GemmProblem* probs, int n_prob, SplitW w, long ldc, int N, int K,
+                     long lda, const int* w_exp = nullptr);
+
 inline ObjPrepArgs obj_prep_args(veto_handle_t h, const veto_inputs_t* in, float* lc) {
   ObjPrepArgs a{};
   a.boxes = in->boxes; a.box_mode = in->box_mode; a.labels = in->obj_labels; a.obj_logits = in->obj_logits;
diff --git a/veto_amd/csrc/gemm_split_ps.hip b/veto_amd/csrc/gemm_split_ps.hip
--- a/veto_amd/csrc/gemm_split_ps.hip
+++ b/veto_amd/csrc/gemm_split_ps.hip
@@ -92,6 +92,16 @@
   while (tile_of(my_tiles) < ntiles) ++my_tiles;
   if (my_tiles == 0) return;
   const int nstages = my_tiles * nk;
+  constexpr bool kGroup = EPI_T == EPI_F32 && !TN;
+  const bool grouped = kGroup && g.n_prob > 1;
+  auto group_tile = [&](int tile) { return gemm_group_tile(tile, g.tiles_n, g.rt_end[0], g.rt_end[1], g.rt_end[2]); };
+  auto problem = [&](int i) {
+    GemmProblem q = g.prob[0];
+    if (i == 1) q = g.prob[1];
+    if (i == 2) q = g.prob[2];
+    if (i == 3) q = g.prob[3];
+    return q;
+  };
 
   if (w >= NCONS) {
     const int lw = (w - NCONS) & (NLOAD - 1);
@@ -121,7 +131,14 @@
     auto setupA = [&](int tile) {
       int k0 = (tile / out_tiles) * nk;
       tile %= out_tiles;
-      const int tile_m = tile / g.tiles_n;
+      int tile_m = tile / g.tiles_n;
+      const __bf16* a_base = g.a;
+      int a_rows = g.M;
+      if (grouped) {
+        const GemmTileRef t = group_tile(tile);
+        const GemmProblem q = problem(t.prob);
+        tile_m = t.tile_m; a_base = q.a; a_rows = q.M;
+      }
       if (g.kb_tiles > 0) k0 = ((tile % g.tiles_n) / g.kb_tiles) * nk;
       if constexpr (TN) {
         tnA = (const char*)g.a + (size_t)tile_m * (BM * 4);
@@ -132,8 +149,8 @@
       for (int i = 0; i < CPA; ++i) {
         const int c = lw + NLOAD * i;
         int row = tile_m * BM + c * 8 + rr;
-        if (g.lda != 2 * K && row >= g.M) row = g.M - 1;
-        srcA[i] = src_of(g.a, g.lda, row, c) + (size_t)k0 * 128;
+        if ((grouped || g.lda != 2 * K) && row >= a_rows) row = a_rows - 1;
+        srcA[i] = src_of(a_base, g.lda, row, c) + (size_t)k0 * 128;
       }
     };
     auto setupW = [&](int tile) {
@@ -154,9 +171,10 @@
     };
     int itA = 0, ktA = 0, bufA = 0, itW = 0, ktW = 0, bufW = 0;
     auto issueA = [&]() {
-      if (ktA == 0 && lw == 0 && g.bias && lane < BN / 4) {
-        const int tn = (tile_of(itA) % out_tiles) % g.tiles_n;
-        glds16((const char*)(g.bias + tn * BN) + lane * 16, smem + kBiasOff + (itA % kBiasSlices) * (BN * 4));
+      if (ktA == 0 && lw == 0) {
+        const int tile = tile_of(itA) % out_tiles, tn = tile % g.tiles_n;
+        const float* bias = grouped ? problem(group_tile(tile).prob).bias : g.bias;
+        if (bias && lane < BN / 4) glds16((const char*)(bias + tn * BN) + lane * 16, smem + kBiasOff + (itA % kBiasSlices) * (BN * 4));
       }
       char* dst = smem + bufA * kABytes + lw * 1024;
       if constexpr (TN) {
@@ -258,7 +276,16 @@
   int s = 0, s3 = 0;
   for (int it = 0; it < my_tiles; ++it) {
     const int tile = tile_of(it) % out_tiles;
-    const int tile_n = tile % g.tiles_n, tile_m = tile / g.tiles_n;
+    const int tile_n = tile % g.tiles_n;
+    int tile_m = tile / g.tiles_n;
+    float* c_base = g.c;
+    int c_rows = g.M;
+    bool has_bias = g.bias != nullptr;
+    if (grouped) {
+      const GemmTileRef t = group_tile(tile);
+      const GemmProblem q = problem(t.prob);
+      tile_m = t.tile_m; c_base = q.c; c_rows = q.M; has_bias = q.bias != nullptr;
+    }
     f32x4 acc[6][4];
 #pragma unroll
     for (int n = 0; n < 6; ++n)
@@ -398,10 +425,10 @@
           f32x4 v = t + res[u & 1][j];
           if (g.bias) v += *(const f32x4*)(bias_lds + n * 64);
           acc[n][m] = v;
-        } else if (row < g.M) {
+        } else if (row < (kGroup ? c_rows : g.M)) {
           const int col = col0 + n * 16;
           f32x4 v = t;
-          if (g.bias) v += *(const f32x4*)(bias_lds + n * 64);
+          if (kGroup ? has_bias : g.bias != nullptr) v += *(const f32x4*)(bias_lds + n * 64);
           if (kDrop) {
 #pragma unroll
             for (int e = 0; e < 4; ++e)
@@ -428,7 +455,7 @@
           } else if (EPI == EPI_F24) {
             *(u32x3*)((char*)g.c + ((size_t)row * g.ldc + col) * 3) = pack_f24x4(v);
           } else {
-            *(f32x4*)(g.c + (size_t)row * g.ldc + col) = v;
+            *(f32x4*)((kGroup ? c_base : g.c) + (size_t)row * g.ldc + col) = v;
           }
         }
       }
@@ -526,10 +553,44 @@
 int gemm_rows_padded(int m) { return (m + BM - 1) / BM * BM; }
 
 hipError_t launch_gemm_split(GemmArgs g, int epi, int precision, hipStream_t s) {
+  g.n_prob = 0;
   if (g.N % BN != 0 || g.K % BK != 0 || g.M <= 0) return hipErrorInvalidValue;
   if (g.lda == 0) g.lda = 2 * (long)g.K;
   g.tiles_m = (g.M + BM - 1) / BM;
   g.tiles_n = g.N / BN;
+  return launch_gemm_split_ps(g, epi, precision, s);
+}
+
+int gemm_group_row_tiles(const int* rows, int n_prob, int (&rt_end)[kGemmMaxProblems - 1]) {
+  if (!rows || n_prob < 1 || n_prob > kGemmMaxProblems) return -1;
+  int total = 0;
+  for (int i = 0; i < kGemmMaxProblems; ++i) {
+    if (i < n_prob) {
+      if (rows[i] <= 0) return -1;
+      total += (rows[i] + BM - 1) / BM;
+    }
+    if (i < kGemmMaxProblems - 1) rt_end[i] = total;
+  }
+  return total;
+}
+
+hipError_t launch_gemm_split_grouped(GemmArgs g, const GemmProblem* probs, int n_prob, int epi, int precision, hipStream_t s) {
+  if (!probs || n_prob < 1 || n_prob > kGemmMaxProblems) return hipErrorInvalidValue;
+  g.a = probs[0].a; g.c = probs[0].c; g.bias = probs[0].bias; g.M = probs[0].M;
+  g.n_prob = 0;
+  if (n_prob == 1) return launch_gemm_split(g, epi, precision, s);
+  if (epi != EPI_F32 || g.tn || g.k_splits > 1 || g.kb_tiles > 0 || g.N % BN != 0 || g.K % BK != 0) return hipErrorInvalidValue;
+  if (g.lda == 0) g.lda = 2 * (long)g.K;
+  int rows[kGemmMaxProblems];
+  for (int i = 0; i < n_prob; ++i) {
+    if (!probs[i].a || !probs[i].c) return hipErrorInvalidValue;
+    rows[i] = probs[i].M;
+    g.prob[i] = probs[i];
+  }
+  g.tiles_m = gemm_group_row_tiles(rows, n_prob, g.rt_end);
+  if (g.tiles_m <= 0) return hipErrorInvalidValue;
+  g.tiles_n = g.N / BN;
+  g.n_prob = n_prob;
   return launch_gemm_split_ps(g, epi, precision, s);
 }
 
diff --git a/veto_amd/csrc/kernels.h b/veto_amd/csrc/kernels.h
--- a/veto_amd/csrc/kernels.h
+++ b/veto_amd/csrc/kernels.h
@@ -4,6 +4,14 @@
 namespace veto {
 
 enum Epi { EPI_F32 = 0, EPI_RESID = 1, EPI_GELU_SPLIT = 2, EPI_ATOMIC = 3, EPI_RESID_DROP = 4, EPI_F24 = 5, EPI_SPLIT = 6, EPI_PRE_GELU = 7, EPI_GELU_BWD = 8 };
+
+constexpr int kGemmMaxProblems = 4;
+struct GemmProblem {
+  const __bf16* a;
+  float* c;
+  const float* bias;
+  int M;
+};
 
 struct GemmArgs {
   const __bf16* a;
@@ -31,7 +39,21 @@
   long ldw;
   int k_valid;
   const __bf16* zero;
-};
+  int n_prob;
+  int rt_end[kGemmMaxProblems - 1];
+  GemmProblem prob[kGemmMaxProblems];
+};
+
+struct GemmTileRef { int prob, tile_m, tile_n; };
+__host__ __device__ inline GemmTileRef gemm_group_tile(int tile, int tiles_n, int e0, int e1, int e2) {
+  GemmTileRef t;
+  const int tm = tile / tiles_n;
+  t.tile_n = tile - tm * tiles_n;
+  t.prob = (tm >= e0) + (tm >= e1) + (tm >= e2);
+  t.tile_m = tm - (t.prob == 0 ? 0 : t.prob == 1 ? e0 : t.prob == 2 ? e1 : e2);
+  return t;
+}
+int gemm_group_row_tiles(const int* rows, int n_prob, int (&rt_end)[kGemmMaxProblems - 1]);
 
 bool env_knob_is(const char* name, const char* value);
 int env_knob_int(const char* name, int dflt);
@@ -39,6 +61,7 @@
 int device_cu_count();
 hipError_t launch_gemm_split(GemmArgs g, int epi, int precision, hipStream_t s);
 hipError_t launch_gemm_split_ps(GemmArgs g, int epi, int precision, hipStream_t s);
+hipError_t launch_gemm_split_grouped(GemmArgs g, const GemmProblem* probs, int n_prob, int epi, int precision, hipStream_t s);
 
 struct FfnArgs {
   const char* a;
@@ -107,6 +130,15 @@
                                const int32_t* img_pair_off, int n_img, int n_pair, int32_t* subj,
                                int32_t* obj, int64_t* subj64, int64_t* obj64, hipStream_t s);
 hipError_t launch_enumerate_pairs(int n, int64_t* out, hipStream_t s);
+
+struct SidePrepArgs {
+  ObjPrepArgs obj;
+  const float* depth; const float* rgb; __bf16* pa;
+  const int64_t* rel_pairs; const int32_t* img_obj_off; const int32_t* img_pair_off;
+  int n_img, n_pair;
+  int32_t* subj; int32_t* obj_idx; int64_t* subj64; int64_t* obj64;
+};
+hipError_t launch_side_prep(const SidePrepArgs& a, hipStream_t s);
 
 struct AssembleArgs {
   const float* patch_tab;
diff --git a/veto_amd/csrc/rowops.hip b/veto_amd/csrc/rowops.hip
--- a/veto_amd/csrc/rowops.hip
+++ b/veto_amd/csrc/rowops.hip
@@ -180,13 +180,13 @@
   }
 }
 
-__global__ __launch_bounds__(256) void obj_prep_kernel(ObjPrepArgs a) {
+__device__ __forceinline__ void obj_prep_body(const ObjPrepArgs& a, const int n, const int y) {
   __shared__ float s_box[4];
   __shared__ float s_pos[kPosDim];
   __shared__ float s_emb[256];
   __shared__ float s_prob[256];
   __shared__ float s_red[2];
-  const int n = blockIdx.x, tid = threadIdx.x;
+  const int tid = threadIdx.x;
 
   if (tid < 4) {
     const float* b = a.boxes + (size_t)n * 4;
@@ -207,7 +207,7 @@
     s_pos[tid] = fmaxf(acc, 0.f);
     if (a.drop_thresh)
       s_pos[tid] = dropout_keep(a.drop_seed, (unsigned long long)n * kPosDim + tid, a.drop_thresh) ? s_pos[tid] * a.drop_scale : 0.f;
-    if (a.pos_out && blockIdx.y == 0) a.pos_out[(size_t)n * kPosDim + tid] = s_pos[tid];
+    if (a.pos_out && y == 0) a.pos_out[(size_t)n * kPosDim + tid] = s_pos[tid];
   }
   if (a.obj_logits) {
     if (tid == 0) {
@@ -234,7 +234,7 @@
   }
   __syncthreads();
   float* out = a.lc + (size_t)n * 2 * (2 * kDim);
-  const int jj = blockIdx.y * 256 + tid;
+  const int jj = y * 256 + tid;
   if (jj < 2 * kDim) {
     float acc = jj < kDim ? a.loc_b[jj] : 0.f;
 #pragma unroll 16
@@ -247,29 +247,44 @@
   }
 }
 
+constexpr int kObjPrepSlices = (2 * kDim + 255) / 256;
+
+__global__ __launch_bounds__(256) void obj_prep_kernel(ObjPrepArgs a) { obj_prep_body(a, blockIdx.x, blockIdx.y); }
+
+template <int PARTS>
+__device__ __forceinline__ void patchify_body(const float* __restrict__ depth, const float* __restrict__ rgb, __bf16* __restrict__ dst,
+                                              const int n, const int mod) {
+  constexpr int YS = 8 / PARTS;
+  const int c = threadIdx.x;
+  const float* in = (mod == 0 ? depth : rgb) + ((size_t)n * 256 + c) * 64;
+#pragma unroll
+  for (int part = 0; part < PARTS; ++part) {
+    float v[YS * 8];
+#pragma unroll
+    for (int i = 0; i < YS * 2; ++i) {
+      const f32x4 t = *(const f32x4*)(in + part * YS * 8 + 4 * i);
+      v[4 * i] = t[0]; v[4 * i + 1] = t[1]; v[4 * i + 2] = t[2]; v[4 * i + 3] = t[3];
+    }
+#pragma unroll
+    for (int yy = 0; yy < YS; ++yy)
+#pragma unroll
+      for (int x = 0; x < 8; ++x) {
+        const int y = part * YS + yy;
+        const int row = n * 16 + (y >> 1) * 4 + (x >> 1);
+        const int col = mod * 1024 + ((y & 1) * 2 + (x & 1)) * 256 + c;
+        __bf16 h, l;
+        split_bf16(v[yy * 8 + x], h, l);
+        __bf16* d = dst + (size_t)row * 4096 + split_index(col);
+        d[0] = h;
+        d[32] = l;
+      }
+  }
+}
+
 __global__ __launch_bounds__(256) void patchify_kernel(const float* __restrict__ depth,
                                                        const float* __restrict__ rgb,
                                                        __bf16* __restrict__ dst) {
-  const int n = blockIdx.x, mod = blockIdx.y, c = threadIdx.x;
-  const float* in = (mod == 0 ? depth : rgb) + ((size_t)n * 256 + c) * 64;
-  float v[64];
-#pragma unroll
-  for (int i = 0; i < 16; ++i) {
-    const f32x4 t = *(const f32x4*)(in + 4 * i);
-    v[4 * i] = t[0]; v[4 * i + 1] = t[1]; v[4 * i + 2] = t[2]; v[4 * i + 3] = t[3];
-  }
-#pragma unroll
-  for (int y = 0; y < 8; ++y)
-#pragma unroll
-    for (int x = 0; x < 8; ++x) {
-      const int row = n * 16 + (y >> 1) * 4 + (x >> 1);
-      const int col = mod * 1024 + ((y & 1) * 2 + (x & 1)) * 256 + c;
-      __bf16 h, l;
-      split_bf16(v[y * 8 + x], h, l);
-      __bf16* d = dst + (size_t)row * 4096 + split_index(col);
-      d[0] = h;
-      d[32] = l;
-    }
+  patchify_body<1>(depth, rgb, dst, blockIdx.x, blockIdx.y);
 }
 
 __global__ __launch_bounds__(256) void unpatchify_kernel(const float* __restrict__ dpa, long ld, float* __restrict__ d_depth,
@@ -293,12 +308,11 @@
   }
 }
 
-__global__ void pair_indices_kernel(const int64_t* __restrict__ rel_pairs,
-                                    const int32_t* __restrict__ img_obj_off,
-                                    const int32_t* __restrict__ img_pair_off, int n_img, int n_pair,
-                                    int32_t* __restrict__ subj, int32_t* __restrict__ obj,
-                                    int64_t* __restrict__ subj64, int64_t* __restrict__ obj64) {
-  const int p = blockIdx.x * blockDim.x + threadIdx.x;
+__device__ __forceinline__ void pair_indices_body(const int64_t* __restrict__ rel_pairs,
+                                                  const int32_t* __restrict__ img_obj_off,
+                                                  const int32_t* __restrict__ img_pair_off, int n_img, int n_pair,
+                                                  int32_t* __restrict__ subj, int32_t* __restrict__ obj,
+                                                  int64_t* __restrict__ subj64, int64_t* __restrict__ obj64, const int p) {
   if (p >= n_pair) return;
   int lo = 0, hi = n_img - 1;
   while (lo < hi) {
@@ -311,6 +325,28 @@
   obj[p] = (int32_t)o;
   if (subj64) subj64[p] = s;
   if (obj64) obj64[p] = o;
+}
+
+__global__ void pair_indices_kernel(const int64_t* __restrict__ rel_pairs,
+                                    const int32_t* __restrict__ img_obj_off,
+                                    const int32_t* __restrict__ img_pair_off, int n_img, int n_pair,
+                                    int32_t* __restrict__ subj, int32_t* __restrict__ obj,
+                                    int64_t* __restrict__ subj64, int64_t* __restrict__ obj64) {
+  pair_indices_body(rel_pairs, img_obj_off, img_pair_off, n_img, n_pair, subj, obj, subj64, obj64, blockIdx.x * blockDim.x + threadIdx.x);
+}
+
+constexpr int kSidePrepPerObj = kObjPrepSlices + 2;
+
+__global__ __launch_bounds__(256) void side_prep_kernel(SidePrepArgs a) {
+  const int b = blockIdx.x, nb_obj = a.obj.n_obj * kSidePrepPerObj;
+  if (b < nb_obj) {
+    const int n = b / kSidePrepPerObj, r = b - n * kSidePrepPerObj;
+    if (r < kObjPrepSlices) obj_prep_body(a.obj, n, r);
+    else patchify_body<2>(a.depth, a.rgb, a.pa, n, r - kObjPrepSlices);
+  } else {
+    pair_indices_body(a.rel_pairs, a.img_obj_off, a.img_pair_off, a.n_img, a.n_pair, a.subj, a.obj_idx, a.subj64, a.obj64,
+                      (b - nb_obj) * 256 + (int)threadIdx.x);
+  }
 }
 
 __global__ void enumerate_pairs_kernel(int n, int64_t* __restrict__ out) {
@@ -681,7 +717,13 @@
 
 hipError_t launch_obj_prep(const ObjPrepArgs& a, hipStream_t s) {
   if (a.num_obj_cls > 256 || a.embed_dim > 256) return hipErrorInvalidValue;
-  VETO_LAUNCH(obj_prep_kernel, dim3(a.n_obj, (2 * kDim + 255) / 256), dim3(256), 0, s, a);
+  VETO_LAUNCH(obj_prep_kernel, dim3(a.n_obj, kObjPrepSlices), dim3(256), 0, s, a);
+  return hipGetLastError();
+}
+
+hipError_t launch_side_prep(const SidePrepArgs& a, hipStream_t s) {
+  if (a.obj.num_obj_cls > 256 || a.obj.embed_dim > 256 || a.obj.n_obj <= 0 || a.n_pair <= 0) return hipErrorInvalidValue;
+  VETO_LAUNCH(side_prep_kernel, dim3((unsigned)(a.obj.n_obj * kSidePrepPerObj + (a.n_pair + 255) / 256)), dim3(256), 0, s, a);
   return hipGetLastError();
 }
 
diff --git a/veto_amd/native.py b/veto_amd/native.py
--- a/veto_amd/native.py
+++ b/veto_amd/native.py
@@ -258,6 +258,7 @@
     "veto_debug_gemm": _sig(_P, _P, _P, _P, _P, _I, _I, _I, _I, _P, _Z),
     "veto_debug_gemm_workspace_bytes": _sig(_I, _I, _I, ret=_Z),
     "veto_debug_gemm_forms": _sig(_P, _P, _P, _P, _I, _I, _I, _I, _I, _I, _P, _Z),
+    "veto_debug_gemm_group_tile": _sig(_P, _I, _I, _I, _P),
     "veto_debug_ffn": _sig(_P, _P, _P, _P, _P, _P, _P, _I, _I, _I, _I, POINTER(c_float), _P, _Z, _P, _P, _P),
     "veto_debug_ffn_workspace_bytes": _sig(_I, ret=_Z),
     "veto_debug_outproj": _sig(_P, _P, _P, _P, _P, _I, _I, _I, _I, POINTER(c_float), _P, _Z, _P, _P, _P),
```

Result: no change. 1.390 million pairs/s, median of 6 (+0.4%).
